# hyeeiin/ECG-Multimodal-Model

Hardware: AMD Instinct MI355X
Metric: samples/sec fwd+bwd, batch-256 multimodal (img+sig+clin), 1->8 MI355X (higher is better)
Workload: dtype bf16; 1 GPU; full multimodal (image 3x224x224 + 5000-pt signal + 16-dim clinical), fwd+bwd+Adam, encoders unfrozen; image_hw=224x224, per_gpu_batch=256, global_batch=256, parallelism=dp1

## Files before the change

### ecg-multimodal-model_amd/csrc/api.hip

```cpp
#include <stdarg.h>

#include "ops.h"

static thread_local char g_err[512] = "";

void ecg_set_error(const char* fmt, ...) {
  va_list ap;
  va_start(ap, fmt);
  vsnprintf(g_err, sizeof(g_err), fmt, ap);
  va_end(ap);
}

static inline ConvGeom geom_of(const ecgmm_conv_desc* c) {
  return make_geom(c->N, c->H, c->W, c->Cin, c->Cout, c->R, c->S, c->stride, c->pad_h, c->pad_w);
}
#define S_(x) ((hipStream_t)(x))

extern "C" {

int ecgmm_version(void) { return ECGMM_VERSION; }
const char* ecgmm_last_error(void) { return g_err; }

const char* ecgmm_switch_name(int i) { return i >= 0 && i < sw::COUNT ? sw::ALL[i]->env : nullptr; }
int ecgmm_switch_get(const char* env_name, int64_t* value) {
  Switch* s = sw::find(env_name);
  if (!s) ECG_FAIL(ECGMM_ERR_SHAPE, "switch_get: unknown switch %s", env_name ? env_name : "(null)");
  if (!value) ECG_FAIL(ECGMM_ERR_SHAPE, "switch_get: null value pointer");
  *value = s->get();
  return 0;
}
int ecgmm_switch_set(const char* env_name, int64_t value) {
  Switch* s = sw::find(env_name);
  if (!s) ECG_FAIL(ECGMM_ERR_SHAPE, "switch_set: unknown switch %s", env_name ? env_name : "(null)");
  if (s == &sw::SIDE_WGRAD)
    ECG_FAIL(ECGMM_ERR_SHAPE, "switch_set: ECGMM_SIDE_WGRAD is each plan's own state after start-up, call ecgmm_side_wgrad()");
  if (!s->runtime) ECG_FAIL(ECGMM_ERR_SHAPE, "switch_set: %s is read once at start-up", s->env);
  s->set((long)value);
  return 0;
}
int ecgmm_conv_halo_enable(int on) { sw::CONV_HALO.set(on); return 0; }
int ecgmm_conv_halo_cus(int cus) { sw::HALO_CUS.set(cus); return 0; }
int ecgmm_conv_halo_w4(int on) { sw::HALO_W4.set(on); return 0; }
int ecgmm_conv_halo_stagger(int on) { sw::HALO_STAGGER.set(on); return 0; }
int ecgmm_conv_halo_stream(int on) { sw::HALO_STREAM.set(on); return 0; }
int ecgmm_conv_halo_pingpong(int on) { sw::HALO_PP.set(on); return 0; }
int ecgmm_conv_wgrad_pingpong(int on) { sw::WGRAD_PP.set(on); return 0; }
int ecgmm_conv_wgrad_ring_enable(int on) { sw::WGRAD_RING.set(on); return 0; }
int ecgmm_bn_fold(int on) { sw::BN_FOLD.set(on); return 0; }
int ecgmm_bn_fold_slice(int on) { sw::BN_FOLD_SLICE.set(on); return 0; }
int ecgmm_bn_dual(int on) { ecg_bn_dual_set(on); return 0; }
int ecgmm_bn_fuse_min_pixels(int64_t m) { sw::BN_FUSE_MIN_M.set((long)m); return 0; }
int ecgmm_stem_recompute(int on) { sw::STEM_RECOMPUTE.set(on); return 0; }
int ecgmm_infer_down_side(int on) { sw::INFER_DOWN_SIDE.set(on); return 0; }

int ecgmm_nchw_to_nhwc(int dtype, const float* src, void* dst, int N, int C, int64_t HW, void* stream) {
  return ecg_nchw_to_nhwc(dtype, src, dst, N, C, (long)HW, S_(stream));
}
int ecgmm_nhwc_to_nchw(int dtype, const void* src, float* dst, int N, int C, int64_t HW, void* stream) {
  return ecg_nhwc_to_nchw(dtype, src, dst, N, C, (long)HW, S_(stream));
}
int ecgmm_cast(int dtype, const float* src, void* dst, int64_t n, void* stream) {
  return ecg_cast(dtype, src, dst, (long)n, S_(stream));
}
int ecgmm_uncast(int dtype, const void* src, float* dst, int64_t n, void* stream) {
  return ecg_uncast(dtype, src, dst, (long)n, S_(stream));
}
int ecgmm_pack_conv_weight(int dtype, const float* w, void* fwd, void* dgrad, int Cout, int Cin, int RS,
                           void* stream) {
  return ecg_pack_weight(dtype, w, fwd, dgrad, Cout, Cin, RS, S_(stream));
}

int ecgmm_conv_stats_rows(int64_t out_pixels) { return ecg_conv_stats_rows((long)out_pixels); }
int ecgmm_conv_fwd(int dtype, const ecgmm_conv_desc* c, const void* x, const void* w_fwd, const float* bias, void* y,
                   float* stats, int act, void* stream) {
  return ecg_conv_igemm(dtype, 0, geom_of(c), x, w_fwd, y, bias, nullptr, stats, act, S_(stream));
}
int ecgmm_conv_bwd_data(int dtype, const ecgmm_conv_desc* c, const void* dy, const void* w_dgrad, const void* addend,
                        void* dx, void* stream) {
  return ecg_conv_igemm(dtype, 1, geom_of(c), dy, w_dgrad, dx, nullptr, addend, nullptr, 0, S_(stream));
}
size_t ecgmm_conv_bwd_weight_workspace(int dtype, const ecgmm_conv_desc* c) {
  return ecg_conv_wgrad_workspace(dtype, geom_of(c));
}
int ecgmm_conv_bwd_weight(int dtype, const ecgmm_conv_desc* c, const void* x, const void* dy, float* dw, int accumulate,
                          void* ws, size_t ws_bytes, void* stream) {
  return ecg_conv_wgrad(dtype, geom_of(c), x, dy, dw, accumulate, ws, ws_bytes, S_(stream));
}

size_t ecgmm_stem_packed_elems(int Cin, int R) { return ecg_stem_packed_elems(Cin, R); }
int ecgmm_stem_stats_rows(int N, int Cin, int H, int W, int R) { return ecg_stem_stats_rows(N, Cin, H, W, R); }
int ecgmm_stem_pack(int dtype, const float* w, void* packed, int Cin, int R, void* stream) {
  return ecg_stem_pack(dtype, w, packed, Cin, R, S_(stream));
}
int ecgmm_stem_fwd(int dtype, const float* x, const void* packed, const float* bias, void* y, float* stats, int N,
                   int Cin, int H, int W, int R, void* stream) {
  return ecg_stem_fwd(dtype, x, packed, bias, y, stats, N, Cin, H, W, R, S_(stream));
}
int ecgmm_stem_wg_stats_rows(int N, int Cin, int H, int W, int R) { return ecg_stem_wg_stats_rows(N, Cin, H, W, R); }
int ecgmm_stem_fwd_wgrows(int dtype, const float* x, const void* packed, const float* bias, void* y, float* stats, int N,
                          int Cin, int H, int W, int R, void* stream) {
  return ecg_stem_fwd_wgrows(dtype, x, packed, bias, y, stats, N, Cin, H, W, R, S_(stream));
}
int ecgmm_stem_stats_only_rows(int N, int Cin, int H, int W, int R) { return ecg_stem_stats_only_rows(N, Cin, H, W, R); }
int ecgmm_stem_stats_only(int dtype, const float* x, const void* packed, const float* bias, float* stats, int N, int Cin,
                          int H, int W, int R, void* stream) {
  return ecg_stem_stats_only(dtype, x, packed, bias, stats, N, Cin, H, W, R, S_(stream));
}
int ecgmm_stem_pool_fwd(const float* x, const void* packed, const float* coef, void* pooled, uint8_t* idx, int N, int Cin,
                        int H, int W, void* stream) {
  return ecg_stem_pool_fwd(x, packed, coef, pooled, idx, N, Cin, H, W, S_(stream));
}
size_t ecgmm_stem_pool_bwd_workspace(int N, int Cin, int H, int W) { return ecg_stem_pool_bwd_workspace(N, Cin, H, W); }
int ecgmm_stem_pool_bwd(const float* x, const void* packed, const float* coef, const float* gamma, const void* dp,
                        const void* pooled, const uint8_t* idx, float* dgamma, float* dbeta, float* dw_oihw, void* ws,
                        size_t ws_bytes, int N, int Cin, int H, int W, void* stream) {
  return ecg_stem_pool_bwd(x, packed, coef, gamma, dp, pooled, idx, dgamma, dbeta, dw_oihw, ws, ws_bytes, N, Cin, H, W,
                           S_(stream));
}
size_t ecgmm_stem_bwd_weight_workspace(int N, int Cin, int H, int W, int R) {
  return ecg_stem_wgrad_workspace(N, Cin, H, W, R);
}
int ecgmm_stem_bwd_weight(int dtype, const float* x, const void* dy, float* dw, int accumulate, void* ws,
                          size_t ws_bytes, int N, int Cin, int H, int W, int R, void* stream) {
  return ecg_stem_wgrad(dtype, x, dy, dw, accumulate, ws, ws_bytes, N, Cin, H, W, R, S_(stream));
}

int ecgmm_stem_bwd_data(int dtype, const void* dy, const float* w_oihw, float* dx, int N, int Cin, int H, int W, int R,
                        void* stream) {
  return ecg_stem_dgrad(dtype, dy, w_oihw, dx, N, Cin, H, W, R, S_(stream));
}

int ecgmm_bn_eval_bwd(int dtype, const void* dout, const void* maskref, const float* gate, const float* addc,
                      int rows_per_sample, const void* y, const float* coef, float* dgamma, float* dbeta, void* dy,
                      void* dz_out, float* dbias, int64_t M, int C, float* scratch, void* stream) {
  return ecg_bn_eval_bwd(dtype, dout, maskref, gate, addc, rows_per_sample, y, coef, dgamma, dbeta, dy, dz_out, dbias,
                         (long)M, C, scratch, S_(stream));
}
int ecgmm_bn_small_eval_bwd(const float* x, const float* dy, const float* gamma, const float* save, float* dx,
                            float* dgamma, float* dbeta, int N, int C, int accumulate, void* stream) {
  return ecg_bn_small_eval_bwd(x, dy, gamma, save, dx, dgamma, dbeta, N, C, accumulate, S_(stream));
}

int ecgmm_col_stats_rows(int dtype, int64_t M, int C) { return ecg_bn_rows(dtype, (long)M, C); }
int ecgmm_col_stats(int dtype, const void* x, int64_t M, int C, float* partial, void* stream) {
  int rows = 0;
  return ecg_col_stats(dtype, x, (long)M, C, partial, &rows, S_(stream));
}
int ecgmm_bn_finalize(const float* partial, int rows, int C, double count, const float* gamma, const float* beta,
                      float* rm, float* rv, int64_t* nbt, float momentum, float eps, float* coef, void* stream) {
  return ecg_bn_finalize(partial, rows, C, count, gamma, beta, rm, rv, (long long*)nbt, momentum, eps, coef,
                         S_(stream));
}
int ecgmm_bn_eval_coef(int C, const float* gamma, const float* beta, const float* rm, const float* rv, float eps,
                       float* coef, void* stream) {
  return ecg_bn_eval_coef(C, gamma, beta, rm, rv, eps, coef, S_(stream));
}
int ecgmm_bn_act(int dtype, const void* y, const float* coef, const void* res, const float* rcoef, const float* gate,
                 int rows_per_sample, int relu, void* out, int64_t M, int C, void* stream) {
  return ecg_bn_act(dtype, y, coef, res, rcoef, gate, rows_per_sample, relu, out, (long)M, C, S_(stream));
}
int ecgmm_bn_act_from_rows(int dtype, const void* y, const float* partial, int rows, double count, const float* gamma,
                           const float* beta, float* running_mean, float* running_var, int64_t* num_batches_tracked,
                           float momentum, float eps, float* coef_out, const void* res, const float* rcoef,
                           const float* gate, int rows_per_sample, int relu, void* out, int64_t M, int C, void* stream) {
  return ecgmm_bn_act_from_rows_bits(dtype, y, partial, rows, count, gamma, beta, running_mean, running_var, num_batches_tracked,
                                     momentum, eps, coef_out, res, rcoef, gate, rows_per_sample, relu, out, nullptr, M, C, stream);
}
int ecgmm_bn_act_from_rows_bits(int dtype, const void* y, const float* partial, int rows, double count, const float* gamma,
                                const float* beta, float* running_mean, float* running_var, int64_t* num_batches_tracked,
                                float momentum, float eps, float* coef_out, const void* res, const float* rcoef,
                                const float* gate, int rows_per_sample, int relu, void* out, uint8_t* relu_bits, int64_t M,
                                int C, void* stream) {
  if (!partial || !coef_out) ECG_FAIL(ECGMM_ERR_SHAPE, "bn_act_from_rows: null partial rows / coef");
  if (!ecg_bn_fold_ok(C, rows)) {
    ECG_TRY(ecg_bn_finalize(partial, rows, C, count, gamma, beta, running_mean, running_var, (long long*)num_batches_tracked,
                            momentum, eps, coef_out, S_(stream)));
    return ecg_bn_act(dtype, y, coef_out, res, rcoef, gate, rows_per_sample, relu, out, (long)M, C, S_(stream), relu_bits);
  }
  EcgBnFold f = {partial, rows, count, gamma, beta, running_mean, running_var, (long long*)num_batches_tracked, momentum, eps};
  return ecg_bn_act_fold(dtype, y, coef_out, f, res, rcoef, gate, rows_per_sample, relu, out, (long)M, C, S_(stream), relu_bits);
}
size_t ecgmm_bn_bwd_scratch(int dtype, int64_t M, int C) { return ecg_bn_bwd_scratch(dtype, (long)M, C); }
int ecgmm_bn_bwd(int dtype, const void* dout, const void* maskref, const float* gate, const float* addc,
                 int rows_per_sample, const void* y, const float* coef, const float* gamma, float* dgamma,
                 float* dbeta, void* dy, void* dz_out, float* dbias, int64_t M, int C, void* scratch, void* stream) {
  return ecg_bn_bwd(dtype, dout, maskref, gate, addc, rows_per_sample, y, coef, gamma, dgamma, dbeta, dy, dz_out, dbias,
                    (long)M, C, (float*)scratch, S_(stream));
}
int ecgmm_bn_bwd_bits(int dtype, const void* dout, const uint8_t* mask_bits, const float* gate, const float* addc,
                      int rows_per_sample, const void* y, const float* coef, const float* gamma, float* dgamma,
                      float* dbeta, void* dy, void* dz_out, float* dbias, int64_t M, int C, void* scratch, void* stream) {
  if (dtype != ECGMM_BF16 || !mask_bits) ECG_FAIL(ECGMM_ERR_SHAPE, "bn_bwd_bits: bf16 with a bit mask only");
  return ecg_bn_bwd(dtype, dout, nullptr, gate, addc, rows_per_sample, y, coef, gamma, dgamma, dbeta, dy, dz_out, dbias,
                    (long)M, C, (float*)scratch, S_(stream), mask_bits);
}
int ecgmm_bn_bwd_dual(int dtype, const void* dout, const void* maskref, const uint8_t* mask_bits, const float* gate,
                      const float* addc, const void* y_a, const float* coef_a, const float* gamma_a, float* dgamma_a,
                      float* dbeta_a, void* dy_a, const void* y_b, const float* coef_b, const float* gamma_b,
                      float* dgamma_b, float* dbeta_b, void* dy_b, void* dz, float* dbias, int64_t M, int C, void* scratch_a,
                      void* scratch_b, void* stream) {
  return ecg_bn_bwd_dual(dtype, dout, maskref, mask_bits, gate, addc, y_a, coef_a, gamma_a, dgamma_a, dbeta_a, dy_a, y_b,
                         coef_b, gamma_b, dgamma_b, dbeta_b, dy_b, dz, dbias, (long)M, C, (float*)scratch_a, (float*)scratch_b,
                         S_(stream));
}

int ecgmm_conv_bwd_data_bnred(int dtype, const ecgmm_conv_desc* c, const void* dy, const void* w_dgrad,
                              const void* addend, void* dx, const void* bn_y, const void* bn_mask, const float* bn_coef,
                              float* rows, int* nrows, void* stream) {
  if (!bn_y || !bn_coef || !rows || !nrows) ECG_FAIL(ECGMM_ERR_SHAPE, "conv_bwd_data_bnred: null BatchNorm operand");
  const ConvGeom g = geom_of(c);
  *nrows = 0;
  if (!ecg_conv_halo_ok(dtype, 1, g))
    return ecg_conv_igemm(dtype, 1, g, dy, w_dgrad, dx, nullptr, addend, nullptr, 0, S_(stream));
  ConvEpi e = {};
  e.wg_rows = 1; e.red_y = bn_y; e.red_mask = bn_mask; e.red_coef = bn_coef; e.red_rows = rows;
  int rc = ecg_conv_igemm(dtype, 1, g, dy, w_dgrad, dx, nullptr, addend, nullptr, 0, S_(stream), &e);
  if (rc == 0 && e.red_done) *nrows = e.red_rows_n;
  return rc;
}
int ecgmm_conv_fwd_wgrows(int dtype, const ecgmm_conv_desc* c, const void* x, const void* w_fwd, const float* bias, void* y,
                          float* stats, int* nrows, int act, void* stream) {
  if (!stats || !nrows) ECG_FAIL(ECGMM_ERR_SHAPE, "conv_fwd_wgrows: null statistics buffer / row count");
// ... 273 lines not shown
```

### ecg-multimodal-model_amd/csrc/conv_wgrad.hip

```cpp
#include "ops.h"

namespace {

struct WgradParams {
  const void* x;
  const void* dy;
  float* slab;
  int N, H, W, Cin, OH, OW, Cout, S, stride, pad_h, pad_w;
  int M;
  int steps_per_split;
  unsigned mul_hw, sh_hw, mul_w, sh_w;
};

__device__ __forceinline__ void wg_dma16(__amdgpu_buffer_rsrc_t rs, unsigned char* lds_wave_base, unsigned voffset) {
#if defined(__HIP_DEVICE_COMPILE__)
  __builtin_amdgcn_raw_ptr_buffer_load_lds(rs, (__attribute__((address_space(3))) void*)lds_wave_base, 16, voffset, 0, 0,
                                           0);
#endif
}

#ifdef ECG_STAMP
__device__ unsigned long long g_wstamp[8];
#define ECG_WSTAMP_AT(t)                                                                 \
  do {                                                                                    \
// ... 490 lines not shown
      s16x4 hi = __builtin_amdgcn_ds_read_tr16_b64_v4i16((__attribute__((address_space(3))) s16x4*)lds_ptr(a0 + 512u));
      uint2 l2 = __builtin_bit_cast(uint2, lo), h2 = __builtin_bit_cast(uint2, hi);
      fa[a] = (u32x4){l2.x, l2.y, h2.x, h2.y};
    }
    int n_ow = st_ow + d_ow;
    const bool cw = n_ow >= p.W;
    n_ow -= cw ? p.W : 0;
    int n_oh = st_oh + d_oh + (cw ? 1 : 0);
    if (n_oh >= p.H) n_oh -= p.H;
    const unsigned n_rot = (rot + 4096u) & (RING_BYTES - 1);
    const TapOk nk = tap_ok(n_oh, n_ow);
    (void)rot;
    auto rd_tap = [&](int t, u32x4& fb) {
#if defined(WG_ABL) && WG_ABL == 2
      fb = (u32x4){al[t], ah[t], 0x3c003c00u, 0x3c003c00u};
      return;
#endif
      s16x4 lo = __builtin_amdgcn_ds_read_tr16_b64_v4i16((__attribute__((address_space(3))) s16x4*)lds_ptr(al[t]));
      s16x4 hi = __builtin_amdgcn_ds_read_tr16_b64_v4i16((__attribute__((address_space(3))) s16x4*)lds_ptr(ah[t]));
      uint2 l2 = __builtin_bit_cast(uint2, lo), h2 = __builtin_bit_cast(uint2, hi);
      fb = (u32x4){l2.x, l2.y, h2.x, h2.y};
    };
    u32x4 fbA, fbB;
    rd_tap(0, fbA);
#pragma unroll
    for (int t = 0; t < NT; ++t) {
      u32x4& cur = (t & 1) ? fbB : fbA;
      u32x4& nxt = (t & 1) ? fbA : fbB;
      if (t + 1 < NT) rd_tap(t + 1, nxt);
#if defined(WG_ABL) && WG_ABL == 1
      asm volatile("" ::"v"(cur), "v"(fa[0]), "v"(fa[1]), "v"(fa[2]), "v"(fa[3]));
#else
#pragma unroll
      for (int a = 0; a < TA; ++a)
        acc[t][a] = __builtin_amdgcn_mfma_f32_16x16x32_bf16(__builtin_bit_cast(bf16x8_t, fa[a]),
                                                            __builtin_bit_cast(bf16x8_t, cur), acc[t][a], 0, 0, 0);
#endif
      if (t >= 1) tap_addr(t - 1, nk, n_rot, al[t - 1], ah[t - 1]);
      if (PP_OK && t == PP_SPLIT - 1 && pp) {
        __builtin_amdgcn_sched_barrier(0);
        __builtin_amdgcn_s_barrier();
        __builtin_amdgcn_sched_barrier(0);
      }
    }
    tap_addr(NT - 1, nk, n_rot, al[NT - 1], ah[NT - 1]);
    st_oh = n_oh;
    st_ow = n_ow;
  };

  const int nsteps = max(s_end - s_begin, 0);
  if (iters > 0) {
    if (nsteps > 0) {
      for (int pc = wv; pc * 8 < 32 + 2 * p.HLa; pc += 4) x_piece(P0 - p.HLa + pc * 8);
      dy_piece(0, s_begin);
      for (int j = 1; j < RING_D && j < nsteps; ++j) dma_step(j, s_begin + j);
    }
    ring_wait_vmcnt<0>();
    __builtin_amdgcn_s_waitcnt(0xC07F);
    __builtin_amdgcn_s_barrier();
    unsigned rot = 0u;
    if (pp && grp == 1) __builtin_amdgcn_s_barrier();
    for (int k = 0; k < iters; ++k) {
      if (GROUPS == 1 || k < nsteps) {
#if !(defined(WG_ABL) && WG_ABL == 3)
        if (k + RING_D < nsteps) dma_step((k + RING_D) % RING_NDY, s_begin + k + RING_D);
#endif
        compute(k % RING_NDY, rot);
        rot = (rot + 4096u) & (RING_BYTES - 1);
        const int younger = (k + RING_D < nsteps ? k + RING_D : nsteps - 1) - (k + 1);
        if (younger >= 2) ring_wait_vmcnt<4>();
        else if (younger == 1) ring_wait_vmcnt<2>();
        else ring_wait_vmcnt<0>();
      } else if (pp) {
        __builtin_amdgcn_s_barrier();
      }
      __builtin_amdgcn_s_waitcnt(0xC07F);
      __builtin_amdgcn_s_barrier();
    }
    if (pp && grp == 0) __builtin_amdgcn_s_barrier();
  }

  if constexpr (GROUPS == 2) {
    float* red = reinterpret_cast<float*>(smem_wg) + (tid & 255);
    if (grp == 1) {
#pragma unroll
      for (int t = 0; t < NT; ++t)
#pragma unroll
        for (int a = 0; a < TA; ++a)
#pragma unroll
          for (int j = 0; j < 4; ++j) red[((t * TA + a) * 4 + j) * 256] = acc[t][a][j];
    }
    __syncthreads();
    if (grp == 1) return;
#pragma unroll
    for (int t = 0; t < NT; ++t)
#pragma unroll
      for (int a = 0; a < TA; ++a)
#pragma unroll
        for (int j = 0; j < 4; ++j) acc[t][a][j] += red[((t * TA + a) * 4 + j) * 256];
  }

  float* base = p.slab + (((size_t)split * NT) * p.Cout + co0 + fq * 4) * p.Cin + ci0 + wave * 16 + fr;
#pragma unroll
  for (int t = 0; t < NT; ++t)
#pragma unroll
    for (int a = 0; a < TA; ++a)
#pragma unroll
      for (int j = 0; j < 4; ++j) base[((size_t)t * p.Cout + a * 16 + j) * p.Cin] = acc[t][a][j];
}

void magic_div(unsigned d, unsigned& m, unsigned& sh) {
  int l = 0;
  while ((1u << l) < d) ++l;
  m = (unsigned)(((1ull << (31 + l)) + d - 1) / d);
  sh = 31 + l;
}

__global__ void wgrad_reduce_kernel(const float* __restrict__ slab, float* __restrict__ grad, int nsplit, int RS,
                                    int Cout, int Cin, int accumulate) {
  __shared__ float sh[4][64];
  size_t per = (size_t)RS * Cout * Cin;
  size_t i = (size_t)blockIdx.x * 64 + (threadIdx.x & 63);
  const int grp = threadIdx.x >> 6;
  float s0 = 0.f, s1 = 0.f;
  if (i < per) {
    int k = grp;
    for (; k + 12 < nsplit; k += 16) {
      const float a0 = slab[(size_t)k * per + i], a1 = slab[(size_t)(k + 4) * per + i];
      const float a2 = slab[(size_t)(k + 8) * per + i], a3 = slab[(size_t)(k + 12) * per + i];
      s0 += a0;
      s1 += a1;
      s0 += a2;
      s1 += a3;
    }
    for (; k + 4 < nsplit; k += 8) {
      s0 += slab[(size_t)k * per + i];
      s1 += slab[(size_t)(k + 4) * per + i];
    }
    if (k < nsplit) s0 += slab[(size_t)k * per + i];
  }
  sh[grp][threadIdx.x & 63] = s0 + s1;
  __syncthreads();
  if (grp == 0 && i < per) {
    float s = (sh[0][threadIdx.x] + sh[1][threadIdx.x]) + (sh[2][threadIdx.x] + sh[3][threadIdx.x]);
    int ci = (int)(i % Cin);
    size_t r = i / Cin;
    int co = (int)(r % Cout);
    int tap = (int)(r / Cout);
    size_t o = ((size_t)co * Cin + ci) * RS + tap;
    grad[o] = accumulate ? grad[o] + s : s;
  }
}

template <typename T, int NT, int GROUPS>
int launch_wgrad_nt(WgradParams& p, dim3 grid, hipStream_t stream) {
  size_t lds = (size_t)GROUPS * 2 * (1 + NT) * 4096;
  if (GROUPS == 2 && lds < (size_t)NT * 16 * 1024) lds = (size_t)NT * 16 * 1024;
  static bool attr_set = false;
  if (!attr_set) {
    (void)hipFuncSetAttribute((const void*)wgrad_kernel<T, NT, GROUPS>, hipFuncAttributeMaxDynamicSharedMemorySize, (int)lds);
    attr_set = true;
  }
  hipLaunchKernelGGL((wgrad_kernel<T, NT, GROUPS>), grid, dim3(256 * GROUPS), lds, stream, p);
  ECG_CHECK_LAUNCH("wgrad_kernel");
  return 0;
}

int wgrad_groups(int dtype, const ConvGeom& g) {
  return dtype == ECGMM_BF16 && g.R * g.S >= 3 && !sw::WGRAD_GROUPS.get() ? 2 : 1;
}

template <typename T>
int launch_wgrad(const ConvGeom& g, WgradParams& p, int nsplit, int groups, hipStream_t stream) {
  const int RS = g.R * g.S;
  dim3 grid(ceil_div(g.Cout, 64) * ceil_div(g.Cin, 64), nsplit);
  if (g.S != 1 && g.S != 3) ECG_FAIL(ECGMM_ERR_SHAPE, "conv wgrad: filter width %d unsupported (1 or 3)", g.S);
  if constexpr (sizeof(T) == 2) {
    if (groups == 2 && RS == 3) return launch_wgrad_nt<T, 3, 2>(p, grid, stream);
    if (groups == 2 && RS == 9) return launch_wgrad_nt<T, 9, 2>(p, grid, stream);
  }
  if (RS == 1) return launch_wgrad_nt<T, 1, 1>(p, grid, stream);
  if (RS == 3) return launch_wgrad_nt<T, 3, 1>(p, grid, stream);
  if (RS == 9) return launch_wgrad_nt<T, 9, 1>(p, grid, stream);
  ECG_FAIL(ECGMM_ERR_SHAPE, "conv wgrad: %dx%d filter unsupported (1, 3 or 9 taps)", g.R, g.S);
}

bool wgrad_ring_ok(int dtype, const ConvGeom& g) {
  const long level = sw::WGRAD_RING.get();
  if (!level || dtype != ECGMM_BF16 || g.stride != 1 || g.S != 3 || g.pad_w != 1) return false;
  if (!((g.R == 3 && g.pad_h == 1) || (g.R == 1 && g.pad_h == 0))) return false;
  if (g.OH != g.H || g.OW != g.W || g.W < 4 || g.Cin % 64 || g.Cout % 64) return false;
  const int HL = g.pad_h * g.W + 1, HLa = (HL + 7) / 8 * 8;
  if (HL + HLa + 32 * RING_D + 32 > RING_ROWS) return false;
  const double M = (double)g.N * g.H * g.W;
  if (!(M * g.Cin * 2.0 < 2.0e9 && M * g.Cout * 2.0 < 2.0e9)) return false;
  if (level == 2) return true;
  return g.R == 3 || g.Cin >= 128;
}

template <int NT, int GROUPS>
int launch_wgrad_ring(const WgradRingParams& p, dim3 grid, hipStream_t stream) {
  int lds = GROUPS * RING_LDS;
  if (GROUPS == 2 && lds < NT * 16 * 1024) lds = NT * 16 * 1024;
  static bool attr_set = false;
  if (!attr_set) {
    (void)hipFuncSetAttribute((const void*)wgrad_ring_kernel<NT, GROUPS>, hipFuncAttributeMaxDynamicSharedMemorySize, lds);
    attr_set = true;
  }
  hipLaunchKernelGGL((wgrad_ring_kernel<NT, GROUPS>), grid, dim3(256 * GROUPS), lds, stream, p);
  ECG_CHECK_LAUNCH("wgrad_ring_kernel");
  return 0;
}

bool g_wgrad_narrow = false;
int g_wgrad_narrow_slots = 256;
int pick_nsplit(const ConvGeom& g, int kp, int groups) {
  long M = (long)g.N * g.OH * g.OW;
  int tiles = ceil_div(g.Cout, 64) * ceil_div(g.Cin, 64);
  int steps = ceil_div(M, kp);
  const int slots_env = (int)sw::WGRAD_WGS.get();
  const int slots = slots_env > 0 ? slots_env : (g_wgrad_narrow ? g_wgrad_narrow_slots : 512);
  int want = ceil_div(slots / groups, tiles);
  int ns = want < 1 ? 1 : want;
  if (ns > steps) ns = steps;
  if (ns > 512) ns = 512;
  return ns < 1 ? 1 : ns;
}

}

void ecg_conv_wgrad_narrow(bool narrow, int slots) { g_wgrad_narrow = narrow; g_wgrad_narrow_slots = slots > 0 ? slots : 256; }

size_t ecg_conv_wgrad_workspace(int dtype, const ConvGeom& g) {
  const bool keep = g_wgrad_narrow;
  g_wgrad_narrow = false;
  struct Restore { bool v; ~Restore() { g_wgrad_narrow = v; } } restore{keep};
  int ns = pick_nsplit(g, dtype == ECGMM_BF16 ? 32 : 16, 1);
  return (size_t)ns * g.R * g.S * g.Cout * g.Cin * sizeof(float);
}

int ecg_conv_wgrad(int dtype, const ConvGeom& g, const void* x, const void* dy, float* grad_oihw, int accumulate,
                   void* workspace, size_t workspace_bytes, hipStream_t stream) {
  const int kp = dtype == ECGMM_BF16 ? 32 : 16;
  const int vec = dtype == ECGMM_BF16 ? 8 : 4;
  if (g.Cin % vec || g.Cout % vec)
    ECG_FAIL(ECGMM_ERR_SHAPE, "conv wgrad: channels (%d,%d) must be multiples of %d", g.Cin, g.Cout, vec);
  long M = (long)g.N * g.OH * g.OW;
  if (M <= 0 || M > 0x7fffffffL) ECG_FAIL(ECGMM_ERR_SHAPE, "conv wgrad: pixel count %ld out of range", M);
  const bool ring = wgrad_ring_ok(dtype, g);
  const int groups = wgrad_groups(dtype, g);
  int ns = pick_nsplit(g, kp, groups);
  size_t need = (size_t)ns * g.R * g.S * g.Cout * g.Cin * sizeof(float);
  if (workspace_bytes < need || !workspace)
    ECG_FAIL(ECGMM_ERR_WORKSPACE, "conv wgrad: workspace %zu < %zu bytes", workspace_bytes, need);
  WgradParams p;
  p.x = x; p.dy = dy; p.slab = (float*)workspace;
  p.N = g.N; p.H = g.H; p.W = g.W; p.Cin = g.Cin; p.OH = g.OH; p.OW = g.OW; p.Cout = g.Cout; p.S = g.S;
  p.stride = g.stride; p.pad_h = g.pad_h; p.pad_w = g.pad_w; p.M = (int)M;
  p.steps_per_split = ceil_div(ceil_div(M, kp), ns);
  magic_div((unsigned)(g.OH * g.OW), p.mul_hw, p.sh_hw);
  magic_div((unsigned)g.OW, p.mul_w, p.sh_w);
  if (dtype != ECGMM_BF16 && dtype != ECGMM_F32) ECG_FAIL(ECGMM_ERR_DTYPE, "conv wgrad: bad dtype %d", dtype);
  ecg_prof_begin(ECG_PROF_WGRAD, 2.0 * (double)M * g.Cout * g.R * g.S * g.Cin,
                 (double)dtype_size(dtype) * ((double)g.N * g.H * g.W * g.Cin + (double)M * g.Cout) +
                     4.0 * g.R * g.S * g.Cin * g.Cout,
                 stream);
  int rc;
  if (ring) {
    WgradRingParams q;
    q.x = x; q.dy = dy; q.slab = (float*)workspace;
    q.H = g.H; q.W = g.W; q.Cin = g.Cin; q.Cout = g.Cout; q.pad_h = g.pad_h; q.M = (int)M;
    q.steps_per_split = p.steps_per_split;
    q.HL = g.pad_h * g.W + 1;
    q.HLa = (q.HL + 7) / 8 * 8;
    q.mul_hw = p.mul_hw; q.sh_hw = p.sh_hw; q.mul_w = p.mul_w; q.sh_w = p.sh_w;
    q.pingpong = (int)sw::WGRAD_PP.get();
    dim3 grid((g.Cout / 64) * (g.Cin / 64), ns);
    if (groups == 2) rc = g.R == 3 ? launch_wgrad_ring<9, 2>(q, grid, stream) : launch_wgrad_ring<3, 2>(q, grid, stream);
    else rc = g.R == 3 ? launch_wgrad_ring<9, 1>(q, grid, stream) : launch_wgrad_ring<3, 1>(q, grid, stream);
  } else {
    rc = dtype == ECGMM_BF16 ? launch_wgrad<bf16_t>(g, p, ns, groups, stream) : launch_wgrad<float>(g, p, ns, 1, stream);
  }
  ecg_prof_end(stream);
  ECG_TRY(rc);
  size_t per = (size_t)g.R * g.S * g.Cout * g.Cin;
  hipLaunchKernelGGL(wgrad_reduce_kernel, dim3(ceil_div(per, 64)), dim3(256), 0, stream, (const float*)workspace,
                     grad_oihw, ns, g.R * g.S, g.Cout, g.Cin, accumulate);
  ECG_CHECK_LAUNCH("wgrad_reduce_kernel");
  return 0;
}
```

### ecg-multimodal-model_amd/csrc/elementwise.hip

```cpp
#include "ops.h"

namespace {

constexpr int EW_THREADS = 256;

__device__ __forceinline__ u32x4 ld16(const void* p) { return *reinterpret_cast<const u32x4*>(p); }
__device__ __forceinline__ u32x4 ld16s(const void* p) {
#ifndef EW_NO_NT
  return __builtin_nontemporal_load(reinterpret_cast<const u32x4*>(p));
#else
  return *reinterpret_cast<const u32x4*>(p);
#endif
}
struct RowDiv { unsigned mul, sh; };
__device__ __forceinline__ long row_div(long r, RowDiv d) { return (long)(((unsigned long long)(unsigned)r * d.mul) >> d.sh); }
static RowDiv make_row_div(int d) {
  unsigned dd = d < 1 ? 1u : (unsigned)d;
  int l = 0;
  while ((1u << l) < dd) ++l;
  RowDiv r;
  r.mul = (unsigned)(((1ull << (31 + l)) + dd - 1) / dd);
  r.sh = 31u + (unsigned)l;
  return r;
}
// ... 1174 lines not shown
    unpack16<T>(qv, v);
#pragma unroll
    for (int j = 0; j < VEC; ++j) {
      f[j] = m[j] > 0.f ? f[j] : 0.f;
      const float yc = v[j] - mu[j];
      ag[j] += f[j] * (v[j] * sc[j] + sf[j]);
      a1[j] += f[j];
      a2[j] += f[j] * yc;
      a3[j] += yc;
    }
    st16(dz + o, pack16<T>(f));
  };
  int r = slice;
  for (; r + 3 * nsl < R; r += 4 * nsl) {
    u32x4 qd[4], qm[4], qv[4];
#pragma unroll
    for (int u = 0; u < 4; ++u) {
      const size_t o = ((size_t)n * R + r + u * nsl) * C + c0;
      qd[u] = ld16(dout + o);
      qm[u] = ld16(maskref + o);
      qv[u] = ld16(y + o);
    }
    __builtin_amdgcn_sched_barrier(0);
#pragma unroll
    for (int u = 0; u < 4; ++u) row(((size_t)n * R + r + u * nsl) * C + c0, qd[u], qm[u], qv[u]);
  }
  for (; r < R; r += nsl) {
    const size_t o = ((size_t)n * R + r) * C + c0;
    const u32x4 qd = ld16(dout + o), qm = ld16(maskref + o), qv = ld16(y + o);
    row(o, qd, qm, qv);
  }
  float* const outs[4] = {dg, a1o, a2o, a3o};
#pragma unroll
  for (int q = 0; q < 4; ++q) {
#pragma unroll
    for (int j = 0; j < VEC; ++j) sh[threadIdx.x][j] = q == 0 ? ag[j] : q == 1 ? a1[j] : q == 2 ? a2[j] : a3[j];
    __syncthreads();
    for (int c = threadIdx.x; c < C; c += EW_THREADS) {
      const int ck = c / VEC, j = c % VEC;
      float s_ = 0.f;
      for (int k = 0; k < nsl; ++k) s_ += sh[k * cpr + ck][j];
      outs[q][(size_t)n * C + c] = s_;
    }
    __syncthreads();
  }
}

constexpr int SE_ROWS = 16;
__global__ __launch_bounds__(256) void se_bn_rows_kernel(const float* __restrict__ a1, const float* __restrict__ a2,
                                                         const float* __restrict__ a3, const float* __restrict__ gate,
                                                         const float* __restrict__ addc, int N, int R, int C,
                                                         float* __restrict__ rows) {
  __shared__ float sh[2][4][64];
  const int c = blockIdx.x * 64 + (threadIdx.x & 63), sl = threadIdx.x >> 6, j = blockIdx.y;
  float s1 = 0.f, s2 = 0.f;
  if (c < C)
    for (int n = j + SE_ROWS * sl; n < N; n += SE_ROWS * 4) {
      const size_t o = (size_t)n * C + c;
      const float g = gate ? gate[o] : 1.f, ad = addc ? addc[o] : 0.f;
      s1 += g * a1[o] + ad * (float)R;
      s2 += g * a2[o] + ad * a3[o];
    }
  sh[0][sl][threadIdx.x & 63] = s1;
  sh[1][sl][threadIdx.x & 63] = s2;
  __syncthreads();
  if (sl == 0 && c < C) {
    float* row = rows + (size_t)j * 2 * C;
    row[c] = (sh[0][0][threadIdx.x] + sh[0][1][threadIdx.x]) + (sh[0][2][threadIdx.x] + sh[0][3][threadIdx.x]);
    row[C + c] = (sh[1][0][threadIdx.x] + sh[1][1][threadIdx.x]) + (sh[1][2][threadIdx.x] + sh[1][3][threadIdx.x]);
  }
}

template <typename T>
__global__ void bcast_rows_kernel(const float* __restrict__ v, T* __restrict__ out, long total, int R, int C,
                                  float scale) {
  for (long i = (long)blockIdx.x * blockDim.x + threadIdx.x; i < total; i += (long)gridDim.x * blockDim.x) {
    int c = (int)(i % C);
    long n = i / ((long)R * C);
    Elem<T>::st(out + i, v[n * C + c] * scale);
  }
}

template <typename T>
__global__ __launch_bounds__(1024) void bcast_rows_vec_kernel(const float* __restrict__ v, T* __restrict__ out, long M,
                                                              RowDiv rdiv, int C, float scale) {
  constexpr int VEC = Elem<T>::VEC;
  const int cpr = C / VEC, rpi = 1024 / cpr;
  const int c0 = (threadIdx.x % cpr) * VEC, r0 = threadIdx.x / cpr;
  for (long r = (long)blockIdx.x * rpi + r0; r < M; r += (long)gridDim.x * rpi) {
    const float* src = v + row_div(r, rdiv) * C + c0;
    float f[VEC];
#pragma unroll
    for (int j = 0; j < VEC; ++j) f[j] = src[j] * scale;
    st16(out + r * C + c0, pack16<T>(f));
  }
}

template <typename T>
__global__ void pack_weight_kernel(const float* __restrict__ w, T* __restrict__ fwd, T* __restrict__ dgr, int Cout,
                                   int Cin, int RS) {
  long total = (long)Cout * Cin * RS;
  for (long i = (long)blockIdx.x * blockDim.x + threadIdx.x; i < total; i += (long)gridDim.x * blockDim.x) {
    int tap = (int)(i % RS);
    long r = i / RS;
    int ci = (int)(r % Cin), co = (int)(r / Cin);
    float v = w[i];
    if (fwd) Elem<T>::st(fwd + ((size_t)co * RS + tap) * Cin + ci, v);
    if (dgr) Elem<T>::st(dgr + ((size_t)ci * RS + tap) * Cout + co, v);
  }
}

struct PackBatch {
  const float* w[ECG_PACK_MAX];
  void* fwd[ECG_PACK_MAX];
  void* dgr[ECG_PACK_MAX];
  int cout[ECG_PACK_MAX], cin[ECG_PACK_MAX], rs[ECG_PACK_MAX];
  int blk0[ECG_PACK_MAX + 1];
  int n;
};
constexpr int PACK_T = 32, PACK_RS_MAX = 9;
template <typename T>
__global__ __launch_bounds__(256) void pack_weight_batch_kernel(PackBatch b) {
  __shared__ float tile[PACK_T][PACK_T * PACK_RS_MAX + 1];
  int t = 0;
  while (t + 1 < b.n && (int)blockIdx.x >= b.blk0[t + 1]) ++t;
  const int Cout = b.cout[t], Cin = b.cin[t], RS = b.rs[t];
  const float* __restrict__ w = b.w[t];
  T* __restrict__ fwd = (T*)b.fwd[t];
  T* __restrict__ dgr = (T*)b.dgr[t];
  const int ci_tiles = (Cin + PACK_T - 1) / PACK_T;
  const int lb = blockIdx.x - b.blk0[t];
  const int co0 = (lb / ci_tiles) * PACK_T, ci0 = (lb % ci_tiles) * PACK_T;
  const int nci = min(PACK_T, Cin - ci0), nco = min(PACK_T, Cout - co0);
  const int run = nci * RS;
  for (int i = threadIdx.x; i < nco * run; i += 256) {
    const int co = i / run, k = i - co * run;
    tile[co][k] = w[((size_t)(co0 + co) * Cin + ci0) * RS + k];
  }
  __syncthreads();
  if (fwd) {
    for (int i = threadIdx.x; i < nco * RS * PACK_T; i += 256) {
      const int ci = i % PACK_T, ct = i / PACK_T, tap = ct % RS, co = ct / RS;
      if (ci < nci) Elem<T>::st(fwd + ((size_t)(co0 + co) * RS + tap) * Cin + ci0 + ci, tile[co][ci * RS + tap]);
    }
  }
  if (dgr) {
    for (int i = threadIdx.x; i < nci * RS * PACK_T; i += 256) {
      const int co = i % PACK_T, ct = i / PACK_T, tap = ct % RS, ci = ct / RS;
      if (co < nco) Elem<T>::st(dgr + ((size_t)(ci0 + ci) * RS + tap) * Cout + co0 + co, tile[co][ci * RS + tap]);
    }
  }
}

template <typename T, bool TO_NHWC>
__global__ __launch_bounds__(256) void nchw_nhwc_kernel(const void* __restrict__ src_, void* __restrict__ dst_, int C,
                                                        long HW) {
  __shared__ float tile[32][33];
  const int n = blockIdx.z;
  const long p0 = (long)blockIdx.x * 32;
  const int c0 = blockIdx.y * 32;
  const int tx = threadIdx.x & 31, ty = threadIdx.x >> 5;
  if (TO_NHWC) {
    const float* src = (const float*)src_ + (size_t)n * C * HW;
    T* dst = (T*)dst_ + (size_t)n * C * HW;
    for (int k = ty; k < 32; k += 8) {
      int c = c0 + k;
      long pp = p0 + tx;
      tile[k][tx] = (c < C && pp < HW) ? src[(size_t)c * HW + pp] : 0.f;
    }
    __syncthreads();
    for (int k = ty; k < 32; k += 8) {
      long pp = p0 + k;
      int c = c0 + tx;
      if (c < C && pp < HW) Elem<T>::st(dst + (size_t)pp * C + c, tile[tx][k]);
    }
  } else {
    const T* src = (const T*)src_ + (size_t)n * C * HW;
    float* dst = (float*)dst_ + (size_t)n * C * HW;
    for (int k = ty; k < 32; k += 8) {
      long pp = p0 + k;
      int c = c0 + tx;
      tile[k][tx] = (c < C && pp < HW) ? Elem<T>::ld(src + (size_t)pp * C + c) : 0.f;
    }
    __syncthreads();
    for (int k = ty; k < 32; k += 8) {
      int c = c0 + k;
      long pp = p0 + tx;
      if (c < C && pp < HW) dst[(size_t)c * HW + pp] = tile[tx][k];
    }
  }
}

template <typename T>
__global__ void cast_kernel(const float* __restrict__ src, T* __restrict__ dst, long n) {
  for (long i = (long)blockIdx.x * blockDim.x + threadIdx.x; i < n; i += (long)gridDim.x * blockDim.x)
    Elem<T>::st(dst + i, src[i]);
}
template <typename T>
__global__ void uncast_kernel(const T* __restrict__ src, float* __restrict__ dst, long n) {
  for (long i = (long)blockIdx.x * blockDim.x + threadIdx.x; i < n; i += (long)gridDim.x * blockDim.x)
    dst[i] = Elem<T>::ld(src + i);
}

inline int ew_grid(long work_items, int per_block) {
  long b = (work_items + per_block - 1) / per_block;
  if (b > 4096) b = 4096;
  if (b < 1) b = 1;
  return (int)b;
}
inline bool chunk_ok(int C, int dtype) {
  int vec = dtype == ECGMM_BF16 ? 8 : 4;
  if (C % vec) return false;
  int cpr = C / vec;
  return cpr <= EW_THREADS && (EW_THREADS % cpr) == 0;
}

}

#define DISPATCH_T(dtype, CALL_BF16, CALL_F32, what)                 \
  if ((dtype) == ECGMM_BF16) { CALL_BF16; }                          \
  else if ((dtype) == ECGMM_F32) { CALL_F32; }                       \
  else ECG_FAIL(ECGMM_ERR_DTYPE, what ": bad dtype %d", (int)(dtype))

int ecg_bn_rows(int dtype, long M, int C) {
  int vec = dtype == ECGMM_BF16 ? 8 : 4;
  if (C < vec) return 1;
  int rpi = EW_THREADS / (C / vec);
  int g = ew_grid(M, rpi * 8);
  return g > 1024 ? 1024 : g;
}

static int fold_rows(const float*& partial, int& rows, int width, hipStream_t stream) {
  if (rows <= 512) return 0;
  float* tail = const_cast<float*>(partial) + (size_t)rows * width;
  int chunk = ceil_div(rows, ECG_TAIL_ROWS);
  int nb = ceil_div(rows, chunk);
  hipLaunchKernelGGL(rows_stage1_kernel, dim3(ceil_div(width, 64), nb), dim3(1024), 0, stream, partial, rows, width,
                     chunk, tail);
  ECG_CHECK_LAUNCH("rows_stage1");
  partial = tail;
  rows = nb;
  return 0;
}

int ecg_bn_finalize(const float* partial, int rows, int C, double count, const float* gamma, const float* beta,
                    float* rm, float* rv, long long* nbt, float momentum, float eps, float* coef,
                    hipStream_t stream) {
  ECG_TRY(fold_rows(partial, rows, 2 * C, stream));
  hipLaunchKernelGGL(bn_finalize_kernel, dim3(ceil_div(C, 64)), dim3(1024), 0, stream, partial, rows, C, count, gamma,
                     beta, rm, rv, nbt, momentum, eps, coef);
  ECG_CHECK_LAUNCH("bn_finalize");
  return 0;
}

int ecg_bn_eval_coef(int C, const float* gamma, const float* beta, const float* rm, const float* rv, float eps,
                     float* coef, hipStream_t stream) {
  hipLaunchKernelGGL(bn_eval_coef_kernel, dim3(ceil_div(C, 256)), dim3(256), 0, stream, C, gamma, beta, rm, rv, eps,
                     coef);
  ECG_CHECK_LAUNCH("bn_eval_coef");
  return 0;
}

int ecg_col_stats(int dtype, const void* x, long M, int C, float* partial, int* rows_out, hipStream_t stream) {
  if (!chunk_ok(C, dtype)) ECG_FAIL(ECGMM_ERR_SHAPE, "col_stats: C=%d unsupported", C);
  int grid = ecg_bn_rows(dtype, M, C);
  *rows_out = grid;
  DISPATCH_T(dtype,
             hipLaunchKernelGGL(col_stats_kernel<bf16_t>, dim3(grid), dim3(EW_THREADS), 0, stream, (const bf16_t*)x, M,
                                C, partial),
             hipLaunchKernelGGL(col_stats_kernel<float>, dim3(grid), dim3(EW_THREADS), 0, stream, (const float*)x, M, C,
                                partial),
             "col_stats");
  ECG_CHECK_LAUNCH("col_stats");
  return 0;
}

bool ecg_bn_fold_ok(int C, int rows) {
  if (!sw::BN_FOLD.get() || rows < 1 || rows > 512 || C > 512) return false;
  return C >= 128 ? C % 128 == 0 : (C >= 16 && 1024 % C == 0);
}

static int bn_fold_slices(int C) {
  return sw::BN_FOLD_SLICE.get() && C >= 256 && C % 128 == 0 ? C / 128 : 1;
}
static dim3 bn_fold_grid(int dtype, long M, int C, int ns, int threads, int trips) {
  const int vec = dtype == ECGMM_BF16 ? 8 : 4;
  int gx = ew_grid(M, (threads / (C / ns / vec)) * trips);
  if (gx > 256 / ns) gx = 256 / ns;
  return dim3(gx, ns);
}

int ecg_bn_act_fold(int dtype, const void* y, float* coef, const EcgBnFold& f, const void* res, const float* rcoef,
                    const float* gate, int rows_per_sample, int relu, void* out, long M, int C, hipStream_t stream,
                    unsigned char* relu_bits) {
  if (!chunk_ok(C, dtype)) ECG_FAIL(ECGMM_ERR_SHAPE, "bn_act: C=%d unsupported", C);
  if (!ecg_bn_fold_ok(C, f.rows)) ECG_FAIL(ECGMM_ERR_SHAPE, "bn_act_fold: C=%d rows=%d not foldable", C, f.rows);
  BnActParams p;
  memset(&p, 0, sizeof(p));
  p.y = y; p.coef = coef; p.res = res; p.rcoef = rcoef; p.gate = gate; p.out = out; p.M = M; p.C = C;
  p.rows_per_sample = rows_per_sample > 0 ? rows_per_sample : 1; p.relu = relu;
  p.rdiv = make_row_div(p.rows_per_sample);
  p.fin.partial = f.partial; p.fin.rows = f.rows; p.fin.count = f.count; p.fin.gamma = f.gamma; p.fin.beta = f.beta;
  p.fin.rm = f.rm; p.fin.rv = f.rv; p.fin.nbt = f.nbt; p.fin.momentum = f.momentum; p.fin.eps = f.eps; p.fin.coef_out = coef;
  p.relu_bits = dtype == ECGMM_BF16 && relu ? relu_bits : nullptr;
  const dim3 grid = bn_fold_grid(dtype, M, C, bn_fold_slices(C), BN_ACT_THREADS, 4);
  DISPATCH_T(dtype, hipLaunchKernelGGL(bn_act_kernel<bf16_t>, grid, dim3(BN_ACT_THREADS), 0, stream, p),
// ... 255 lines not shown

bool ecg_stem_fuse_on() { return sw::STEM_FUSE.get() != 0; }

int ecg_pool_bn_bwd(int dtype, const void* dp, const void* pooled, const unsigned char* idx, const void* y,
                    const float* coef, const float* gamma, float* dgamma, float* dbeta, void* dy, float* dbias, int N,
                    int H, int W, int C, float* scratch, hipStream_t stream) {
  if (!chunk_ok(C, dtype)) ECG_FAIL(ECGMM_ERR_SHAPE, "pool_bn_bwd: C=%d unsupported", C);
  const int OH = (H - 1) / 2 + 1, OW = (W - 1) / 2 + 1;
  const int rows = bn_bwd_rows(dtype, (long)N * H * W, C);
  DISPATCH_T(dtype, (pool_bwd_launch<bf16_t>(dp, pooled, idx, y, coef, gamma, dgamma, dbeta, dy, dbias, N, H, W, C, OH, OW, scratch, rows, stream)),
             (pool_bwd_launch<float>(dp, pooled, idx, y, coef, gamma, dgamma, dbeta, dy, dbias, N, H, W, C, OH, OW, scratch, rows, stream)),
             "pool_bn_bwd");
  ECG_CHECK_LAUNCH("pool_bn_bwd");
  return 0;
}

int ecg_rows_sum(const float* partial, int rows, int C, float* out, int accumulate, hipStream_t stream) {
  hipLaunchKernelGGL(rows_sum_kernel, dim3(ceil_div(C, 64)), dim3(1024), 0, stream, partial, rows, C, out, accumulate);
  ECG_CHECK_LAUNCH("rows_sum");
  return 0;
}

int ecg_bnrelu_maxpool(int dtype, const void* y, const float* coef, void* out, unsigned char* idx, int N, int H, int W,
                       int C, hipStream_t stream) {
  if (!chunk_ok(C, dtype)) ECG_FAIL(ECGMM_ERR_SHAPE, "maxpool: C=%d unsupported", C);
  int OH = (H + 2 - 3) / 2 + 1, OW = (W + 2 - 3) / 2 + 1;
  int vec = dtype == ECGMM_BF16 ? 8 : 4;
  int grid = ew_grid((long)N * OH * ((OW + 1) / 2) * (C / vec), EW_THREADS);
  DISPATCH_T(dtype,
             hipLaunchKernelGGL(bnrelu_maxpool_kernel<bf16_t>, dim3(grid), dim3(EW_THREADS), 0, stream,
                                (const bf16_t*)y, coef, (bf16_t*)out, idx, N, H, W, C, OH, OW),
             hipLaunchKernelGGL(bnrelu_maxpool_kernel<float>, dim3(grid), dim3(EW_THREADS), 0, stream, (const float*)y,
                                coef, (float*)out, idx, N, H, W, C, OH, OW),
             "maxpool");
  ECG_CHECK_LAUNCH("bnrelu_maxpool");
  return 0;
}

int ecg_maxpool_relu_bwd(int dtype, const void* dp, const void* pooled, const unsigned char* idx, void* dz, int N,
                         int H, int W, int C, hipStream_t stream) {
  if (!chunk_ok(C, dtype)) ECG_FAIL(ECGMM_ERR_SHAPE, "maxpool bwd: C=%d unsupported", C);
  int OH = (H + 2 - 3) / 2 + 1, OW = (W + 2 - 3) / 2 + 1;
  int vec = dtype == ECGMM_BF16 ? 8 : 4;
  int grid = ew_grid((long)N * ((H + 1) / 2) * ((W + 1) / 2) * (C / vec), EW_THREADS);
  DISPATCH_T(dtype,
             hipLaunchKernelGGL(maxpool_relu_bwd_kernel<bf16_t>, dim3(grid), dim3(EW_THREADS), 0, stream,
                                (const bf16_t*)dp, (const bf16_t*)pooled, idx, (bf16_t*)dz, N, H, W, C, OH, OW),
             hipLaunchKernelGGL(maxpool_relu_bwd_kernel<float>, dim3(grid), dim3(EW_THREADS), 0, stream,
                                (const float*)dp, (const float*)pooled, idx, (float*)dz, N, H, W, C, OH, OW),
             "maxpool bwd");
  ECG_CHECK_LAUNCH("maxpool_relu_bwd");
  return 0;
}

int ecg_avgpool(int dtype, const void* x, float* out, int N, int R, int C, const float* coef, hipStream_t stream) {
  if (!chunk_ok(C, dtype)) ECG_FAIL(ECGMM_ERR_SHAPE, "avgpool: C=%d unsupported", C);
  DISPATCH_T(dtype,
             hipLaunchKernelGGL((sample_reduce_kernel<bf16_t, false>), dim3(N), dim3(EW_THREADS), 0, stream,
                                (const bf16_t*)x, (const bf16_t*)nullptr, (const bf16_t*)nullptr, coef, out, R, C),
             hipLaunchKernelGGL((sample_reduce_kernel<float, false>), dim3(N), dim3(EW_THREADS), 0, stream,
                                (const float*)x, (const float*)nullptr, (const float*)nullptr, coef, out, R, C),
             "avgpool");
  ECG_CHECK_LAUNCH("avgpool");
  return 0;
}

int ecg_bcast_rows(int dtype, const float* v, void* out, int N, int R, int C, float scale, hipStream_t stream) {
  long total = (long)N * R * C;
  const int vecw = dtype == ECGMM_BF16 ? 8 : 4;
  if (C % vecw == 0 && C / vecw <= 1024 && 1024 % (C / vecw) == 0 && ((uintptr_t)out & 15) == 0) {
    const long M = (long)N * R;
    int g = ew_grid(M, (1024 / (C / vecw)) * 4);
    if (g > 256) g = 256;
    DISPATCH_T(dtype,
               hipLaunchKernelGGL(bcast_rows_vec_kernel<bf16_t>, dim3(g), dim3(1024), 0, stream, v, (bf16_t*)out, M, make_row_div(R), C, scale),
               hipLaunchKernelGGL(bcast_rows_vec_kernel<float>, dim3(g), dim3(1024), 0, stream, v, (float*)out, M, make_row_div(R), C, scale),
               "bcast_rows");
    ECG_CHECK_LAUNCH("bcast_rows_vec");
    return 0;
  }
  int grid = ew_grid(total, 256);
  DISPATCH_T(dtype,
             hipLaunchKernelGGL(bcast_rows_kernel<bf16_t>, dim3(grid), dim3(256), 0, stream, v, (bf16_t*)out, total, R,
                                C, scale),
             hipLaunchKernelGGL(bcast_rows_kernel<float>, dim3(grid), dim3(256), 0, stream, v, (float*)out, total, R, C,
                                scale),
             "bcast_rows");
  ECG_CHECK_LAUNCH("bcast_rows");
  return 0;
}

int ecg_se_gate_grad(int dtype, const void* dout, const void* maskref, const void* y, const float* coef, float* dg,
                     int N, int R, int C, hipStream_t stream) {
  if (!chunk_ok(C, dtype)) ECG_FAIL(ECGMM_ERR_SHAPE, "se_gate_grad: C=%d unsupported", C);
  DISPATCH_T(dtype,
             hipLaunchKernelGGL((sample_reduce_kernel<bf16_t, true>), dim3(N), dim3(EW_THREADS), 0, stream,
                                (const bf16_t*)dout, (const bf16_t*)maskref, (const bf16_t*)y, coef, dg, R, C),
             hipLaunchKernelGGL((sample_reduce_kernel<float, true>), dim3(N), dim3(EW_THREADS), 0, stream,
                                (const float*)dout, (const float*)maskref, (const float*)y, coef, dg, R, C),
             "se_gate_grad");
  ECG_CHECK_LAUNCH("se_gate_grad");
  return 0;
}

int ecg_se_gate_bn(int dtype, const void* dout, const void* maskref, const void* y, const float* coef, void* dz,
                   float* dg, float* a1, float* a2, float* a3, int N, int R, int C, hipStream_t stream) {
  if (!chunk_ok(C, dtype)) ECG_FAIL(ECGMM_ERR_SHAPE, "se_gate_bn: C=%d unsupported", C);
  DISPATCH_T(dtype,
             hipLaunchKernelGGL(se_gate_bn_kernel<bf16_t>, dim3(N), dim3(EW_THREADS), 0, stream, (const bf16_t*)dout,
                                (const bf16_t*)maskref, (const bf16_t*)y, coef, (bf16_t*)dz, dg, a1, a2, a3, R, C),
             hipLaunchKernelGGL(se_gate_bn_kernel<float>, dim3(N), dim3(EW_THREADS), 0, stream, (const float*)dout,
                                (const float*)maskref, (const float*)y, coef, (float*)dz, dg, a1, a2, a3, R, C),
             "se_gate_bn");
  ECG_CHECK_LAUNCH("se_gate_bn");
  return 0;
}
int ecg_se_bn_rows(const float* a1, const float* a2, const float* a3, const float* gate, const float* addc, int N, int R,
                   int C, float* rows, hipStream_t stream) {
  hipLaunchKernelGGL(se_bn_rows_kernel, dim3(ceil_div(C, 64), SE_ROWS), dim3(256), 0, stream, a1, a2, a3, gate, addc, N, R,
                     C, rows);
  ECG_CHECK_LAUNCH("se_bn_rows");
  return 0;
}
int ecg_se_bn_nrows() { return SE_ROWS; }

int ecg_pack_weight(int dtype, const float* w_oihw, void* fwd, void* dgrad, int Cout, int Cin, int RS,
                    hipStream_t stream) {
  long total = (long)Cout * Cin * RS;
  int grid = ew_grid(total, 256);
  DISPATCH_T(dtype,
             hipLaunchKernelGGL(pack_weight_kernel<bf16_t>, dim3(grid), dim3(256), 0, stream, w_oihw, (bf16_t*)fwd,
                                (bf16_t*)dgrad, Cout, Cin, RS),
             hipLaunchKernelGGL(pack_weight_kernel<float>, dim3(grid), dim3(256), 0, stream, w_oihw, (float*)fwd,
                                (float*)dgrad, Cout, Cin, RS),
             "pack_weight");
  ECG_CHECK_LAUNCH("pack_weight");
  return 0;
}

int ecg_pack_weight_batch(int dtype, const EcgPackItem* items, int n, hipStream_t stream) {
  for (int base = 0; base < n; base += ECG_PACK_MAX) {
    PackBatch b;
    memset(&b, 0, sizeof(b));
    b.n = n - base < ECG_PACK_MAX ? n - base : ECG_PACK_MAX;
    int blocks = 0;
    for (int i = 0; i < b.n; ++i) {
      const EcgPackItem& it = items[base + i];
      b.w[i] = it.w; b.fwd[i] = it.fwd; b.dgr[i] = it.dgrad; b.cout[i] = it.Cout; b.cin[i] = it.Cin; b.rs[i] = it.RS;
      b.blk0[i] = blocks;
      if (it.RS > 9) ECG_FAIL(ECGMM_ERR_SHAPE, "pack_weight_batch: %d taps unsupported (<= 9)", it.RS);
      blocks += ceil_div(it.Cout, 32) * ceil_div(it.Cin, 32);
    }
    b.blk0[b.n] = blocks;
    DISPATCH_T(dtype, hipLaunchKernelGGL(pack_weight_batch_kernel<bf16_t>, dim3(blocks), dim3(256), 0, stream, b),
               hipLaunchKernelGGL(pack_weight_batch_kernel<float>, dim3(blocks), dim3(256), 0, stream, b), "pack_weight_batch");
    ECG_CHECK_LAUNCH("pack_weight_batch");
  }
  return 0;
}

int ecg_nchw_to_nhwc(int dtype, const float* src, void* dst, int N, int C, long HW, hipStream_t stream) {
  dim3 grid(ceil_div(HW, 32), ceil_div(C, 32), N);
  DISPATCH_T(dtype,
             hipLaunchKernelGGL((nchw_nhwc_kernel<bf16_t, true>), grid, dim3(256), 0, stream, src, dst, C, HW),
             hipLaunchKernelGGL((nchw_nhwc_kernel<float, true>), grid, dim3(256), 0, stream, src, dst, C, HW),
             "nchw_to_nhwc");
  ECG_CHECK_LAUNCH("nchw_to_nhwc");
  return 0;
}

int ecg_nhwc_to_nchw(int dtype, const void* src, float* dst, int N, int C, long HW, hipStream_t stream) {
  dim3 grid(ceil_div(HW, 32), ceil_div(C, 32), N);
  DISPATCH_T(dtype,
             hipLaunchKernelGGL((nchw_nhwc_kernel<bf16_t, false>), grid, dim3(256), 0, stream, src, dst, C, HW),
             hipLaunchKernelGGL((nchw_nhwc_kernel<float, false>), grid, dim3(256), 0, stream, src, dst, C, HW),
             "nhwc_to_nchw");
  ECG_CHECK_LAUNCH("nhwc_to_nchw");
  return 0;
}

int ecg_cast(int dtype, const float* src, void* dst, long n, hipStream_t stream) {
  int grid = ew_grid(n, 256);
  DISPATCH_T(dtype, hipLaunchKernelGGL(cast_kernel<bf16_t>, dim3(grid), dim3(256), 0, stream, src, (bf16_t*)dst, n),
             hipLaunchKernelGGL(cast_kernel<float>, dim3(grid), dim3(256), 0, stream, src, (float*)dst, n), "cast");
  ECG_CHECK_LAUNCH("cast");
  return 0;
}
int ecg_uncast(int dtype, const void* src, float* dst, long n, hipStream_t stream) {
  int grid = ew_grid(n, 256);
  DISPATCH_T(dtype,
             hipLaunchKernelGGL(uncast_kernel<bf16_t>, dim3(grid), dim3(256), 0, stream, (const bf16_t*)src, dst, n),
             hipLaunchKernelGGL(uncast_kernel<float>, dim3(grid), dim3(256), 0, stream, (const float*)src, dst, n),
             "uncast");
  ECG_CHECK_LAUNCH("uncast");
  return 0;
}
```

### ecg-multimodal-model_amd/csrc/ops.h

```cpp
#pragma once
#include "common.h"
#include "switches.h"

int ecg_iir_lanes(const double* a, int order, int E);

int ecg_conv_stats_rows(long M);
struct ConvEpi {
  const void* red_y;
  const void* red_mask;
  const float* red_coef;
  float* red_rows;
  int wg_rows;
  const void* src2;
  const void* wpk2;
  int src2_done;
  int stats_rows;
  int red_done;
  int red_rows_n;
};
int ecg_conv_igemm(int dtype, int mode, const ConvGeom& g, const void* src, const void* wpk, void* dst,
                   const float* bias, const void* addend, float* stats, int act, hipStream_t stream,
                   ConvEpi* epi = nullptr);
bool ecg_conv_halo_ok(int dtype, int mode, const ConvGeom& g);
int ecg_conv_halo_rows(int mode, const ConvGeom& g);
int ecg_conv_halo(int mode, const ConvGeom& g, const void* src, const void* wpk, void* dst, const float* bias,
                  const void* addend, float* stats, int act, ConvEpi* epi, hipStream_t stream);
size_t ecg_conv_wgrad_workspace(int dtype, const ConvGeom& g);
void ecg_conv_wgrad_narrow(bool narrow, int slots = 256);
int ecg_conv_wgrad(int dtype, const ConvGeom& g, const void* x, const void* dy, float* grad_oihw, int accumulate,
                   void* workspace, size_t workspace_bytes, hipStream_t stream);
size_t ecg_stem_packed_elems(int Cin, int R);
int ecg_stem_stats_rows(int N, int Cin, int H, int W, int R);
int ecg_stem_pack(int dtype, const float* w, void* out, int Cin, int R, hipStream_t stream);
int ecg_stem_fwd(int dtype, const float* x, const void* wpk, const float* bias, void* y, float* stats, int N, int Cin,
                 int H, int W, int R, hipStream_t stream);
size_t ecg_stem_wgrad_workspace(int N, int Cin, int H, int W, int R);
int ecg_stem_wgrad(int dtype, const float* x, const void* dy, float* grad, int accumulate, void* workspace,
                   size_t workspace_bytes, int N, int Cin, int H, int W, int R, hipStream_t stream);
int ecg_stem_stats_only_rows(int N, int Cin, int H, int W, int R);
int ecg_stem_wg_stats_rows(int N, int Cin, int H, int W, int R);
int ecg_stem_fwd_wgrows(int dtype, const float* x, const void* wpk, const float* bias, void* y, float* stats, int N, int Cin,
                        int H, int W, int R, hipStream_t stream);
int ecg_stem_stats_only(int dtype, const float* x, const void* wpk, const float* bias, float* stats, int N, int Cin, int H,
                        int W, int R, hipStream_t stream);
int ecg_stem_wgrad_reduce(const float* slab, float* grad, int rows, int NG, int accumulate, hipStream_t stream);
int ecg_stem_dgrad(int dtype, const void* dy, const float* w, float* dx, int N, int Cin, int H, int W, int R,
                   hipStream_t stream);
bool ecg_stem_fused_ok(int dtype, int Cin, int R);
int ecg_stem_pool_fwd(const float* x, const void* wpk, const float* coef, void* pooled, unsigned char* idx, int N, int Cin,
                      int H, int W, hipStream_t stream);
size_t ecg_stem_pool_bwd_workspace(int N, int Cin, int H, int W);
int ecg_stem_pool_bwd(const float* x, const void* wpk, const float* coef, const float* gamma, const void* dp, const void* pooled,
                      const unsigned char* idx, float* dgamma, float* dbeta, float* dw, void* ws, size_t ws_bytes, int N,
                      int Cin, int H, int W, hipStream_t stream);
int ecg_pool_bn_bwd_reduce(int dtype, const void* dp, const void* pooled, const float* coef, const float* gamma, float* dgamma,
                           float* dbeta, int N, int H, int W, int C, float* scratch, const float** bcoef_out,
                           hipStream_t stream);
int ecg_bn_rows(int dtype, long M, int C);
int ecg_bn_finalize(const float* partial, int rows, int C, double count, const float* gamma, const float* beta,
                    float* rm, float* rv, long long* nbt, float momentum, float eps, float* coef, hipStream_t stream);
int ecg_bn_eval_coef(int C, const float* gamma, const float* beta, const float* rm, const float* rv, float eps,
                     float* coef, hipStream_t stream);
int ecg_col_stats(int dtype, const void* x, long M, int C, float* partial, int* rows_out, hipStream_t stream);
struct EcgBnFold {
  const float* partial; int rows; double count;
  const float* gamma; const float* beta;
  float* rm; float* rv; long long* nbt;
  float momentum, eps;
};
bool ecg_bn_fold_ok(int C, int rows);
int ecg_bn_act_fold(int dtype, const void* y, float* coef, const EcgBnFold& f, const void* res, const float* rcoef,
                    const float* gate, int rows_per_sample, int relu, void* out, long M, int C, hipStream_t stream,
                    unsigned char* relu_bits = nullptr);
int ecg_bn_act(int dtype, const void* y, const float* coef, const void* res, const float* rcoef, const float* gate,
               int rows_per_sample, int relu, void* out, long M, int C, hipStream_t stream, unsigned char* relu_bits = nullptr);
size_t ecg_bn_bwd_scratch(int dtype, long M, int C);
int ecg_bn_bwd(int dtype, const void* dout, const void* maskref, const float* gate, const float* addc,
               int rows_per_sample, const void* y, const float* coef, const float* gamma, float* dgamma, float* dbeta,
               void* dy, void* dz_out, float* dbias, long M, int C, float* scratch, hipStream_t stream,
               const unsigned char* mask_bits = nullptr);
int ecg_bn_bwd_dual(int dtype, const void* dout, const void* maskref, const unsigned char* mask_bits, const float* gate,
                    const float* addc, const void* y_a, const float* coef_a, const float* gamma_a, float* dgamma_a,
                    float* dbeta_a, void* dy_a, const void* y_b, const float* coef_b, const float* gamma_b, float* dgamma_b,
                    float* dbeta_b, void* dy_b, void* dz, float* dbias, long M, int C, float* scratch_a, float* scratch_b,
                    hipStream_t stream);
void ecg_bn_dual_set(int on);
bool ecg_bn_dual_on();
int ecg_bn_bwd_tail(int dtype, const void* dout, const void* maskref, const void* y, const float* coef,
                    const float* gamma, float* dgamma, float* dbeta, void* dy, const float* partial, int rows, long M,
                    int C, float* scratch, hipStream_t stream, const float* gate = nullptr, const float* addc = nullptr,
                    int rows_per_sample = 1, float* dbias = nullptr);
int ecg_bn_eval_bwd(int dtype, const void* dout, const void* maskref, const float* gate, const float* addc,
                    int rows_per_sample, const void* y, const float* coef, float* dgamma, float* dbeta, void* dy,
                    void* dz_out, float* dbias, long M, int C, float* scratch, hipStream_t stream);
int ecg_bn_small_eval_bwd(const float* x, const float* dy, const float* gamma, const float* save, float* dx, float* dgamma,
                          float* dbeta, int N, int C, int accumulate, hipStream_t stream);
int ecg_gradcam(int dtype, const void* act, const float* dpooled, float* small, float* out, int N, int Hs, int Ws, int C,
                int H, int W, hipStream_t stream);
size_t ecg_crnn_gradcam_workspace(int B, int Tp, int Fp, int C);
int ecg_crnn_gradcam(const float* seq, const float* dseq, const int* steps, const int* frames, void* ws, size_t ws_bytes,
                     float* cam, int B, int Tp, int C, int Fp, int F, int T, hipStream_t stream);
int ecg_se_gate_bn(int dtype, const void* dout, const void* maskref, const void* y, const float* coef, void* dz,
                   float* dg, float* a1, float* a2, float* a3, int N, int R, int C, hipStream_t stream);
int ecg_se_bn_nrows();
int ecg_se_bn_rows(const float* a1, const float* a2, const float* a3, const float* gate, const float* addc, int N, int R,
                   int C, float* rows, hipStream_t stream);
int ecg_rows_sum(const float* partial, int rows, int C, float* out, int accumulate, hipStream_t stream);
int ecg_bnrelu_maxpool(int dtype, const void* y, const float* coef, void* out, unsigned char* idx, int N, int H, int W,
                       int C, hipStream_t stream);
int ecg_maxpool_relu_bwd(int dtype, const void* dp, const void* pooled, const unsigned char* idx, void* dz, int N,
                         int H, int W, int C, hipStream_t stream);
int ecg_pool_bn_bwd(int dtype, const void* dp, const void* pooled, const unsigned char* idx, const void* y,
                    const float* coef, const float* gamma, float* dgamma, float* dbeta, void* dy, float* dbias, int N,
                    int H, int W, int C, float* scratch, hipStream_t stream);
bool ecg_stem_fuse_on();
int ecg_avgpool(int dtype, const void* x, float* out, int N, int R, int C, const float* coef, hipStream_t stream);
int ecg_bcast_rows(int dtype, const float* v, void* out, int N, int R, int C, float scale, hipStream_t stream);
int ecg_se_gate_grad(int dtype, const void* dout, const void* maskref, const void* y, const float* coef, float* dg,
                     int N, int R, int C, hipStream_t stream);
constexpr int ECG_PACK_MAX = 24;
struct EcgPackItem {
  const float* w;
  void* fwd;
  void* dgrad;
  int Cout, Cin, RS;
};
int ecg_pack_weight_batch(int dtype, const EcgPackItem* items, int n, hipStream_t stream);
constexpr int ECG_FOLD_MAX = 32;
enum { ECG_FOLD_CONV = 0,
       ECG_FOLD_STEM = 1,
       ECG_FOLD_COPY = 2,
       ECG_FOLD_OIHW = 3 };
struct EcgFoldItem {
  int kind;
  const float* w;
  const float* conv_bias;
  const float *gamma, *beta, *rm, *rv;
  void* wout;
  float* bout;
  float* scale_out;
  int Cout, Cin, RS;
};
int ecg_fold_batch(int dtype, const EcgFoldItem* items, int n, float eps, hipStream_t stream);
int ecg_relu_maxpool(int dtype, const void* y, void* out, int N, int H, int W, int C, hipStream_t stream);
int ecg_gate_res_relu(int dtype, const void* y, const float* gate, const void* res, void* out, long M, int C,
                      int rows_per_sample, hipStream_t stream);
int ecg_resnet1d_side_enable(int on);
int ecg_pack_weight(int dtype, const float* w_oihw, void* fwd, void* dgrad, int Cout, int Cin, int RS,
                    hipStream_t stream);
int ecg_nchw_to_nhwc(int dtype, const float* src, void* dst, int N, int C, long HW, hipStream_t stream);
int ecg_nhwc_to_nchw(int dtype, const void* src, float* dst, int N, int C, long HW, hipStream_t stream);
int ecg_cast(int dtype, const float* src, void* dst, long n, hipStream_t stream);
int ecg_uncast(int dtype, const void* src, float* dst, long n, hipStream_t stream);
int ecg_linear_fwd_valu(const float* x, const float* w, const float* bias, float* y, int B, int In, int Out, int act,
                        hipStream_t s);
int ecg_linear_dgrad_valu(const float* dy, const float* w, float* dx, int B, int In, int Out, int accumulate,
                          hipStream_t s);
int ecg_linear_wgrad_valu(const float* dy, const float* x, float* dw, float* db, int B, int In, int Out,
                          int accumulate, hipStream_t s);
int ecg_act_bwd(const float* dy, const float* y, float* dz, long n, int act, hipStream_t s);
int ecg_axpby(float a, const float* x, float b, float* y, long n, hipStream_t s);
int ecg_layernorm_fwd(const float* const* seg, const int* dims, int nseg, const float* fusion_w, const float* gamma,
                      const float* beta, float* out, float* stat, float* soft_w, int B, float eps, hipStream_t s);
size_t ecg_layernorm_bwd_scratch(int B, int D);
int ecg_layernorm_bwd(const float* const* seg, const int* dims, int nseg, const float* fusion_w, const float* gamma,
                      const float* stat, const float* dout, float* const* dseg, int dseg_accumulate, float* dgamma,
                      float* dbeta, float* dfusion_w, int B, float* scratch, hipStream_t s);
bool ecg_head_fused_ok(const int* dim, int B, int hidden, int num_classes);
int ecg_head_partial_floats(const int* dim, int num_classes);
int ecg_head_bwd_blocks(int B);
int ecg_head_rows_fwd(const float* const* raw, const float* const* ln_g, const float* const* ln_b,
                      const float* const* cls_w, const float* const* cls_b, const float* aw, const float* fg,
                      const float* fb, float* const* feat, float* const* stat, float* const* logits, float* rowvar,
                      float* fused, float* statf, float* soft_w, const int* dim, int B, int NC, float eps,
                      hipStream_t s);
int ecg_head_rows_bwd(const float* const* raw, const float* const* ln_g, const float* const* cls_w, const float* aw,
                      const float* fg, const float* const* feat, const float* const* stat, const float* statf,
                      const float* dfused, const float* const* dlog, const float* dvar, const float* gs,
                      float* const* draw, const int* have, float* partial, const int* dim, int B, int NC,
                      hipStream_t s);
int ecg_head_finalize(const float* partial, int rows, const int* dim, int NC, float* const* g_ln, float* const* g_cls,
                      float* g_aw, float* g_fg, float* g_fb, const float* aw, const int* have, const int* have_cls,
                      int have_fusion, const float* dz, int B, int H, float* fc0_db, hipStream_t s);
// ... 106 lines not shown
```

### ecg-multimodal-model_amd/csrc/plan_common.h

```cpp
#pragma once
#include "net_desc.h"

inline const float* P(const void* const* params, int i) { return (const float*)params[i]; }
inline float* G(void* const* grads, int i) { return grads ? (float*)grads[i] : nullptr; }

#define ECG_NEED(ptr, have, need, what)                                                                       \
  do {                                                                                                        \
    if (!(ptr) || (have) < (need)) ECG_FAIL(ECGMM_ERR_WORKSPACE, "%s %zu < %zu", what, (size_t)(have), (size_t)(need)); \
  } while (0)

inline int bn_coef(const BnCfg& c, const float* stats, int rows, int C, long count, const void* const* params, int p_bn,
                   void* const* buffers, int b_bn, float* coef, hipStream_t s) {
  if (c.training)
    return ecg_bn_finalize(stats, rows, C, (double)count, P(params, p_bn), P(params, p_bn + 1), (float*)buffers[b_bn],
                           (float*)buffers[b_bn + 1], (long long*)buffers[b_bn + 2], c.momentum, c.eps, coef, s);
  return ecg_bn_eval_coef(C, P(params, p_bn), P(params, p_bn + 1), (const float*)buffers[b_bn],
                          (const float*)buffers[b_bn + 1], c.eps, coef, s);
}

inline int bn_bwd_mode(const BnCfg& c, const void* dout, const void* maskref, const float* gate, const float* addc, int rps,
                       const void* y, const float* coef, const float* gamma, float* dgamma, float* dbeta, void* dy,
                       void* dz_out, float* dbias, long M, int C, float* scratch, hipStream_t s,
                       const unsigned char* mask_bits = nullptr) {
  if (c.training)
    return ecg_bn_bwd(c.dtype, dout, maskref, gate, addc, rps, y, coef, gamma, dgamma, dbeta, dy, dz_out, dbias, M, C,
                      scratch, s, mask_bits);
  return ecg_bn_eval_bwd(c.dtype, dout, maskref, gate, addc, rps, y, coef, dgamma, dbeta, dy, dz_out, dbias, M, C, scratch,
                         s);
}

inline int stem_forward(int dt, const float* x, const void* wpk, const float* bias, void* y, float* stats, int N, int Cin,
                        int H, int W, int R, hipStream_t s) {
  if (dt == ECGMM_BF16) return ecg_stem_fwd_wgrows(dt, x, wpk, bias, y, stats, N, Cin, H, W, R, s);
  return ecg_stem_fwd(dt, x, wpk, bias, y, stats, N, Cin, H, W, R, s);
}
inline int stem_forward_rows(int dt, int N, int Cin, int H, int W, int R) {
  return dt == ECGMM_BF16 ? ecg_stem_wg_stats_rows(N, Cin, H, W, R) : ecg_stem_stats_rows(N, Cin, H, W, R);
}

inline int se_mlp_forward(const float* m, const float* w1, const float* b1, const float* w2, const float* b2, float* h,
                          float* g, int N, int C, int CR, hipStream_t s) {
  if (ecg_se_mlp_fused_ok(C, CR)) return ecg_se_mlp_fwd(m, w1, b1, w2, b2, h, g, N, C, CR, s);
  ECG_TRY(ecg_linear_fwd(m, w1, b1, h, N, C, CR, ECGMM_ACT_RELU, nullptr, s));
  return ecg_linear_fwd(h, w2, b2, g, N, CR, C, ECGMM_ACT_SIGMOID, nullptr, s);
}

struct BlockWs {
  void *w1f, *w1d, *w2f, *w2d, *wdf, *wdd;
  void *y1, *a1, *y2, *yd, *out;
  unsigned char* bits;
  float *coef1, *coef2, *coefd, *m, *h, *g;
};
inline void layout_block(Arena& a, BlockWs& b, int N, size_t pix, int cin, int cout, int taps, bool down, size_t es,
                         bool want_bits, int cr) {
  const size_t osz = (size_t)N * pix * cout, w1 = (size_t)cout * cin * taps * es, w2 = (size_t)cout * cout * taps * es;
  b = BlockWs{};
  b.w1f = a.take_bytes(w1, "w1f");
  b.w1d = a.take_bytes(w1, "w1d");
  b.w2f = a.take_bytes(w2, "w2f");
  b.w2d = a.take_bytes(w2, "w2d");
  b.y1 = a.take_bytes(osz * es, "y1");
  b.a1 = a.take_bytes(osz * es, "a1");
  b.y2 = a.take_bytes(osz * es, "y2");
  b.out = a.take_bytes(osz * es, "out");
  if (want_bits) b.bits = a.take<unsigned char>(osz / 8, "bits");
  b.coef1 = a.take<float>(4 * cout, "coef1");
  b.coef2 = a.take<float>(4 * cout, "coef2");
  if (cr) {
    b.m = a.take<float>((size_t)N * cout, "m");
    b.h = a.take<float>((size_t)N * cr, "h");
    b.g = a.take<float>((size_t)N * cout, "g");
  }
  if (down) {
    b.wdf = a.take_bytes((size_t)cout * cin * es, "wdf");
    b.wdd = a.take_bytes((size_t)cout * cin * es, "wdd");
    b.yd = a.take_bytes(osz * es, "yd");
    b.coefd = a.take<float>(4 * cout, "coefd");
  }
}

inline int ws_view_find(const char* who, const WsTable& t, const char* name, int index, size_t ws_bytes, size_t* offset,
                        size_t* bytes) {
  if (t.overflow) ECG_FAIL(ECGMM_ERR_SHAPE, "%s: more named tensors than the view table holds", who);
  for (int i = 0; i < t.n; ++i) {
    const WsTable::Entry& e = t.e[i];
    if (e.index != index || strcmp(e.name, name) != 0) continue;
    if (e.off + e.bytes > ws_bytes) ECG_FAIL(ECGMM_ERR_WORKSPACE, "%s: '%s' ends past the workspace", who, name);
    *offset = e.off;
    *bytes = e.bytes;
    return 0;
  }
  ECG_FAIL(ECGMM_ERR_SHAPE, "%s: no tensor '%s' (index %d) for this descriptor", who, name, index);
}
```

### ecg-multimodal-model_amd/csrc/plan_resnet18.hip

```cpp
#include "plan_common.h"
#include "side_stream.h"

namespace {
bool stem_recompute(int dtype) {
  return sw::STEM_RECOMPUTE.get() && ecg_stem_fused_ok(dtype, 3, 7);
}
bool relu_bits_on() { return sw::RELU_BITS.get() != 0; }

int build(const ecgmm_resnet18_desc* d, Net18& r) {
  ECG_TRY(net18_static(d, r, "resnet18"));
  return net18_shape(r, "resnet18");
}

struct FwdWs {
  void* wstem;
  void* y0; float* coef0; void* p0; unsigned char* idx0;
  BlockWs b[8];
  float* pooled;
  float* stats;
  float* stats_d;
  size_t bytes;
};

void layout_fwd(const Net18& r, void* base, FwdWs& w, WsTable* views = nullptr) {
// ... 159 lines not shown
  Net18 r;
  if (build(d, r)) return 0;
  BwdWs w;
  layout_bwd(r, nullptr, w);
  return w.bytes;
}

extern "C" int ecgmm_resnet18_ws_view(const ecgmm_resnet18_desc* d, int backward, const char* name, int index,
                                      size_t* offset, size_t* bytes) {
  Net18 r;
  ECG_TRY(build(d, r));
  if (!name || !offset || !bytes) ECG_FAIL(ECGMM_ERR_SHAPE, "resnet18 ws_view: null argument");
  WsTable t;
  FwdWs w;
  BwdWs q;
  if (backward) layout_bwd(r, nullptr, q, &t);
  else layout_fwd(r, nullptr, w, &t);
  return ws_view_find(backward ? "resnet18 ws_view (backward)" : "resnet18 ws_view (forward)", t, name, index,
                      backward ? q.bytes : w.bytes, offset, bytes);
}

extern "C" int ecgmm_resnet18_forward(const ecgmm_resnet18_desc* d, const float* image, const void* const* params,
                                      void* const* buffers, float* feat_out, void* ws, size_t ws_bytes,
                                      void* stream_) {
  hipStream_t s = (hipStream_t)stream_;
  Net18 r;
  ECG_TRY(build(d, r));
  FwdWs w;
  layout_fwd(r, ws, w);
  ECG_NEED(ws, ws_bytes, w.bytes, "resnet18 fwd: workspace");
  const int dt = r.d.dtype, N = r.d.N;
  const int stats_rows = r.d.training ? 1 : 0;
  ECG_TRY(side_init());
  const bool side_fwd = g_side.enabled && sw::DOWN_SIDE.get();

  ecg_tl_mark(100, s);
  {
    EcgPackItem items[ECG_PACK_MAX];
    int n = 0;
    for (int i = 0; i < 8; ++i) {
      const Blk18& k = r.blk[i];
      BlockWs& b = w.b[i];
      items[n++] = {P(params, k.p_conv1), b.w1f, b.w1d, k.cout, k.cin, 9};
      items[n++] = {P(params, k.p_conv2), b.w2f, b.w2d, k.cout, k.cout, 9};
      if (k.down) items[n++] = {P(params, k.p_dconv), b.wdf, b.wdd, k.cout, k.cin, 1};
    }
    ECG_TRY(ecg_pack_weight_batch(dt, items, n, s));
  }
  ECG_TRY(ecg_stem_pack(dt, P(params, 0), w.wstem, 3, 7, s));
  if (stem_recompute(dt)) {
    if (stats_rows) ECG_TRY(ecg_stem_stats_only(dt, image, w.wstem, nullptr, w.stats, N, 3, r.d.H, r.d.W, 7, s));
    ECG_TRY(bn_coef(r.bn, w.stats, ecg_stem_stats_only_rows(N, 3, r.d.H, r.d.W, 7), 64, (long)N * r.H1 * r.W1, params, 1,
                    buffers, 0, w.coef0, s));
    ECG_TRY(ecg_stem_pool_fwd(image, w.wstem, w.coef0, w.p0, w.idx0, N, 3, r.d.H, r.d.W, s));
  } else {
    ECG_TRY(stem_forward(dt, image, w.wstem, nullptr, w.y0, stats_rows ? w.stats : nullptr, N, 3, r.d.H, r.d.W, 7, s));
    ECG_TRY(bn_coef(r.bn, w.stats, stem_forward_rows(dt, N, 3, r.d.H, r.d.W, 7), 64, (long)N * r.H1 * r.W1, params, 1,
                    buffers, 0, w.coef0, s));
    ECG_TRY(ecg_bnrelu_maxpool(dt, w.y0, w.coef0, w.p0, w.idx0, N, r.H1, r.W1, 64, s));
  }

  ecg_tl_mark(101, s);
  const void* cur = w.p0;
  for (int i = 0; i < 8; ++i) {
    const Blk18& k = r.blk[i];
    BlockWs& b = w.b[i];
    const long M = (long)N * k.hout * k.wout;
    const int rows = ecg_conv_stats_rows(M);
    ConvGeom g1 = k.conv1_geom(N);
    ConvGeom g2 = k.conv2_geom(N);
    ConvEpi e1 = {}, e2 = {};
    e1.wg_rows = e2.wg_rows = 1;
    hipEvent_t down_done = nullptr;
    const bool down_side = k.down && side_fwd;
    if (down_side) {
      ConvGeom gd = k.down_geom(N);
      side_fork(s);
      ECG_TRY(ecg_conv_igemm(dt, 0, gd, cur, b.wdf, b.yd, nullptr, nullptr, stats_rows ? w.stats_d : nullptr, 0, g_side.s));
      ECG_TRY(bn_coef(r.bn, w.stats_d, rows, k.cout, M, params, k.p_dbn, buffers, k.b_dbn, b.coefd, g_side.s));
      down_done = side_mark();
    }
    ECG_TRY(ecg_conv_igemm(dt, 0, g1, cur, b.w1f, b.y1, nullptr, nullptr, stats_rows ? w.stats : nullptr, 0, s, &e1));
    ECG_TRY(bn_then_act(r, w.stats, e1.stats_rows, k.cout, M, params, k.p_bn1, buffers, k.b_bn1, b.coef1, b.y1, nullptr,
                        nullptr, b.a1, s));
    ECG_TRY(ecg_conv_igemm(dt, 0, g2, b.a1, b.w2f, b.y2, nullptr, nullptr, stats_rows ? w.stats : nullptr, 0, s, &e2));
    if (k.down) {
      if (down_side) {
        main_wait(s, down_done);
      } else {
        ConvGeom gd = k.down_geom(N);
        ECG_TRY(ecg_conv_igemm(dt, 0, gd, cur, b.wdf, b.yd, nullptr, nullptr, stats_rows ? w.stats_d : nullptr, 0, s));
        ECG_TRY(bn_coef(r.bn, w.stats_d, rows, k.cout, M, params, k.p_dbn, buffers, k.b_dbn, b.coefd, s));
      }
      ECG_TRY(bn_then_act(r, w.stats, e2.stats_rows, k.cout, M, params, k.p_bn2, buffers, k.b_bn2, b.coef2, b.y2, b.yd,
                          b.coefd, b.out, s, r.d.training && relu_bits_on() ? b.bits : nullptr));
    } else {
      ECG_TRY(bn_then_act(r, w.stats, e2.stats_rows, k.cout, M, params, k.p_bn2, buffers, k.b_bn2, b.coef2, b.y2, cur,
                          nullptr, b.out, s, r.d.training && relu_bits_on() ? b.bits : nullptr));
    }
    cur = b.out;
    ecg_tl_mark(102 + i, s);
  }
  const Blk18& last = r.blk[7];
  ECG_TRY(ecg_avgpool(dt, cur, w.pooled, N, last.hout * last.wout, 512, nullptr, s));
  ECG_TRY(ecg_linear_fwd(w.pooled, P(params, r.p_fc), P(params, r.p_fc + 1), feat_out, N, 512, r.d.out_dim, 0, nullptr,
                         s));
  ecg_tl_mark(110, s);
  return 0;
}

static int r18_backward(const ecgmm_resnet18_desc* d, const float* image, const float* dfeat, const void* const* params,
                        void* const* grads, void* ws_fwd, void* ws_bwd, size_t ws_bwd_bytes, int stage_begin, int stage_end,
                        float* dimage, hipStream_t s) {
  Net18 r;
  ECG_TRY(build(d, r));
  const bool train = r.d.training != 0;
  if (stem_recompute(r.d.dtype) && (dimage || !train))
    ECG_FAIL(ECGMM_ERR_SHAPE, "resnet18 bwd: %s needs the stored stem conv output; switch ecgmm_stem_recompute(0) "
             "(ECGMM_STEM_RECOMPUTE) off", dimage ? "the input gradient" : "an eval-mode backward");
  FwdWs w;
  layout_fwd(r, ws_fwd, w);
  BwdWs q;
  layout_bwd(r, ws_bwd, q);
  ECG_NEED(ws_fwd && ws_bwd, ws_bwd_bytes, q.bytes, "resnet18 bwd: workspace");
  const int dt = r.d.dtype, N = r.d.N;
  ECG_TRY(side_init());
  const bool side = g_side.enabled;
  ecg_conv_wgrad_narrow(side, N >= 192 ? 192 : 256);
  struct NarrowOff { ~NarrowOff() { ecg_conv_wgrad_narrow(false); } } narrow_off;
  hipStream_t ws = side ? g_side.s : s;

  if (stage_begin == 0) ecg_tl_mark(200, s);
  for (int st = stage_begin; st < stage_end; ++st) {
    if (st > 0) ecg_tl_mark(200 + st, s);
    if (st == 0) {
      g_side.doneA = g_side.doneB = g_side.doneC = nullptr;
      for (int a = 0; a < 3; ++a) g_side.done2[a][0] = g_side.done2[a][1] = nullptr;
      const Blk18& last = r.blk[7];
      ECG_TRY(fc_bwd(r, w, q, dfeat, params, grads, s));
      const int R = last.hout * last.wout;
      ECG_TRY(ecg_bcast_rows(dt, q.dpooled, q.X[0], N, R, 512, 1.f / (float)R, s));
    } else if (st <= 8) {
      const int i = 8 - st;
      const Blk18& k = r.blk[i];
      BlockWs& b = w.b[i];
      const void* in = i == 0 ? w.p0 : w.b[i - 1].out;
      const void* dcur = q.X[(st - 1) & 1];
      void* din = q.X[st & 1];
      const long M = (long)N * k.hout * k.wout;
      ConvGeom g1 = k.conv1_geom(N);
      ConvGeom g2 = k.conv2_geom(N);
      const int pp = st & 1;
      void *dyb = q.dy[pp], *dy1b = q.dy1[pp], *dydb = q.dyd[pp];
      bool fused2 = false;
      int fused2_rows = 0;
      const bool fuse_here = train && sw::BN_FUSE.get() && M >= sw::BN_FUSE_MIN_M.get();
      if (fuse_here && i + 1 < 8 && !r.blk[i + 1].down) {
        const Blk18& kn = r.blk[i + 1];
        const ConvGeom gn = kn.conv1_geom(N);
        fused2 = ecg_conv_halo_ok(dt, 1, gn);
        fused2_rows = fused2 ? ecg_conv_halo_rows(1, gn) : 0;
      }
      main_wait(s, g_side.done2[0][pp]);
      const void* dzp = q.dz;
      const bool dual = k.down && train && !fused2 && ecg_bn_dual_on() &&
                        ecg_bn_bwd_scratch(dt, M, k.cout) <= RED_ROWS_FLOATS * sizeof(float);
      if (dual) {
        main_wait(s, g_side.done2[2][pp]);
        ECG_TRY(ecg_bn_bwd_dual(dt, dcur, b.out, relu_bits_on() ? b.bits : nullptr, nullptr, nullptr, b.y2, b.coef2,
                                P(params, k.p_bn2), G(grads, k.p_bn2), G(grads, k.p_bn2 + 1), dyb, b.yd, b.coefd,
                                P(params, k.p_dbn), G(grads, k.p_dbn), G(grads, k.p_dbn + 1), dydb, q.dz, nullptr, M, k.cout,
                                q.bn_scratch, q.red2, s));
      } else if (fused2) {
        dzp = dcur;
        ECG_TRY(ecg_bn_bwd_tail(dt, dcur, nullptr, b.y2, b.coef2, P(params, k.p_bn2), G(grads, k.p_bn2),
                                G(grads, k.p_bn2 + 1), dyb, q.red2, fused2_rows, M, k.cout, q.bn_scratch, s));
      } else {
        ECG_TRY(bn_bwd_mode(r.bn, dcur, b.out, nullptr, nullptr, 1, b.y2, b.coef2, P(params, k.p_bn2), G(grads, k.p_bn2),
                            G(grads, k.p_bn2 + 1), dyb, q.dz, nullptr, M, k.cout, q.bn_scratch, s,
                            train && relu_bits_on() ? b.bits : nullptr));
      }
      if (G(grads, k.p_conv2)) {
        if (side) side_fork(s);
        ECG_TRY(ecg_conv_wgrad(dt, g2, b.a1, dyb, G(grads, k.p_conv2), 0, q.wg_ws, q.wg_bytes, ws));
        if (side) g_side.done2[0][pp] = side_mark();
      }
      ConvEpi ea = {};
      if (fuse_here) { ea.wg_rows = 1; ea.red_y = b.y1; ea.red_mask = b.y1; ea.red_coef = b.coef1; ea.red_rows = q.red1; }
      ECG_TRY(ecg_conv_igemm(dt, 1, g2, dyb, b.w2d, q.da, nullptr, nullptr, nullptr, 0, s, &ea));
      main_wait(s, g_side.done2[1][pp]);
      if (ea.red_done) {
        ECG_TRY(ecg_bn_bwd_tail(dt, q.da, b.y1, b.y1, b.coef1, P(params, k.p_bn1), G(grads, k.p_bn1),
                                G(grads, k.p_bn1 + 1), dy1b, q.red1, ea.red_rows_n, M, k.cout, q.bn_scratch, s));
      } else {
        ECG_TRY(bn_bwd_mode(r.bn, q.da, b.y1, nullptr, nullptr, 1, b.y1, b.coef1, P(params, k.p_bn1), G(grads, k.p_bn1),
                            G(grads, k.p_bn1 + 1), dy1b, nullptr, nullptr, M, k.cout, q.bn_scratch, s));
      }
      if (G(grads, k.p_conv1)) {
        if (side) side_fork(s);
        ECG_TRY(ecg_conv_wgrad(dt, g1, in, dy1b, G(grads, k.p_conv1), 0, q.wg_ws, q.wg_bytes, ws));
        if (side) g_side.done2[1][pp] = side_mark();
      }
      if (k.down) {
        ConvGeom gd = k.down_geom(N);
        if (!dual) {
          main_wait(s, g_side.done2[2][pp]);
          ECG_TRY(bn_bwd_mode(r.bn, dzp, nullptr, nullptr, nullptr, 1, b.yd, b.coefd, P(params, k.p_dbn), G(grads, k.p_dbn),
                              G(grads, k.p_dbn + 1), dydb, nullptr, nullptr, M, k.cout, q.bn_scratch, s));
        }
        if (G(grads, k.p_dconv)) {
          if (side) side_fork(s);
          ECG_TRY(ecg_conv_wgrad(dt, gd, in, dydb, G(grads, k.p_dconv), 0, q.wg_ws, q.wg_bytes, ws));
          if (side) g_side.done2[2][pp] = side_mark();
        }
        ConvEpi ed = {};
        ed.src2 = dydb; ed.wpk2 = b.wdd;
        if (!sw::DOWN_FOLD.get()) ed.src2 = nullptr;
        if (ed.src2) {
          ECG_TRY(ecg_conv_igemm(dt, 1, g1, dy1b, b.w1d, din, nullptr, nullptr, nullptr, 0, s, &ed));
        }
        if (!ed.src2_done) {
          ECG_TRY(ecg_conv_igemm(dt, 1, gd, dydb, b.wdd, q.dtmp, nullptr, nullptr, nullptr, 0, s));
          ECG_TRY(ecg_conv_igemm(dt, 1, g1, dy1b, b.w1d, din, nullptr, q.dtmp, nullptr, 0, s));
        }
      } else {
        ConvEpi eb = {};
        if (fuse_here && i > 0 && ecg_conv_halo_ok(dt, 1, g1)) {
          const BlockWs& pb = w.b[i - 1];
          eb.wg_rows = 1; eb.red_y = pb.y2; eb.red_mask = pb.out; eb.red_coef = pb.coef2; eb.red_rows = q.red2;
        }
        ECG_TRY(ecg_conv_igemm(dt, 1, g1, dy1b, b.w1d, din, nullptr, dzp, nullptr, 0, s, &eb));
      }
    } else if (st == 9) {
      const void* dp0 = q.X[8 & 1];
      if (stem_recompute(dt)) {
        ECG_TRY(ecg_stem_pool_bwd(image, w.wstem, w.coef0, P(params, 1), dp0, w.p0, w.idx0, G(grads, 1), G(grads, 2),
                                  G(grads, 0), q.stem_ws, q.stem_bytes, N, 3, r.d.H, r.d.W, s));
        continue;
      }
      if (train && ecg_stem_fuse_on()) {
        ECG_TRY(ecg_pool_bn_bwd(dt, dp0, w.p0, w.idx0, w.y0, w.coef0, P(params, 1), G(grads, 1), G(grads, 2), q.big1,
                                nullptr, N, r.H1, r.W1, 64, q.bn_scratch, s));
      } else {
        ECG_TRY(ecg_maxpool_relu_bwd(dt, dp0, w.p0, w.idx0, q.big0, N, r.H1, r.W1, 64, s));
        ECG_TRY(bn_bwd_mode(r.bn, q.big0, nullptr, nullptr, nullptr, 1, w.y0, w.coef0, P(params, 1), G(grads, 1), G(grads, 2),
                            q.big1, nullptr, nullptr, (long)N * r.H1 * r.W1, 64, q.bn_scratch, s));
      }
      if (G(grads, 0)) {
        ECG_TRY(ecg_stem_wgrad(dt, image, q.big1, G(grads, 0), 0, q.stem_ws, q.stem_bytes, N, 3, r.d.H, r.d.W, 7, s));
      }
      if (dimage) ECG_TRY(ecg_stem_dgrad(dt, q.big1, P(params, 0), dimage, N, 3, r.d.H, r.d.W, 7, s));
    } else {
      ECG_FAIL(ECGMM_ERR_SHAPE, "resnet18 bwd: stage %d out of range", st);
    }
  }
  if (stage_end == 10) ecg_tl_mark(210, s);
  if (side && !g_side.defer_join) {
    hipEvent_t e = side_next_ev();
    (void)hipEventRecord(e, g_side.s);
    (void)hipStreamWaitEvent(s, e, 0);
  }
  if (stage_end == 10) ecg_tl_mark(211, s);
  return 0;
}

extern "C" int ecgmm_resnet18_backward(const ecgmm_resnet18_desc* d, const float* image, const float* dfeat,
                                       const void* const* params, void* const* grads, void* ws_fwd, void* ws_bwd,
                                       size_t ws_bwd_bytes, int stage_begin, int stage_end, void* stream_) {
  return r18_backward(d, image, dfeat, params, grads, ws_fwd, ws_bwd, ws_bwd_bytes, stage_begin, stage_end, nullptr,
                      (hipStream_t)stream_);
}

extern "C" int ecgmm_resnet18_backward_dx(const ecgmm_resnet18_desc* d, const float* image, const float* dfeat,
                                          const void* const* params, void* const* grads, void* ws_fwd, void* ws_bwd,
                                          size_t ws_bwd_bytes, int stage_begin, int stage_end, float* dimage,
                                          void* stream_) {
  return r18_backward(d, image, dfeat, params, grads, ws_fwd, ws_bwd, ws_bwd_bytes, stage_begin, stage_end, dimage,
                      (hipStream_t)stream_);
}

extern "C" int ecgmm_resnet18_gradcam(const ecgmm_resnet18_desc* d, const float* dfeat, const void* const* params,
                                      void* ws_fwd, void* ws_bwd, size_t ws_bwd_bytes, float* cam, void* stream_) {
  hipStream_t s = (hipStream_t)stream_;
  Net18 r;
  ECG_TRY(build(d, r));
  FwdWs w;
  layout_fwd(r, ws_fwd, w);
  BwdWs q;
  layout_bwd(r, ws_bwd, q);
  ECG_NEED(ws_fwd && ws_bwd, ws_bwd_bytes, q.bytes, "resnet18 gradcam: workspace");
  if (!dfeat || !cam) ECG_FAIL(ECGMM_ERR_SHAPE, "resnet18 gradcam: null operand");
  ECG_TRY(fc_bwd(r, w, q, dfeat, params, nullptr, s));
  const Blk18& last = r.blk[7];
  return ecg_gradcam(r.d.dtype, w.b[7].out, q.dpooled, (float*)q.X[0], cam, r.d.N, last.hout, last.wout, 512, r.d.H, r.d.W,
                     s);
}
```

### ecg-multimodal-model_amd/csrc/plan_resnet1d.hip

```cpp
#include "plan_common.h"
#include "side_stream.h"

namespace {

int build(const ecgmm_resnet1d_desc* d, Net1D& r) {
  ECG_TRY(net1d_static(d, r, "resnet1d"));
  return net1d_shape(r, "resnet1d");
}

struct Fwd1 {
  void* wstem; void* y0; float* coef0; void* p0; unsigned char* idx0;
  BlockWs b[3];
  float *pooled, *h1, *hd;
  unsigned char* dmask;
  float* stats;
  size_t bytes;
};

void layout_fwd(const Net1D& r, void* base, Fwd1& w, WsTable* views = nullptr) {
  Arena a(base, views);
  const size_t es = dtype_size(r.d.dtype);
  const int N = r.d.N;
  w.wstem = a.take_bytes(ecg_stem_packed_elems(r.d.cin, 1) * es, "wstem");
  w.y0 = a.take_bytes((size_t)N * r.L1 * 64 * es, "y0");
// ... 98 lines not shown
  return ecg_linear_bwd(q.dh1, w.pooled, P(params, pc + T1_CLS_W1), q.dpooled, G(grads, pc + T1_CLS_W1),
                        G(grads, pc + T1_CLS_B1), N, 256, 64, q.lin_ws, q.lin_bytes, s);
}

}

static SideStream g_side1;
int ecg_resnet1d_side_enable(int on) {
  ECG_TRY(g_side1.init());
  g_side1.enabled = on != 0;
  return 0;
}
static bool g_side1_alone = true;
extern "C" int ecgmm_resnet1d_side_wgrad(int on) {
  g_side1_alone = on != 0;
  return 0;
}

extern "C" size_t ecgmm_resnet1d_fwd_workspace(const ecgmm_resnet1d_desc* d) {
  Net1D r;
  if (build(d, r)) return 0;
  Fwd1 w;
  layout_fwd(r, nullptr, w);
  return w.bytes;
}
extern "C" size_t ecgmm_resnet1d_bwd_workspace(const ecgmm_resnet1d_desc* d) {
  Net1D r;
  if (build(d, r)) return 0;
  Bwd1 w;
  layout_bwd(r, nullptr, w);
  return w.bytes;
}

extern "C" int ecgmm_resnet1d_ws_view(const ecgmm_resnet1d_desc* d, int backward, const char* name, int index,
                                      size_t* offset, size_t* bytes) {
  Net1D r;
  ECG_TRY(build(d, r));
  if (!name || !offset || !bytes) ECG_FAIL(ECGMM_ERR_SHAPE, "resnet1d ws_view: null argument");
  WsTable t;
  Fwd1 w;
  Bwd1 q;
  if (backward) layout_bwd(r, nullptr, q, &t);
  else layout_fwd(r, nullptr, w, &t);
  return ws_view_find(backward ? "resnet1d ws_view (backward)" : "resnet1d ws_view (forward)", t, name, index,
                      backward ? q.bytes : w.bytes, offset, bytes);
}

extern "C" int ecgmm_resnet1d_forward(const ecgmm_resnet1d_desc* d, const float* signal, const void* const* params,
                                      void* const* buffers, float* feat_out, void* ws, size_t ws_bytes,
                                      void* stream_) {
  hipStream_t s = (hipStream_t)stream_;
  Net1D r;
  ECG_TRY(build(d, r));
  Fwd1 w;
  layout_fwd(r, ws, w);
  ECG_NEED(ws, ws_bytes, w.bytes, "resnet1d fwd: workspace");
  const int dt = r.d.dtype, N = r.d.N, cin = r.d.cin;
  float* st = r.d.training ? w.stats : nullptr;

  {
    EcgPackItem items[ECG_PACK_MAX];
    int n = 0;
    for (int i = 0; i < 3; ++i) {
      const Blk1& k = r.blk[i];
      BlockWs& b = w.b[i];
      items[n++] = {P(params, k.p0 + T1_CONV1_W), b.w1f, b.w1d, k.cout, k.cin, 3};
      items[n++] = {P(params, k.p0 + T1_CONV2_W), b.w2f, b.w2d, k.cout, k.cout, 3};
      if (k.down) items[n++] = {P(params, k.p0 + T1_DOWN_W), b.wdf, b.wdd, k.cout, k.cin, 1};
    }
    ECG_TRY(ecg_pack_weight_batch(dt, items, n, s));
  }
  ECG_TRY(ecg_stem_pack(dt, P(params, 0), w.wstem, cin, 1, s));
  ECG_TRY(stem_forward(dt, signal, w.wstem, P(params, 1), w.y0, st, N, cin, 1, r.d.L, 1, s));
  ECG_TRY(bn_coef(r.bn, w.stats, stem_forward_rows(dt, N, cin, 1, r.d.L, 1), 64, (long)N * r.L1, params, 2, buffers, 0,
                  w.coef0, s));
  ECG_TRY(ecg_bnrelu_maxpool(dt, w.y0, w.coef0, w.p0, w.idx0, N, 1, r.L1, 64, s));

  const void* cur = w.p0;
  for (int i = 0; i < 3; ++i) {
    const Blk1& k = r.blk[i];
    BlockWs& b = w.b[i];
    const int p = k.p0, bb = k.b0;
    const long M = (long)N * k.lout;
    const int rows = ecg_conv_stats_rows(M);
    ConvGeom g1 = k.conv1_geom(N);
    ConvGeom g2 = k.conv2_geom(N);
    ECG_TRY(ecg_conv_igemm(dt, 0, g1, cur, b.w1f, b.y1, P(params, p + T1_CONV1_B), nullptr, st, 0, s));
    ECG_TRY(bn_coef(r.bn, w.stats, rows, k.cout, M, params, p + T1_BN1, buffers, bb + T1B_BN1, b.coef1, s));
    ECG_TRY(ecg_bn_act(dt, b.y1, b.coef1, nullptr, nullptr, nullptr, 1, 1, b.a1, M, k.cout, s));
    ECG_TRY(ecg_conv_igemm(dt, 0, g2, b.a1, b.w2f, b.y2, P(params, p + T1_CONV2_B), nullptr, st, 0, s));
    ECG_TRY(bn_coef(r.bn, w.stats, rows, k.cout, M, params, p + T1_BN2, buffers, bb + T1B_BN2, b.coef2, s));
    ECG_TRY(ecg_avgpool(dt, b.y2, b.m, N, k.lout, k.cout, b.coef2, s));
    ECG_TRY(se_mlp_forward(b.m, P(params, p + T1_SE_W1), P(params, p + T1_SE_B1), P(params, p + T1_SE_W2),
                           P(params, p + T1_SE_B2), b.h, b.g, N, k.cout, k.cr, s));
    if (k.down) {
      ConvGeom gd = k.down_geom(N);
      ECG_TRY(ecg_conv_igemm(dt, 0, gd, cur, b.wdf, b.yd, P(params, p + T1_DOWN_B), nullptr, st, 0, s));
      ECG_TRY(bn_coef(r.bn, w.stats, rows, k.cout, M, params, p + T1_DBN, buffers, bb + T1B_DBN, b.coefd, s));
      ECG_TRY(ecg_bn_act(dt, b.y2, b.coef2, b.yd, b.coefd, b.g, k.lout, 1, b.out, M, k.cout, s));
    } else {
      ECG_TRY(ecg_bn_act(dt, b.y2, b.coef2, cur, nullptr, b.g, k.lout, 1, b.out, M, k.cout, s));
    }
    cur = b.out;
  }
  const int pc = r.p_cls;
  ECG_TRY(ecg_avgpool(dt, cur, w.pooled, N, r.blk[2].lout, 256, nullptr, s));
  ECG_TRY(ecg_linear_fwd(w.pooled, P(params, pc + T1_CLS_W1), P(params, pc + T1_CLS_B1), w.h1, N, 256, 64, ECGMM_ACT_RELU,
                         nullptr, s));
  const float* hin = w.h1;
  if (r.d.training && r.d.dropout_p > 0.f) {
    ECG_TRY(ecg_dropout_fwd(w.h1, w.hd, w.dmask, (long)N * 64, r.d.dropout_p, r.d.seed, r.d.offset, s));
    hin = w.hd;
  }
  ECG_TRY(ecg_linear_fwd(hin, P(params, pc + T1_CLS_W2), P(params, pc + T1_CLS_B2), feat_out, N, 64, r.d.num_classes, 0,
                         nullptr, s));
  return 0;
}

static int r1d_backward(const ecgmm_resnet1d_desc* d, const float* signal, const float* dfeat, const void* const* params,
                        void* const* grads, void* ws_fwd, void* ws_bwd, size_t ws_bwd_bytes, int stage_begin, int stage_end,
                        float* dsignal, hipStream_t s) {
  Net1D r;
  ECG_TRY(build(d, r));
  const bool train = r.d.training != 0;
  Fwd1 w;
  layout_fwd(r, ws_fwd, w);
  Bwd1 q;
  layout_bwd(r, ws_bwd, q);
  ECG_NEED(ws_fwd && ws_bwd, ws_bwd_bytes, q.bytes, "resnet1d bwd: workspace");
  const int dt = r.d.dtype, N = r.d.N, cin = r.d.cin;
  ECG_TRY(g_side1.init());
  const bool side = g_side1.enabled && g_side1_alone;
  ecg_conv_wgrad_narrow(side);
  struct NarrowOff { ~NarrowOff() { ecg_conv_wgrad_narrow(false); } } narrow_off;
  hipStream_t wst = side ? g_side1.s : s;

  for (int st = stage_begin; st < stage_end; ++st) {
    if (st == 0) {
      g_side1.doneA = g_side1.doneB = g_side1.doneC = nullptr;
      ECG_TRY(classifier_bwd(r, w, q, dfeat, params, grads, s));
      const int R = r.blk[2].lout;
      ECG_TRY(ecg_bcast_rows(dt, q.dpooled, q.X[0], N, R, 256, 1.f / (float)R, s));
    } else if (st <= 3) {
      const int i = 3 - st;
      const Blk1& k = r.blk[i];
      BlockWs& b = w.b[i];
      const int p = k.p0;
      const void* in = i == 0 ? w.p0 : w.b[i - 1].out;
      const void* dcur = q.X[(st - 1) & 1];
      void* din = q.X[st & 1];
      const long M = (long)N * k.lout;
      ConvGeom g1 = k.conv1_geom(N);
      ConvGeom g2 = k.conv2_geom(N);
      const bool se_merge = sw::SE_MERGE.get() && train;
      if (se_merge) {
        ECG_TRY(ecg_se_gate_bn(dt, dcur, b.out, b.y2, b.coef2, q.dz, q.dg, q.sa1, q.sa2, q.sa3, N, k.lout, k.cout, s));
      } else {
        ECG_TRY(ecg_se_gate_grad(dt, dcur, b.out, b.y2, b.coef2, q.dg, N, k.lout, k.cout, s));
      }
      if (ecg_se_mlp_fused_ok(k.cout, k.cr)) {
        ECG_TRY(ecg_se_mlp_bwd(q.dg, b.g, b.h, b.m, P(params, p + T1_SE_W1), P(params, p + T1_SE_W2), q.ds, q.dh, q.dm,
                               G(grads, p + T1_SE_W1), G(grads, p + T1_SE_B1), G(grads, p + T1_SE_W2), G(grads, p + T1_SE_B2),
                               N, k.cout, k.cr, 1.f / (float)k.lout, s));
      } else {
        ECG_TRY(ecg_act_bwd(q.dg, b.g, q.ds, (long)N * k.cout, ECGMM_ACT_SIGMOID, s));
        ECG_TRY(ecg_linear_bwd(q.ds, b.h, P(params, p + T1_SE_W2), q.dh, G(grads, p + T1_SE_W2), G(grads, p + T1_SE_B2), N,
                               k.cr, k.cout, q.lin_ws, q.lin_bytes, s));
        ECG_TRY(ecg_act_bwd(q.dh, b.h, q.dh, (long)N * k.cr, ECGMM_ACT_RELU, s));
        ECG_TRY(ecg_linear_bwd(q.dh, b.m, P(params, p + T1_SE_W1), q.dm, G(grads, p + T1_SE_W1), G(grads, p + T1_SE_B1), N,
                               k.cout, k.cr, q.lin_ws, q.lin_bytes, s));
        ECG_TRY(ecg_axpby(1.f / (float)k.lout, q.dm, 0.f, q.dm, (long)N * k.cout, s));
      }
      main_wait(s, g_side1.doneA);
      if (se_merge) {
        ECG_TRY(ecg_se_bn_rows(q.sa1, q.sa2, q.sa3, b.g, q.dm, N, k.lout, k.cout, q.se_rows, s));
        ECG_TRY(ecg_bn_bwd_tail(dt, q.dz, nullptr, b.y2, b.coef2, P(params, p + T1_BN2), G(grads, p + T1_BN2),
                                G(grads, p + T1_BN2 + 1), q.dy, q.se_rows, ecg_se_bn_nrows(), M, k.cout, q.bn_scratch, s, b.g,
                                q.dm, k.lout, G(grads, p + T1_CONV2_B)));
      } else {
        ECG_TRY(bn_bwd_mode(r.bn, dcur, b.out, b.g, q.dm, k.lout, b.y2, b.coef2, P(params, p + T1_BN2), G(grads, p + T1_BN2),
                            G(grads, p + T1_BN2 + 1), q.dy, q.dz, G(grads, p + T1_CONV2_B), M, k.cout, q.bn_scratch, s));
      }
      if (G(grads, p + T1_CONV2_W)) {
        if (side) g_side1.fork(s);
        ECG_TRY(ecg_conv_wgrad(dt, g2, b.a1, q.dy, G(grads, p + T1_CONV2_W), 0, q.wg_ws, q.wg_bytes, wst));
        if (side) g_side1.doneA = g_side1.mark();
      }
      ECG_TRY(ecg_conv_igemm(dt, 1, g2, q.dy, b.w2d, q.da, nullptr, nullptr, nullptr, 0, s));
      main_wait(s, g_side1.doneB);
      ECG_TRY(bn_bwd_mode(r.bn, q.da, b.y1 , nullptr, nullptr, 1, b.y1, b.coef1,
                          P(params, p + T1_BN1), G(grads, p + T1_BN1), G(grads, p + T1_BN1 + 1), q.dy1, nullptr,
                          G(grads, p + T1_CONV1_B), M, k.cout, q.bn_scratch, s));
      if (G(grads, p + T1_CONV1_W)) {
        if (side) g_side1.fork(s);
        ECG_TRY(ecg_conv_wgrad(dt, g1, in, q.dy1, G(grads, p + T1_CONV1_W), 0, q.wg_ws, q.wg_bytes, wst));
        if (side) g_side1.doneB = g_side1.mark();
      }
      if (k.down) {
        ConvGeom gd = k.down_geom(N);
        main_wait(s, g_side1.doneC);
        ECG_TRY(bn_bwd_mode(r.bn, q.dz, nullptr, nullptr, nullptr, 1, b.yd, b.coefd, P(params, p + T1_DBN),
                            G(grads, p + T1_DBN), G(grads, p + T1_DBN + 1), q.dyd, nullptr, G(grads, p + T1_DOWN_B), M, k.cout,
                            q.bn_scratch, s));
        if (G(grads, p + T1_DOWN_W)) {
          if (side) g_side1.fork(s);
          ECG_TRY(ecg_conv_wgrad(dt, gd, in, q.dyd, G(grads, p + T1_DOWN_W), 0, q.wg_ws, q.wg_bytes, wst));
          if (side) g_side1.doneC = g_side1.mark();
        }
        ConvEpi ed = {};
        if (sw::DOWN_FOLD.get()) { ed.src2 = q.dyd; ed.wpk2 = b.wdd; }
        if (ed.src2) ECG_TRY(ecg_conv_igemm(dt, 1, g1, q.dy1, b.w1d, din, nullptr, nullptr, nullptr, 0, s, &ed));
        if (!ed.src2_done) {
          ECG_TRY(ecg_conv_igemm(dt, 1, gd, q.dyd, b.wdd, q.dtmp, nullptr, nullptr, nullptr, 0, s));
          ECG_TRY(ecg_conv_igemm(dt, 1, g1, q.dy1, b.w1d, din, nullptr, q.dtmp, nullptr, 0, s));
        }
      } else {
        ECG_TRY(ecg_conv_igemm(dt, 1, g1, q.dy1, b.w1d, din, nullptr, q.dz, nullptr, 0, s));
      }
    } else if (st == 4) {
      const void* dp0 = q.X[3 & 1];
      if (train && ecg_stem_fuse_on()) {
        ECG_TRY(ecg_pool_bn_bwd(dt, dp0, w.p0, w.idx0, w.y0, w.coef0, P(params, 2), G(grads, 2), G(grads, 3), q.big1,
                                G(grads, 1), N, 1, r.L1, 64, q.bn_scratch, s));
      } else {
        ECG_TRY(ecg_maxpool_relu_bwd(dt, dp0, w.p0, w.idx0, q.big0, N, 1, r.L1, 64, s));
        ECG_TRY(bn_bwd_mode(r.bn, q.big0, nullptr, nullptr, nullptr, 1, w.y0, w.coef0, P(params, 2), G(grads, 2), G(grads, 3),
                            q.big1, nullptr, G(grads, 1), (long)N * r.L1, 64, q.bn_scratch, s));
      }
      if (G(grads, 0))
        ECG_TRY(ecg_stem_wgrad(dt, signal, q.big1, G(grads, 0), 0, q.stem_ws, q.stem_bytes, N, cin, 1, r.d.L, 1, s));
      if (dsignal) ECG_TRY(ecg_stem_dgrad(dt, q.big1, P(params, 0), dsignal, N, cin, 1, r.d.L, 1, s));
    } else {
      ECG_FAIL(ECGMM_ERR_SHAPE, "resnet1d bwd: stage %d out of range", st);
    }
  }
  if (side) ECG_TRY(g_side1.wait_on(s));
  return 0;
}

extern "C" int ecgmm_resnet1d_backward(const ecgmm_resnet1d_desc* d, const float* signal, const float* dfeat,
                                       const void* const* params, void* const* grads, void* ws_fwd, void* ws_bwd,
                                       size_t ws_bwd_bytes, int stage_begin, int stage_end, void* stream_) {
  return r1d_backward(d, signal, dfeat, params, grads, ws_fwd, ws_bwd, ws_bwd_bytes, stage_begin, stage_end, nullptr,
                      (hipStream_t)stream_);
}

extern "C" int ecgmm_resnet1d_backward_dx(const ecgmm_resnet1d_desc* d, const float* signal, const float* dfeat,
                                          const void* const* params, void* const* grads, void* ws_fwd, void* ws_bwd,
                                          size_t ws_bwd_bytes, int stage_begin, int stage_end, float* dsignal,
                                          void* stream_) {
  return r1d_backward(d, signal, dfeat, params, grads, ws_fwd, ws_bwd, ws_bwd_bytes, stage_begin, stage_end, dsignal,
                      (hipStream_t)stream_);
}

extern "C" int ecgmm_resnet1d_gradcam(const ecgmm_resnet1d_desc* d, const float* dfeat, const void* const* params,
                                      void* ws_fwd, void* ws_bwd, size_t ws_bwd_bytes, float* cam, void* stream_) {
  hipStream_t s = (hipStream_t)stream_;
  Net1D r;
  ECG_TRY(build(d, r));
  Fwd1 w;
  layout_fwd(r, ws_fwd, w);
  Bwd1 q;
  layout_bwd(r, ws_bwd, q);
  ECG_NEED(ws_fwd && ws_bwd, ws_bwd_bytes, q.bytes, "resnet1d gradcam: workspace");
  if (!dfeat || !cam) ECG_FAIL(ECGMM_ERR_SHAPE, "resnet1d gradcam: null operand");
  ECG_TRY(classifier_bwd(r, w, q, dfeat, params, nullptr, s));
  return ecg_gradcam(r.d.dtype, w.b[2].out, q.dpooled, (float*)q.X[0], cam, r.d.N, 1, r.blk[2].lout, 256, 1, r.d.L, s);
}
```

### ecg-multimodal-model_amd/csrc/switches.h

```cpp
#pragma once
#include <limits.h>

#include "common.h"

struct Switch {
  enum Kind {
    ON,
    OFF,
    LEVEL,
    INT
  };
  const char* env;
  Kind kind;
  long def;
  long hi, neg;
  bool runtime;
  const char* doc;
  long v = LONG_MIN;

  long clamp(long x) const {
    if (kind == LEVEL) return x < 0 ? 0 : x > hi ? hi : x;
    if (kind == INT) return x < 0 ? neg : x;
    return x != 0;
  }
  long from_env() const {
    if (kind == ON) return env_on(env);
    if (kind == OFF) return env_off(env);
    if (kind == LEVEL) return env_level(env, (int)hi, (int)def);
    return clamp(env_int(env, def));
  }
  long get() {
    if (v == LONG_MIN) v = from_env();
    return v;
  }
  void set(long x) { v = clamp(x); }
};

namespace sw {
constexpr long NEVER = 1L << 40;
inline Switch CONV_HALO      {"ECGMM_CONV_HALO",       Switch::LEVEL, 1,     2, 0,     true,  "halo-resident conv kernel: 0 = never, 1 = where it is faster, 2 = wherever applicable"};
inline Switch HALO_CUS       {"ECGMM_HALO_CUS",        Switch::INT,   0,     0, 0,     true,  "cap on the CUs (persistent workgroups) of a halo-kernel launch; 0 or negative = all"};
inline Switch HALO_W4        {"ECGMM_HALO_W4",         Switch::OFF,   0,     0, 0,     true,  "64 -> 64 channel 3x3 tiles on 4-wave workgroups, two per CU"};
inline Switch HALO_STAGGER   {"ECGMM_HALO_STAGGER",    Switch::ON,    1,     0, 0,     true,  "waves 4-7 run a step's first MFMA block behind its barrier (0: lock step); bit-identical"};
inline Switch HALO_STREAM    {"ECGMM_HALO_STREAM",     Switch::ON,    1,     0, 0,     true,  "stream form of the 64 -> 64 channel 3x3 tiles (0: one tile at a time); bit-identical"};
inline Switch HALO_PP        {"ECGMM_HALO_PP",         Switch::ON,    1,     0, 0,     true,  "ping-pong K loop on the 128-channel 3x3 tiles (0: lock step); bit-identical"};
inline Switch HALO_NCS1      {"ECGMM_HALO_NCS1",       Switch::ON,    1,     0, 0,     false, "64-channel 3x3 layers prefetch the next tile's halo during the K loop"};
inline Switch WGRAD_RING     {"ECGMM_WGRAD_RING",      Switch::LEVEL, 1,     2, 0,     true,  "ring weight-gradient kernel: 0 = never, 1 = where it is faster, 2 = wherever applicable"};
inline Switch WGRAD_PP       {"ECGMM_WGRAD_PP",        Switch::OFF,   0,     0, 0,     true,  "ping-pong between the two wave groups of the ring weight gradient; bit-identical"};
inline Switch WGRAD_GROUPS   {"ECGMM_WGRAD_GROUPS",    Switch::OFF,   0,     0, 0,     false, "1 = 256-thread weight-gradient workgroups instead of two 4-wave groups sharing a slab tile"};
inline Switch WGRAD_WGS      {"ECGMM_WGRAD_WGS",       Switch::INT,   0,     0, 0,     false, "four-wave slots of a weight-gradient launch; 0 or negative = 512 alone, the plan's choice on the side stream"};
inline Switch BN_FOLD        {"ECGMM_BN_FOLD",         Switch::ON,    1,     0, 0,     true,  "BatchNorm finalize folded into its consumer pass (0: separate launches)"};
inline Switch BN_FOLD_SLICE  {"ECGMM_BN_FOLD_SLICE",   Switch::ON,    1,     0, 0,     true,  "folded passes at C >= 256 as (pixel chunk, 128-channel slice) workgroups; bit-identical"};
inline Switch BN_FUSE        {"ECGMM_BN_FUSE",         Switch::ON,    1,     0, 0,     false, "0 = BatchNorm-backward reductions always as their own pass, whatever the threshold"};
inline Switch BN_FUSE_MIN_M  {"ECGMM_BN_FUSE_MIN_M",   Switch::INT,   NEVER, 0, NEVER, true,  "pixel count from which a BatchNorm-backward reduction is fused into the producing dgrad; negative = never"};
inline Switch RELU_BITS      {"ECGMM_RELU_BITS",       Switch::ON,    1,     0, 0,     false, "bn2's backward reads the ReLU mask as bits the forward wrote (forward and backward must agree)"};
inline Switch STEM_FUSE      {"ECGMM_STEM_FUSE",       Switch::ON,    1,     0, 0,     false, "stem backward as one pool + BatchNorm pass (0: max-pool backward + full BatchNorm backward)"};
inline Switch STEM_RECOMPUTE {"ECGMM_STEM_RECOMPUTE",  Switch::OFF,   0,     0, 0,     true,  "image stem by recompute, without its full-resolution conv output (changes the workspace layouts)"};
inline Switch DOWN_FOLD      {"ECGMM_DOWN_FOLD",       Switch::ON,    1,     0, 0,     false, "downsample branch's input gradient folded into the stride-2 dgrad (0: own launch + addend)"};
inline Switch DOWN_SIDE      {"ECGMM_DOWN_SIDE",       Switch::ON,    1,     0, 0,     false, "downsample branch of the training forward on the side stream (0: the caller's stream)"};
inline Switch SIDE_WGRAD     {"ECGMM_SIDE_WGRAD",      Switch::ON,    1,     0, 0,     false, "initial state of each plan's weight-gradient side stream; per plan at run time: ecgmm_side_wgrad()"};
inline Switch INFER_DOWN_SIDE{"ECGMM_INFER_DOWN_SIDE", Switch::OFF,   0,     0, 0,     true,  "downsample convolution of the inference plans on a side stream beside conv1"};
inline Switch SE_MERGE       {"ECGMM_SE_MERGE",        Switch::ON,    1,     0, 0,     false, "ResNet1D_SE backward: SE-gate gradient and bn2's reduction in one pass (0: two passes)"};
inline Switch SE_MLP_FUSED   {"ECGMM_SE_MLP_FUSED",    Switch::ON,    1,     0, 0,     false, "the SE MLP as fused kernels (0: per-op launches)"};
inline Switch HEAD_FUSED     {"ECGMM_HEAD_FUSED",      Switch::ON,    1,     0, 0,     false, "fusion head on the row kernels of head_fused.hip (0: ~45 per-op launches)"};
inline Switch DENSE16        {"ECGMM_DENSE16",         Switch::ON,    1,     0, 0,     false, "batch-sized Linear layers on dense16_kernel (0: the implicit-GEMM route)"};

inline Switch* const ALL[] = {
    &CONV_HALO,  &HALO_CUS,      &HALO_W4,       &HALO_STAGGER, &HALO_STREAM,   &HALO_PP,   &HALO_NCS1,  &WGRAD_RING,      &WGRAD_PP,
    &WGRAD_GROUPS, &WGRAD_WGS,   &BN_FOLD,       &BN_FOLD_SLICE, &BN_FUSE,      &BN_FUSE_MIN_M, &RELU_BITS, &STEM_FUSE,    &STEM_RECOMPUTE,
    &DOWN_FOLD,  &DOWN_SIDE,     &SIDE_WGRAD,    &INFER_DOWN_SIDE, &SE_MERGE,   &SE_MLP_FUSED, &HEAD_FUSED, &DENSE16};
constexpr int COUNT = (int)(sizeof(ALL) / sizeof(ALL[0]));

inline Switch* find(const char* env) {
  for (Switch* s : ALL)
    if (env && strcmp(s->env, env) == 0) return s;
  return nullptr;
}
}
```

### ecg-multimodal-model_amd/hip/lib.py

```python
import ctypes as C
import os

F32, BF16 = 0, 1
ACT_NONE, ACT_RELU, ACT_SIGMOID = 0, 1, 2
RESNET18_NPARAMS, RESNET18_NBUFFERS = 62, 60
RESNET1D_NPARAMS, RESNET1D_NBUFFERS = 52, 27

_PKG_DIR = os.path.dirname(os.path.dirname(os.path.abspath(__file__)))
LIB_PATH = os.environ.get("ECGMM_LIB") or os.path.join(_PKG_DIR, "libecgmm_hip.so")

vp, i32, i64, u64, f32, f64, sz = C.c_void_p, C.c_int, C.c_int64, C.c_uint64, C.c_float, C.c_double, C.c_size_t


class ConvDesc(C.Structure):
    _fields_ = [(n, i32) for n in ("N", "H", "W", "Cin", "Cout", "R", "S", "stride", "pad_h", "pad_w")]


class ResNet18Desc(C.Structure):
    _fields_ = [("N", i32), ("H", i32), ("W", i32), ("out_dim", i32), ("dtype", i32), ("training", i32),
                ("bn_momentum", f32), ("bn_eps", f32)]


class ResNet1DDesc(C.Structure):
    _fields_ = [("N", i32), ("cin", i32), ("L", i32), ("num_classes", i32), ("dtype", i32), ("training", i32),
                ("bn_momentum", f32), ("bn_eps", f32), ("dropout_p", f32), ("seed", u64), ("offset", u64)]


class HeadDesc(C.Structure):
    _fields_ = [("B", i32), ("dim", i32 * 3), ("hidden", i32), ("num_classes", i32), ("training", i32),
                ("ln_eps", f32), ("dropout_p", f32), ("seed", u64), ("offset", u64)]


class LSTMDesc(C.Structure):
    _fields_ = [(n, i32) for n in ("B", "T", "In", "H", "layers", "bidirectional", "batch_first", "save_for_backward")]


class MHADesc(C.Structure):
    _fields_ = [(n, i32) for n in ("S", "N", "heads", "head_dim", "batch_first")] + [("p_drop", f32)]


class CRNNFrontDesc(C.Structure):
    _fields_ = [("B", i32), ("F", i32), ("T", i32), ("dtype", i32), ("training", i32), ("bn_momentum", f32), ("bn_eps", f32)]


class TransformerInferDesc(C.Structure):
    _fields_ = [(n, i32) for n in ("B", "L", "input_dim", "E", "heads", "ff", "layers", "classes", "batch_first")] + [("eps", f32)]


class TabNetInferDesc(C.Structure):
    _fields_ = [(n, i32) for n in ("input_dim", "n_d", "n_a", "n_steps", "n_shared", "n_independent", "out_dim")] + \
               [("gamma", f32), ("epsilon", f32), ("bn_eps", f32)]


P = C.POINTER
SIGNATURES = {
    "ecgmm_version": (i32, []),
    "ecgmm_last_error": (C.c_char_p, []),
    "ecgmm_switch_name": (C.c_char_p, [i32]),
    "ecgmm_switch_get": (i32, [C.c_char_p, P(i64)]),
    "ecgmm_switch_set": (i32, [C.c_char_p, i64]),
    "ecgmm_resnet18_fwd_workspace": (sz, [P(ResNet18Desc)]),
    "ecgmm_resnet18_bwd_workspace": (sz, [P(ResNet18Desc)]),
    "ecgmm_resnet18_forward": (i32, [P(ResNet18Desc), vp, P(vp), P(vp), vp, vp, sz, vp]),
    "ecgmm_resnet18_backward": (i32, [P(ResNet18Desc), vp, vp, P(vp), P(vp), vp, vp, sz, i32, i32, vp]),
    "ecgmm_resnet18_backward_dx": (i32, [P(ResNet18Desc), vp, vp, P(vp), P(vp), vp, vp, sz, i32, i32, vp, vp]),
    "ecgmm_resnet18_gradcam": (i32, [P(ResNet18Desc), vp, P(vp), vp, vp, sz, vp, vp]),
    "ecgmm_resnet18_ws_view": (i32, [P(ResNet18Desc), i32, C.c_char_p, i32, P(sz), P(sz)]),
    "ecgmm_head_fwd_workspace": (sz, [P(HeadDesc)]),
    "ecgmm_head_bwd_workspace": (sz, [P(HeadDesc)]),
    "ecgmm_head_forward": (i32, [P(HeadDesc), P(vp), P(vp), P(vp), vp, vp, vp, sz, vp]),
    "ecgmm_head_backward": (i32, [P(HeadDesc), P(vp), P(vp), P(vp), P(vp), vp, P(vp), vp, vp, sz, vp]),
    "ecgmm_conv_halo_enable": (i32, [i32]),
    "ecgmm_conv_halo_cus": (i32, [i32]),
    "ecgmm_conv_halo_w4": (i32, [i32]),
    "ecgmm_conv_halo_stagger": (i32, [i32]),
    "ecgmm_conv_halo_stream": (i32, [i32]),
    "ecgmm_conv_halo_pingpong": (i32, [i32]),
    "ecgmm_conv_wgrad_pingpong": (i32, [i32]),
    "ecgmm_conv_wgrad_ring_enable": (i32, [i32]),
    "ecgmm_side_wgrad": (i32, [i32]),
    "ecgmm_side_defer_join": (i32, [i32]),
    "ecgmm_resnet1d_side_wgrad": (i32, [i32]),
    "ecgmm_side_wait": (i32, [vp]),
    "ecgmm_side_stream": (vp, []),
    "ecgmm_side_fork": (i32, [vp]),
    "ecgmm_resnet1d_fwd_workspace": (sz, [P(ResNet1DDesc)]),
    "ecgmm_resnet1d_bwd_workspace": (sz, [P(ResNet1DDesc)]),
    "ecgmm_resnet1d_forward": (i32, [P(ResNet1DDesc), vp, P(vp), P(vp), vp, vp, sz, vp]),
    "ecgmm_resnet1d_backward": (i32, [P(ResNet1DDesc), vp, vp, P(vp), P(vp), vp, vp, sz, i32, i32, vp]),
    "ecgmm_resnet1d_backward_dx": (i32, [P(ResNet1DDesc), vp, vp, P(vp), P(vp), vp, vp, sz, i32, i32, vp, vp]),
    "ecgmm_resnet1d_gradcam": (i32, [P(ResNet1DDesc), vp, P(vp), vp, vp, sz, vp, vp]),
    "ecgmm_resnet1d_ws_view": (i32, [P(ResNet1DDesc), i32, C.c_char_p, i32, P(sz), P(sz)]),
    "ecgmm_nchw_to_nhwc": (i32, [i32, vp, vp, i32, i32, i64, vp]),
    "ecgmm_nhwc_to_nchw": (i32, [i32, vp, vp, i32, i32, i64, vp]),
    "ecgmm_cast": (i32, [i32, vp, vp, i64, vp]),
    "ecgmm_uncast": (i32, [i32, vp, vp, i64, vp]),
    "ecgmm_pack_conv_weight": (i32, [i32, vp, vp, vp, i32, i32, i32, vp]),
    "ecgmm_conv_stats_rows": (i32, [i64]),
    "ecgmm_conv_fwd": (i32, [i32, P(ConvDesc), vp, vp, vp, vp, vp, i32, vp]),
    "ecgmm_conv_fwd_wgrows": (i32, [i32, P(ConvDesc), vp, vp, vp, vp, vp, vp, i32, vp]),
    "ecgmm_conv_bwd_data": (i32, [i32, P(ConvDesc), vp, vp, vp, vp, vp]),
    "ecgmm_conv_bwd_weight_workspace": (sz, [i32, P(ConvDesc)]),
    "ecgmm_conv_bwd_weight": (i32, [i32, P(ConvDesc), vp, vp, vp, i32, vp, sz, vp]),
    "ecgmm_stem_packed_elems": (sz, [i32, i32]),
    "ecgmm_stem_stats_rows": (i32, [i32, i32, i32, i32, i32]),
    "ecgmm_stem_pack": (i32, [i32, vp, vp, i32, i32, vp]),
    "ecgmm_stem_fwd": (i32, [i32, vp, vp, vp, vp, vp, i32, i32, i32, i32, i32, vp]),
    "ecgmm_stem_wg_stats_rows": (i32, [i32, i32, i32, i32, i32]),
    "ecgmm_stem_fwd_wgrows": (i32, [i32, vp, vp, vp, vp, vp, i32, i32, i32, i32, i32, vp]),
    "ecgmm_stem_stats_only_rows": (i32, [i32, i32, i32, i32, i32]),
    "ecgmm_stem_stats_only": (i32, [i32, vp, vp, vp, vp, i32, i32, i32, i32, i32, vp]),
    "ecgmm_stem_pool_fwd": (i32, [vp, vp, vp, vp, vp, i32, i32, i32, i32, vp]),
    "ecgmm_stem_pool_bwd_workspace": (sz, [i32, i32, i32, i32]),
    "ecgmm_stem_pool_bwd": (i32, [vp, vp, vp, vp, vp, vp, vp, vp, vp, vp, vp, sz, i32, i32, i32, i32, vp]),
    "ecgmm_stem_bwd_weight_workspace": (sz, [i32, i32, i32, i32, i32]),
    "ecgmm_stem_bwd_weight": (i32, [i32, vp, vp, vp, i32, vp, sz, i32, i32, i32, i32, i32, vp]),
    "ecgmm_stem_bwd_data": (i32, [i32, vp, vp, vp, i32, i32, i32, i32, i32, vp]),
    "ecgmm_col_stats_rows": (i32, [i32, i64, i32]),
    "ecgmm_col_stats": (i32, [i32, vp, i64, i32, vp, vp]),
    "ecgmm_bn_finalize": (i32, [vp, i32, i32, f64, vp, vp, vp, vp, vp, f32, f32, vp, vp]),
    "ecgmm_bn_eval_coef": (i32, [i32, vp, vp, vp, vp, f32, vp, vp]),
    "ecgmm_bn_act": (i32, [i32, vp, vp, vp, vp, vp, i32, i32, vp, i64, i32, vp]),
    "ecgmm_bn_act_from_rows": (i32, [i32, vp, vp, i32, f64, vp, vp, vp, vp, vp, f32, f32, vp, vp, vp, vp, i32, i32, vp, i64, i32, vp]),
    "ecgmm_bn_bwd_scratch": (sz, [i32, i64, i32]),
    "ecgmm_bn_bwd": (i32, [i32, vp, vp, vp, vp, i32, vp, vp, vp, vp, vp, vp, vp, vp, i64, i32, vp, vp]),
    "ecgmm_bn_eval_bwd": (i32, [i32, vp, vp, vp, vp, i32, vp, vp, vp, vp, vp, vp, vp, i64, i32, vp, vp]),
    "ecgmm_conv_bwd_data_with_downsample": (i32, [i32, P(ConvDesc), vp, vp, vp, vp, vp, vp, vp]),
    "ecgmm_conv_bwd_data_bnred": (i32, [i32, P(ConvDesc), vp, vp, vp, vp, vp, vp, vp, vp, P(i32), vp]),
    "ecgmm_conv_bwd_data_bnred_rows": (i32, [i32, P(ConvDesc)]),
    "ecgmm_bn_bwd_from_rows": (i32, [i32, vp, vp, vp, vp, vp, vp, vp, vp, vp, i32, i64, i32, vp, vp]),
    "ecgmm_bnrelu_maxpool": (i32, [i32, vp, vp, vp, vp, i32, i32, i32, i32, vp]),
    "ecgmm_maxpool_relu_bwd": (i32, [i32, vp, vp, vp, vp, i32, i32, i32, i32, vp]),
    "ecgmm_bn_fuse_min_pixels": (i32, [i64]),
    "ecgmm_bn_fold": (i32, [i32]),
    "ecgmm_bn_fold_slice": (i32, [i32]),
    "ecgmm_bn_act_from_rows_bits": (i32, [i32, vp, vp, i32, f64, vp, vp, vp, vp, vp, f32, f32, vp, vp, vp, vp, i32, i32, vp, vp, i64, i32, vp]),
    "ecgmm_bn_bwd_bits": (i32, [i32, vp, vp, vp, vp, i32, vp, vp, vp, vp, vp, vp, vp, vp, i64, i32, vp, vp]),
    "ecgmm_bn_bwd_dual": (i32, [i32] + [vp] * 19 + [i64, i32, vp, vp, vp]),
    "ecgmm_bn_dual": (i32, [i32]),
    "ecgmm_tl_enable": (i32, [i32]),
    "ecgmm_tl_mark": (i32, [i32, vp]),
    "ecgmm_tl_collect": (i32, [i32, vp, vp]),
    "ecgmm_stem_recompute": (i32, [i32]),
    "ecgmm_pool_bn_bwd": (i32, [i32, vp, vp, vp, vp, vp, vp, vp, vp, vp, vp, i32, i32, i32, i32, vp, vp]),
    "ecgmm_avgpool": (i32, [i32, vp, vp, i32, i32, i32, vp, vp]),
    "ecgmm_bcast_rows": (i32, [i32, vp, vp, i32, i32, i32, f32, vp]),
    "ecgmm_se_gate_grad": (i32, [i32, vp, vp, vp, vp, vp, i32, i32, i32, vp]),
    "ecgmm_se_gate_bn": (i32, [i32, vp, vp, vp, vp, vp, vp, vp, vp, vp, i32, i32, i32, vp]),
    "ecgmm_se_mlp_fwd": (i32, [vp, vp, vp, vp, vp, vp, vp, i32, i32, i32, vp]),
    "ecgmm_se_mlp_bwd": (i32, [vp, vp, vp, vp, vp, vp, vp, vp, vp, vp, vp, vp, vp, i32, i32, i32, f32, vp]),
    "ecgmm_linear_fwd": (i32, [vp, vp, vp, vp, i32, i32, i32, i32, vp]),
    "ecgmm_linear_bwd_scratch": (sz, [i32, i32, i32]),
    "ecgmm_linear_bwd": (i32, [vp, vp, vp, vp, vp, vp, i32, i32, i32, vp, sz, vp]),
    "ecgmm_act_bwd": (i32, [vp, vp, vp, i64, i32, vp]),
    "ecgmm_layernorm_fwd": (i32, [P(vp), P(i32), i32, vp, vp, vp, vp, vp, vp, i32, f32, vp]),
    "ecgmm_layernorm_bwd_scratch": (sz, [i32, i32]),
    "ecgmm_layernorm_bwd": (i32, [P(vp), P(i32), i32, vp, vp, vp, vp, P(vp), i32, vp, vp, vp, i32, vp, vp]),
    "ecgmm_varloss_fwd": (i32, [vp, vp, vp, i32, i32, i32, i32, vp, vp, vp]),
    "ecgmm_varloss_bwd": (i32, [vp, i32, i32, vp, vp, i32, vp, i32, vp]),
    "ecgmm_ce_fwd": (i32, [vp, vp, i32, i32, i32, f32, f32, vp, vp, vp]),
    "ecgmm_ce_bwd": (i32, [vp, vp, i32, i32, vp, vp, vp, vp]),
    "ecgmm_ce_plus_fwd": (i32, [vp, vp, i32, i32, vp, f32, vp, vp, vp]),
    "ecgmm_ce_plus_bwd": (i32, [vp, vp, i32, i32, vp, vp, vp, vp, f32, vp]),
    "ecgmm_dropout_fwd": (i32, [vp, vp, vp, i64, f32, u64, u64, vp]),
    "ecgmm_dropout_bwd": (i32, [vp, vp, vp, i64, f32, vp]),
    "ecgmm_adam": (i32, [vp, vp, vp, vp, i64, f32, f32, f32, f32, f32, i64, f32, vp]),
    "ecgmm_axpby": (i32, [f32, vp, f32, vp, i64, vp]),
    "ecgmm_signal_preprocess_workspace": (sz, [i32, i32, i32]),
    "ecgmm_signal_preprocess": (i32, [vp, vp, i32, i32, vp, vp, i32, P(f64), P(f64), P(f64), i32, vp, sz, vp]),
    "ecgmm_signal_preprocess_i16": (i32, [vp, i32, i32, i32, P(i32), i32, vp, vp, i32, vp, i32, i32, P(f64), P(f64), P(f64),
                                          i32, vp]),
    "ecgmm_weighted_sample": (i32, [vp, i64, i64, vp, vp, i64, u64, u64, vp]),
    "ecgmm_signal_filter_zscore": (i32, [vp, vp, i32, i32, P(f64), P(f64), P(f64), i32, i32, f64, vp]),
    "ecgmm_signal_filter_lanes": (i32, [P(f64), i32, i32]),
    "ecgmm_signal_resample_len": (i32, [i32, f64]),
    "ecgmm_signal_resample_workspace": (sz, [i32, i32, i32]),
    "ecgmm_signal_resample": (i32, [vp, i32, i32, vp, i32, f64, vp, i32, vp, vp, sz, vp]),
    "ecgmm_signal_gather_augment": (i32, [vp, i64, i32, vp, i32, vp, vp, i32, f32, f32, f32, f32, i32, i32, u64, u64, vp]),
    "ecgmm_glu_fwd": (i32, [vp, vp, i64, i32, vp]),
    "ecgmm_glu_bwd": (i32, [vp, vp, vp, i64, i32, vp]),
    "ecgmm_sparsemax_fwd": (i32, [vp, vp, i64, i32, vp]),
    "ecgmm_sparsemax_bwd": (i32, [vp, vp, vp, i64, i32, vp]),
    "ecgmm_ew": (i32, [i32, vp, vp, vp, i64, f32, vp]),
    "ecgmm_split_cols": (i32, [vp, vp, vp, i64, i32, i32, i32, vp]),
    "ecgmm_split_cols_bwd": (i32, [vp, vp, vp, vp, i64, i32, i32, i32, vp]),
    "ecgmm_bn_small_fwd": (i32, [vp, vp, vp, vp, vp, vp, vp, vp, i32, i32, i32, f32, f32, vp]),
    "ecgmm_bn_small_bwd": (i32, [vp, vp, vp, vp, vp, vp, vp, i32, i32, i32, vp]),
    "ecgmm_bn_small_eval_bwd": (i32, [vp, vp, vp, vp, vp, vp, vp, i32, i32, i32, vp]),
    "ecgmm_entropy_fwd": (i32, [vp, vp, i64, i32, f32, vp]),
    "ecgmm_entropy_bwd": (i32, [vp, vp, vp, i64, i32, f32, vp]),
    "ecgmm_image_resize_tables_bytes": (sz, [i32, i32, i32, i32]),
    "ecgmm_image_resize_tables": (i32, [i32, i32, i32, i32, vp, sz]),
    "ecgmm_image_transform": (i32, [vp, vp, i32, i32, i32, i32, i32, vp, sz, P(f32), P(f32), vp]),
    "ecgmm_resnet18_infer_prepared_bytes": (sz, [P(ResNet18Desc)]),
    "ecgmm_resnet18_infer_prepare": (i32, [P(ResNet18Desc), P(vp), P(vp), vp, sz, vp]),
    "ecgmm_resnet18_infer_workspace": (sz, [P(ResNet18Desc)]),
    "ecgmm_resnet18_infer": (i32, [P(ResNet18Desc), vp, vp, sz, vp, vp, sz, vp]),
    "ecgmm_resnet1d_infer_prepared_bytes": (sz, [P(ResNet1DDesc)]),
    "ecgmm_resnet1d_infer_prepare": (i32, [P(ResNet1DDesc), P(vp), P(vp), vp, sz, vp]),
    "ecgmm_resnet1d_infer_workspace": (sz, [P(ResNet1DDesc)]),
    "ecgmm_resnet1d_infer": (i32, [P(ResNet1DDesc), vp, vp, sz, vp, vp, sz, vp]),
    "ecgmm_infer_down_side": (i32, [i32]),
    "ecgmm_conv_fwd_fused": (i32, [i32, P(ConvDesc), vp, vp, vp, vp, vp, i32, vp]),
    "ecgmm_fold_conv_bn": (i32, [i32, i32, vp, vp, vp, vp, vp, vp, f32, vp, vp, vp, i32, i32, i32, vp]),
    "ecgmm_relu_maxpool": (i32, [i32, vp, vp, i32, i32, i32, i32, vp]),
    "ecgmm_gate_res_relu": (i32, [i32, vp, vp, vp, vp, i64, i32, i32, vp]),
    "ecgmm_prof_enable": (i32, [i32]),
    "ecgmm_prof_pause": (i32, [i32]),
    "ecgmm_prof_collect": (i32, [i32, P(f64), P(f64), P(f64), P(i64)]),
    "ecgmm_lstm_fwd_workspace": (sz, [P(LSTMDesc)]),
    "ecgmm_lstm_bwd_workspace": (sz, [P(LSTMDesc)]),
    "ecgmm_lstm_forward": (i32, [P(LSTMDesc), vp, P(vp), vp, vp, vp, vp, vp, vp, sz, vp]),
    "ecgmm_lstm_backward": (i32, [P(LSTMDesc), vp, P(vp), vp, vp, vp, vp, vp, vp, vp, P(vp), vp, vp, vp, sz, vp]),
    "ecgmm_lstm_forward_varlen": (i32, [P(LSTMDesc), vp, vp, P(vp), vp, vp, vp, vp, vp, vp, sz, vp]),
    "ecgmm_lstm_backward_varlen": (i32, [P(LSTMDesc), vp, vp, P(vp), vp, vp, vp, vp, vp, vp, vp, P(vp), vp, vp, vp, sz,
                                         vp]),
    "ecgmm_seq_mean_varlen_fwd": (i32, [vp, vp, vp, i32, i32, i32, vp]),
    "ecgmm_seq_mean_varlen_bwd": (i32, [vp, vp, vp, i32, i32, i32, vp]),
    "ecgmm_conv5_in1_stats_rows": (i32, [i32, i32, i32]),
    "ecgmm_conv5_in1_fwd": (i32, [i32, vp, vp, vp, vp, vp, i32, i32, i32, vp]),
    "ecgmm_conv5_in1_bwd_weight_workspace": (sz, [i32, i32, i32]),
    "ecgmm_conv5_in1_bwd_weight": (i32, [i32, vp, vp, vp, vp, i32, vp, sz, i32, i32, i32, vp]),
    "ecgmm_conv5_bwd_weight_workspace": (sz, [i32, P(ConvDesc)]),
    "ecgmm_conv5_bwd_weight": (i32, [i32, P(ConvDesc), vp, vp, vp, i32, vp, sz, vp]),
    "ecgmm_bnrelu_maxpool2": (i32, [i32, vp, vp, vp, vp, i32, i32, i32, i32, i32, vp]),
    "ecgmm_pool2_bn_bwd_workspace": (sz, [i32, i32, i32, i32]),
    "ecgmm_pool2_bn_bwd": (i32, [i32, vp, vp, vp, vp, i32, vp, vp, vp, vp, i32, i32, i32, i32, i32, vp, sz, vp]),
    "ecgmm_crnn_front_fwd_workspace": (sz, [P(CRNNFrontDesc)]),
    "ecgmm_crnn_front_bwd_workspace": (sz, [P(CRNNFrontDesc)]),
    "ecgmm_crnn_front_forward": (i32, [P(CRNNFrontDesc), vp, P(vp), P(vp), vp, vp, sz, vp]),
    "ecgmm_crnn_front_backward": (i32, [P(CRNNFrontDesc), vp, vp, P(vp), P(vp), vp, vp, sz, vp]),
    "ecgmm_crnn_front_backward_dx": (i32, [P(CRNNFrontDesc), vp, vp, P(vp), P(vp), vp, vp, sz, vp, vp]),
    "ecgmm_conv5_in1_bwd_data": (i32, [i32, vp, vp, vp, i32, i32, i32, vp]),
    "ecgmm_conv5_in1_bwd_data_tile": (None, [i32, P(i32), P(i32), P(i32)]),
    "ecgmm_crnn_gradcam_workspace": (sz, [i32, i32, i32, i32]),
    "ecgmm_crnn_gradcam": (i32, [vp, vp, vp, vp, vp, sz, vp, i32, i32, i32, i32, i32, i32, vp]),
    "ecgmm_relu_maxpool2": (i32, [i32, vp, vp, i32, i32, i32, i32, i32, vp]),
    "ecgmm_conv5_in1_relu_pool2": (i32, [i32, vp, vp, vp, vp, i32, i32, i32, vp]),
    "ecgmm_fold_conv5_bn": (i32, [i32, i32, vp, vp, vp, vp, vp, vp, f32, vp, vp, vp, i32, i32, vp]),
    "ecgmm_crnn_front_infer_prepared_bytes": (sz, [P(CRNNFrontDesc)]),
    "ecgmm_crnn_front_infer_prepare": (i32, [P(CRNNFrontDesc), P(vp), P(vp), vp, sz, vp]),
    "ecgmm_crnn_front_infer_workspace": (sz, [P(CRNNFrontDesc)]),
    "ecgmm_crnn_front_infer": (i32, [P(CRNNFrontDesc), vp, vp, sz, vp, vp, sz, vp]),
    "ecgmm_log_spectrogram_frames": (i32, [i32, i32, i32]),
    "ecgmm_log_spectrogram": (i32, [vp, i32, i32, vp, i32, i32, vp, i32, vp]),
    "ecgmm_lime_perturb": (i32, [vp, vp, vp, vp, vp, vp, i32, i32, i32, i32, i32, u64, u64, vp, vp, vp, vp, vp]),
    "ecgmm_lime_ridge_workspace": (sz, [i32, i32, i32]),
    "ecgmm_lime_ridge": (i32, [vp, vp, vp, vp, i32, i32, i32, i32, i32, f64, f64, vp, vp, vp, vp, vp, vp, sz, vp]),
    "ecgmm_lime_prob": (i32, [vp, i64, i32, i32, vp, i64, vp]),
    "ecgmm_shap_mlp_workspace": (sz, [i32, i32, i32, i32, i32]),
    "ecgmm_shap_gradient": (i32, [vp, vp, vp, vp, vp, vp, vp, i32, i32, i32, i32, i32, i32, vp, vp, vp, vp, sz, vp]),
    "ecgmm_shap_deep": (i32, [vp, vp, vp, vp, vp, i32, i32, i32, i32, i32, vp, vp, vp, vp, sz, vp]),
    "ecgmm_mha_bwd_workspace": (sz, [P(MHADesc)]),
    "ecgmm_mha_forward": (i32, [P(MHADesc), vp, vp, vp, u64, u64, vp]),
    "ecgmm_mha_backward": (i32, [P(MHADesc), vp, vp, vp, vp, vp, vp, sz, u64, u64, vp]),
    "ecgmm_mha_keep_mask": (i32, [P(MHADesc), vp, u64, u64, vp]),
    "ecgmm_mha_forward_varlen": (i32, [P(MHADesc), vp, vp, vp, vp, u64, u64, vp]),
    "ecgmm_mha_backward_varlen": (i32, [P(MHADesc), vp, vp, vp, vp, vp, vp, vp, sz, u64, u64, vp]),
    "ecgmm_mha_weights": (i32, [P(MHADesc), vp, vp, vp, vp, i32, vp]),
    "ecgmm_mha_rollout_step": (i32, [P(MHADesc), vp, vp, vp, vp, vp, f32, vp]),
    "ecgmm_embed1d_fwd": (i32, [vp, vp, vp, vp, vp, i32, i32, i32, i32, vp]),
    "ecgmm_embed1d_bwd_workspace": (sz, [i32, i32, i32, i32]),
    "ecgmm_embed1d_bwd": (i32, [vp, vp, vp, vp, vp, vp, vp, i32, i32, i32, i32, i32, vp, sz, vp]),
    "ecgmm_linear_res_ln": (i32, [vp, vp, vp, vp, vp, vp, vp, i64, i32, i32, f32, vp]),
    "ecgmm_ffn_res_ln": (i32, [vp, vp, vp, vp, vp, vp, vp, vp, i64, i32, i32, f32, vp]),
    "ecgmm_transformer_infer_prepared_bytes": (sz, [P(TransformerInferDesc)]),
    "ecgmm_transformer_infer_prepare": (i32, [P(TransformerInferDesc), P(vp), vp, sz, vp]),
    "ecgmm_transformer_infer_workspace": (sz, [P(TransformerInferDesc)]),
    "ecgmm_transformer_infer": (i32, [P(TransformerInferDesc), vp, vp, vp, sz, vp, vp, sz, vp]),
    "ecgmm_tabnet_infer_prepared_bytes": (sz, [P(TabNetInferDesc)]),
    "ecgmm_tabnet_infer_prepare": (i32, [P(TabNetInferDesc), P(vp), vp, sz, vp]),
    "ecgmm_tabnet_infer": (i32, [P(TabNetInferDesc), vp, i64, vp, sz, vp, vp, vp, vp, vp]),
}

LATER_SYMBOLS = ("ecgmm_resnet18_backward_dx", "ecgmm_resnet18_gradcam", "ecgmm_resnet1d_backward_dx",
                 "ecgmm_resnet1d_gradcam", "ecgmm_stem_bwd_data", "ecgmm_bn_eval_bwd", "ecgmm_bn_small_eval_bwd",
                 "ecgmm_resnet18_infer_prepared_bytes", "ecgmm_resnet18_infer_prepare", "ecgmm_resnet18_infer_workspace",
                 "ecgmm_resnet18_infer", "ecgmm_resnet1d_infer_prepared_bytes", "ecgmm_resnet1d_infer_prepare",
                 "ecgmm_resnet1d_infer_workspace", "ecgmm_resnet1d_infer", "ecgmm_infer_down_side", "ecgmm_conv_fwd_fused",
                 "ecgmm_fold_conv_bn", "ecgmm_relu_maxpool", "ecgmm_gate_res_relu",
                 "ecgmm_signal_filter_zscore", "ecgmm_signal_gather_augment",
                 "ecgmm_lstm_fwd_workspace", "ecgmm_lstm_bwd_workspace", "ecgmm_lstm_forward", "ecgmm_lstm_backward",
                 "ecgmm_conv5_in1_stats_rows", "ecgmm_conv5_in1_fwd", "ecgmm_conv5_in1_bwd_weight_workspace",
                 "ecgmm_conv5_in1_bwd_weight", "ecgmm_conv5_bwd_weight_workspace", "ecgmm_conv5_bwd_weight",
                 "ecgmm_bnrelu_maxpool2", "ecgmm_pool2_bn_bwd_workspace", "ecgmm_pool2_bn_bwd",
                 "ecgmm_crnn_front_fwd_workspace", "ecgmm_crnn_front_bwd_workspace", "ecgmm_crnn_front_forward",
                 "ecgmm_crnn_front_backward",
                 "ecgmm_switch_name", "ecgmm_switch_get", "ecgmm_switch_set",
                 "ecgmm_log_spectrogram_frames", "ecgmm_log_spectrogram",
                 "ecgmm_se_mlp_fwd", "ecgmm_se_mlp_bwd",
                 "ecgmm_signal_preprocess_i16", "ecgmm_weighted_sample",
                 "ecgmm_resnet18_ws_view", "ecgmm_resnet1d_ws_view",
                 "ecgmm_lime_perturb", "ecgmm_lime_ridge_workspace", "ecgmm_lime_ridge", "ecgmm_lime_prob",
                 "ecgmm_shap_mlp_workspace", "ecgmm_shap_gradient", "ecgmm_shap_deep",
                 "ecgmm_bn_bwd_dual", "ecgmm_bn_dual",
                 "ecgmm_mha_bwd_workspace", "ecgmm_mha_forward", "ecgmm_mha_backward", "ecgmm_mha_keep_mask",
                 "ecgmm_embed1d_fwd", "ecgmm_embed1d_bwd_workspace", "ecgmm_embed1d_bwd",
                 "ecgmm_se_gate_bn",
                 "ecgmm_lstm_forward_varlen", "ecgmm_lstm_backward_varlen", "ecgmm_seq_mean_varlen_fwd",
                 "ecgmm_seq_mean_varlen_bwd",
                 "ecgmm_signal_filter_lanes",
                 "ecgmm_mha_forward_varlen", "ecgmm_mha_backward_varlen",
                 "ecgmm_mha_weights", "ecgmm_mha_rollout_step",
                 "ecgmm_crnn_front_backward_dx", "ecgmm_conv5_in1_bwd_data", "ecgmm_conv5_in1_bwd_data_tile",
                 "ecgmm_crnn_gradcam_workspace", "ecgmm_crnn_gradcam",
                 "ecgmm_signal_resample_len", "ecgmm_signal_resample_workspace", "ecgmm_signal_resample",
                 "ecgmm_relu_maxpool2", "ecgmm_conv5_in1_relu_pool2", "ecgmm_fold_conv5_bn",
                 "ecgmm_crnn_front_infer_prepared_bytes", "ecgmm_crnn_front_infer_prepare",
                 "ecgmm_crnn_front_infer_workspace", "ecgmm_crnn_front_infer",
                 "ecgmm_linear_res_ln", "ecgmm_ffn_res_ln", "ecgmm_transformer_infer_prepared_bytes",
                 "ecgmm_transformer_infer_prepare", "ecgmm_transformer_infer_workspace", "ecgmm_transformer_infer",
                 "ecgmm_tabnet_infer_prepared_bytes", "ecgmm_tabnet_infer_prepare", "ecgmm_tabnet_infer")

_lib = None


def _missing(name):
    def fail(*_a):
        raise RuntimeError(f"{LIB_PATH} does not export {name}: rebuild the HIP library (there is no fallback)")
    return fail


def lib():
    global _lib
    if _lib is None:
        if not os.path.exists(LIB_PATH):
            raise RuntimeError(
                f"libecgmm_hip.so not found at {LIB_PATH}: the HIP extension is the only compute path "
                "(no CPU fallback). Build it with `python __graft_entry__.py` or "
                "`make -C ecg-multimodal-model_amd/csrc`.")
        import torch
        h = C.CDLL(LIB_PATH)
        for name, (res, args) in SIGNATURES.items():
            if name in LATER_SYMBOLS and os.environ.get("ECGMM_LIB") and not hasattr(h, name):
                setattr(h, name, _missing(name))
                continue
            fn = getattr(h, name)
            fn.restype, fn.argtypes = res, args
        if h.ecgmm_version() != 100:
            raise RuntimeError(f"libecgmm_hip.so version {h.ecgmm_version()} != 100 (stale build?)")
        _lib = h
    return _lib


def check(rc, what=""):
    if rc != 0:
        msg = lib().ecgmm_last_error().decode(errors="replace")
        raise RuntimeError(f"ecgmm {what} failed (code {rc}): {msg}")
```

### include/ecgmm.h

```cpp
#ifndef ECGMM_H
#define ECGMM_H
#include <stddef.h>
#include <stdint.h>

#ifdef __cplusplus
extern "C" {
#endif

#define ECGMM_VERSION 100

enum { ECGMM_F32 = 0, ECGMM_BF16 = 1 };
enum { ECGMM_ACT_NONE = 0, ECGMM_ACT_RELU = 1, ECGMM_ACT_SIGMOID = 2 };
enum {
  ECGMM_OK = 0,
  ECGMM_ERR_SHAPE = 1,
  ECGMM_ERR_DTYPE = 2,
  ECGMM_ERR_WORKSPACE = 3,
  ECGMM_ERR_LAUNCH = 4
};

int ecgmm_version(void);
const char* ecgmm_last_error(void);

const char* ecgmm_switch_name(int i);
int ecgmm_switch_get(const char* env_name, int64_t* value);
int ecgmm_switch_set(const char* env_name, int64_t value);

#define ECGMM_RESNET18_NPARAMS 62
#define ECGMM_RESNET18_NBUFFERS 60
typedef struct {
  int N, H, W;
  int out_dim;
  int dtype;
  int training;
  float bn_momentum, bn_eps;
} ecgmm_resnet18_desc;

size_t ecgmm_resnet18_fwd_workspace(const ecgmm_resnet18_desc* d);
size_t ecgmm_resnet18_bwd_workspace(const ecgmm_resnet18_desc* d);
int ecgmm_resnet18_forward(const ecgmm_resnet18_desc* d, const float* image, const void* const* params,
                           void* const* buffers, float* feat_out, void* ws, size_t ws_bytes, void* stream);
int ecgmm_resnet18_backward(const ecgmm_resnet18_desc* d, const float* image, const float* dfeat,
                            const void* const* params, void* const* grads, void* ws_fwd, void* ws_bwd,
                            size_t ws_bwd_bytes, int stage_begin, int stage_end, void* stream);
int ecgmm_resnet18_backward_dx(const ecgmm_resnet18_desc* d, const float* image, const float* dfeat,
                               const void* const* params, void* const* grads, void* ws_fwd, void* ws_bwd,
                               size_t ws_bwd_bytes, int stage_begin, int stage_end, float* dimage, void* stream);
int ecgmm_resnet18_gradcam(const ecgmm_resnet18_desc* d, const float* dfeat, const void* const* params, void* ws_fwd,
                           void* ws_bwd, size_t ws_bwd_bytes, float* cam, void* stream);
int ecgmm_resnet18_ws_view(const ecgmm_resnet18_desc* d, int backward, const char* name, int index, size_t* offset,
                           size_t* bytes);

int ecgmm_side_wgrad(int on);
int ecgmm_side_defer_join(int defer);
int ecgmm_resnet1d_side_wgrad(int on);
int ecgmm_side_wait(void* stream);
void* ecgmm_side_stream(void);
int ecgmm_side_fork(void* stream);

#define ECGMM_RESNET1D_NPARAMS 52
#define ECGMM_RESNET1D_NBUFFERS 27
typedef struct {
  int N, cin, L;
  int num_classes;
  int dtype;
  int training;
  float bn_momentum, bn_eps;
  float dropout_p;
  uint64_t seed, offset;
} ecgmm_resnet1d_desc;

size_t ecgmm_resnet1d_fwd_workspace(const ecgmm_resnet1d_desc* d);
size_t ecgmm_resnet1d_bwd_workspace(const ecgmm_resnet1d_desc* d);
int ecgmm_resnet1d_forward(const ecgmm_resnet1d_desc* d, const float* signal, const void* const* params,
                           void* const* buffers, float* feat_out, void* ws, size_t ws_bytes, void* stream);
int ecgmm_resnet1d_backward(const ecgmm_resnet1d_desc* d, const float* signal, const float* dfeat,
                            const void* const* params, void* const* grads, void* ws_fwd, void* ws_bwd,
                            size_t ws_bwd_bytes, int stage_begin, int stage_end, void* stream);
int ecgmm_resnet1d_backward_dx(const ecgmm_resnet1d_desc* d, const float* signal, const float* dfeat,
                               const void* const* params, void* const* grads, void* ws_fwd, void* ws_bwd,
                               size_t ws_bwd_bytes, int stage_begin, int stage_end, float* dsignal, void* stream);
int ecgmm_resnet1d_gradcam(const ecgmm_resnet1d_desc* d, const float* dfeat, const void* const* params, void* ws_fwd,
                           void* ws_bwd, size_t ws_bwd_bytes, float* cam, void* stream);
int ecgmm_resnet1d_ws_view(const ecgmm_resnet1d_desc* d, int backward, const char* name, int index, size_t* offset,
                           size_t* bytes);

size_t ecgmm_resnet18_infer_prepared_bytes(const ecgmm_resnet18_desc* d);
int ecgmm_resnet18_infer_prepare(const ecgmm_resnet18_desc* d, const void* const* params, const void* const* buffers,
                                 void* blob, size_t blob_bytes, void* stream);
size_t ecgmm_resnet18_infer_workspace(const ecgmm_resnet18_desc* d);
int ecgmm_resnet18_infer(const ecgmm_resnet18_desc* d, const float* image, const void* blob, size_t blob_bytes,
                         float* feat_out, void* ws, size_t ws_bytes, void* stream);
size_t ecgmm_resnet1d_infer_prepared_bytes(const ecgmm_resnet1d_desc* d);
int ecgmm_resnet1d_infer_prepare(const ecgmm_resnet1d_desc* d, const void* const* params, const void* const* buffers,
                                 void* blob, size_t blob_bytes, void* stream);
size_t ecgmm_resnet1d_infer_workspace(const ecgmm_resnet1d_desc* d);
int ecgmm_resnet1d_infer(const ecgmm_resnet1d_desc* d, const float* signal, const void* blob, size_t blob_bytes,
                         float* feat_out, void* ws, size_t ws_bytes, void* stream);
int ecgmm_infer_down_side(int on);

#define ECGMM_HEAD_NPARAMS 19
typedef struct {
  int B;
  int dim[3];
  int hidden;
  int num_classes;
  int training;
  float ln_eps;
  float dropout_p;
  uint64_t seed, offset;
} ecgmm_head_desc;
size_t ecgmm_head_fwd_workspace(const ecgmm_head_desc* d);
size_t ecgmm_head_bwd_workspace(const ecgmm_head_desc* d);
int ecgmm_head_forward(const ecgmm_head_desc* d, const float* const* raw, const void* const* params,
                       float* const* logits, float* var_loss, float* soft_w, void* ws, size_t ws_bytes, void* stream);
int ecgmm_head_backward(const ecgmm_head_desc* d, const float* const* raw, const void* const* params,
                        void* const* grads, const float* const* dlogits, const float* dvar, float* const* draw,
                        void* ws_fwd, void* ws_bwd, size_t ws_bwd_bytes, void* stream);

typedef struct {
  int N, H, W, Cin, Cout, R, S, stride, pad_h, pad_w;
} ecgmm_conv_desc;

int ecgmm_nchw_to_nhwc(int dtype, const float* src, void* dst, int N, int C, int64_t HW, void* stream);
int ecgmm_nhwc_to_nchw(int dtype, const void* src, float* dst, int N, int C, int64_t HW, void* stream);
int ecgmm_cast(int dtype, const float* src, void* dst, int64_t n, void* stream);
int ecgmm_uncast(int dtype, const void* src, float* dst, int64_t n, void* stream);
int ecgmm_pack_conv_weight(int dtype, const float* w_oihw, void* fwd, void* dgrad, int Cout, int Cin, int RS,
                           void* stream);

int ecgmm_conv_stats_rows(int64_t out_pixels);
int ecgmm_conv_halo_enable(int on);
int ecgmm_conv_halo_cus(int cus);
int ecgmm_conv_halo_w4(int on);
int ecgmm_conv_halo_stagger(int on);
int ecgmm_conv_halo_stream(int on);
int ecgmm_conv_halo_pingpong(int on);
int ecgmm_conv_wgrad_pingpong(int on);
int ecgmm_conv_wgrad_ring_enable(int on);
int ecgmm_conv_fwd(int dtype, const ecgmm_conv_desc* c, const void* x, const void* w_fwd, const float* bias, void* y,
                   float* stats, int act, void* stream);
int ecgmm_conv_fwd_wgrows(int dtype, const ecgmm_conv_desc* c, const void* x, const void* w_fwd, const float* bias, void* y,
                          float* stats, int* nrows, int act, void* stream);
int ecgmm_conv_bwd_data(int dtype, const ecgmm_conv_desc* c, const void* dy, const void* w_dgrad, const void* addend,
                        void* dx, void* stream);
size_t ecgmm_conv_bwd_weight_workspace(int dtype, const ecgmm_conv_desc* c);
int ecgmm_conv_bwd_weight(int dtype, const ecgmm_conv_desc* c, const void* x, const void* dy, float* dw_oihw,
                          int accumulate, void* ws, size_t ws_bytes, void* stream);

size_t ecgmm_stem_packed_elems(int Cin, int R);
int ecgmm_stem_stats_rows(int N, int Cin, int H, int W, int R);
int ecgmm_stem_pack(int dtype, const float* w_oihw, void* packed, int Cin, int R, void* stream);
int ecgmm_stem_fwd(int dtype, const float* x, const void* packed, const float* bias, void* y, float* stats, int N,
                   int Cin, int H, int W, int R, void* stream);
int ecgmm_stem_wg_stats_rows(int N, int Cin, int H, int W, int R);
int ecgmm_stem_fwd_wgrows(int dtype, const float* x, const void* packed, const float* bias, void* y, float* stats, int N,
                          int Cin, int H, int W, int R, void* stream);
size_t ecgmm_stem_bwd_weight_workspace(int N, int Cin, int H, int W, int R);
int ecgmm_stem_bwd_weight(int dtype, const float* x, const void* dy, float* dw_oihw, int accumulate, void* ws,
                          size_t ws_bytes, int N, int Cin, int H, int W, int R, void* stream);
int ecgmm_stem_bwd_data(int dtype, const void* dy, const float* w_oihw, float* dx, int N, int Cin, int H, int W, int R,
                        void* stream);

int ecgmm_stem_stats_only_rows(int N, int Cin, int H, int W, int R);
int ecgmm_stem_stats_only(int dtype, const float* x, const void* packed, const float* bias, float* stats, int N, int Cin,
                          int H, int W, int R, void* stream);
int ecgmm_stem_pool_fwd(const float* x, const void* packed, const float* coef, void* pooled, uint8_t* idx, int N, int Cin,
                        int H, int W, void* stream);
size_t ecgmm_stem_pool_bwd_workspace(int N, int Cin, int H, int W);
int ecgmm_stem_pool_bwd(const float* x, const void* packed, const float* coef, const float* gamma, const void* dp,
                        const void* pooled, const uint8_t* idx, float* dgamma, float* dbeta, float* dw_oihw, void* ws,
                        size_t ws_bytes, int N, int Cin, int H, int W, void* stream);

#define ECGMM_BN_TAIL_ROWS 64
int ecgmm_col_stats_rows(int dtype, int64_t M, int C);
int ecgmm_col_stats(int dtype, const void* x, int64_t M, int C, float* partial, void* stream);
int ecgmm_bn_finalize(const float* partial, int rows, int C, double count, const float* gamma, const float* beta,
                      float* running_mean, float* running_var, int64_t* num_batches_tracked, float momentum, float eps,
                      float* coef, void* stream);
int ecgmm_bn_eval_coef(int C, const float* gamma, const float* beta, const float* running_mean,
                       const float* running_var, float eps, float* coef, void* stream);
int ecgmm_bn_act(int dtype, const void* y, const float* coef, const void* res, const float* rcoef, const float* gate,
                 int rows_per_sample, int relu, void* out, int64_t M, int C, void* stream);
int ecgmm_bn_act_from_rows(int dtype, const void* y, const float* partial, int rows, double count, const float* gamma,
                           const float* beta, float* running_mean, float* running_var, int64_t* num_batches_tracked,
                           float momentum, float eps, float* coef_out, const void* res, const float* rcoef,
                           const float* gate, int rows_per_sample, int relu, void* out, int64_t M, int C, void* stream);
size_t ecgmm_bn_bwd_scratch(int dtype, int64_t M, int C);
int ecgmm_bn_bwd(int dtype, const void* dout, const void* maskref, const float* gate, const float* addc,
                 int rows_per_sample, const void* y, const float* coef, const float* gamma, float* dgamma,
                 float* dbeta, void* dy, void* dz_out, float* dbias, int64_t M, int C, void* scratch, void* stream);
int ecgmm_bn_eval_bwd(int dtype, const void* dout, const void* maskref, const float* gate, const float* addc,
                      int rows_per_sample, const void* y, const float* coef, float* dgamma, float* dbeta, void* dy,
                      void* dz_out, float* dbias, int64_t M, int C, float* scratch, void* stream);

int ecgmm_conv_bwd_data_bnred(int dtype, const ecgmm_conv_desc* c, const void* dy, const void* w_dgrad,
                              const void* addend, void* dx, const void* bn_y, const void* bn_mask, const float* bn_coef,
                              float* rows, int* nrows, void* stream);
int ecgmm_conv_bwd_data_bnred_rows(int dtype, const ecgmm_conv_desc* c);
int ecgmm_conv_bwd_data_with_downsample(int dtype, const ecgmm_conv_desc* c, const void* dy, const void* w_dgrad,
                                        const void* dy_down, const void* w_down_dgrad, void* dx, void* tmp,
                                        void* stream);
int ecgmm_bn_bwd_from_rows(int dtype, const void* dout, const void* maskref, const void* y, const float* coef,
                           const float* gamma, float* dgamma, float* dbeta, void* dy, const float* rows, int nrows,
                           int64_t M, int C, void* scratch, void* stream);

int ecgmm_bn_fuse_min_pixels(int64_t m);
int ecgmm_bn_fold(int on);
int ecgmm_bn_fold_slice(int on);
int ecgmm_bn_act_from_rows_bits(int dtype, const void* y, const float* partial, int rows, double count, const float* gamma,
                                const float* beta, float* running_mean, float* running_var, int64_t* num_batches_tracked,
                                float momentum, float eps, float* coef_out, const void* res, const float* rcoef,
                                const float* gate, int rows_per_sample, int relu, void* out, uint8_t* relu_bits, int64_t M,
                                int C, void* stream);
int ecgmm_bn_bwd_bits(int dtype, const void* dout, const uint8_t* mask_bits, const float* gate, const float* addc,
                      int rows_per_sample, const void* y, const float* coef, const float* gamma, float* dgamma,
                      float* dbeta, void* dy, void* dz_out, float* dbias, int64_t M, int C, void* scratch, void* stream);
int ecgmm_bn_bwd_dual(int dtype, const void* dout, const void* maskref, const uint8_t* mask_bits, const float* gate,
                      const float* addc, const void* y_a, const float* coef_a, const float* gamma_a, float* dgamma_a,
                      float* dbeta_a, void* dy_a, const void* y_b, const float* coef_b, const float* gamma_b,
                      float* dgamma_b, float* dbeta_b, void* dy_b, void* dz, float* dbias, int64_t M, int C, void* scratch_a,
                      void* scratch_b, void* stream);
int ecgmm_bn_dual(int on);
int ecgmm_stem_recompute(int on);

int ecgmm_bnrelu_maxpool(int dtype, const void* y, const float* coef, void* out, uint8_t* idx, int N, int H, int W,
                         int C, void* stream);
int ecgmm_maxpool_relu_bwd(int dtype, const void* dp, const void* pooled, const uint8_t* idx, void* dz, int N, int H,
                           int W, int C, void* stream);
int ecgmm_pool_bn_bwd(int dtype, const void* dp, const void* pooled, const uint8_t* idx, const void* y, const float* coef,
                      const float* gamma, float* dgamma, float* dbeta, void* dy, float* dbias, int N, int H, int W, int C,
                      void* scratch, void* stream);
int ecgmm_avgpool(int dtype, const void* x, float* out, int N, int R, int C, const float* coef, void* stream);
int ecgmm_bcast_rows(int dtype, const float* v, void* out, int N, int R, int C, float scale, void* stream);
int ecgmm_se_gate_grad(int dtype, const void* dout, const void* maskref, const void* y, const float* coef, float* dg,
                       int N, int R, int C, void* stream);
int ecgmm_se_gate_bn(int dtype, const void* dout, const void* maskref, const void* y, const float* coef, void* dz, float* dg,
                     float* a1, float* a2, float* a3, int N, int R, int C, void* stream);
int ecgmm_se_mlp_fwd(const float* m, const float* w1, const float* b1, const float* w2, const float* b2, float* h, float* g,
                     int N, int C, int CR, void* stream);
int ecgmm_se_mlp_bwd(const float* dg, const float* g, const float* h, const float* m, const float* w1, const float* w2,
                     float* ds, float* dh, float* dm, float* dw1, float* db1, float* dw2, float* db2, int N, int C, int CR,
                     float scale, void* stream);

int ecgmm_linear_fwd(const float* x, const float* w, const float* bias, float* y, int B, int In, int Out, int act,
                     void* stream);
size_t ecgmm_linear_bwd_scratch(int B, int In, int Out);
int ecgmm_linear_bwd(const float* dz, const float* x, const float* w, float* dx, float* dw, float* db, int B, int In,
                     int Out, void* scratch, size_t scratch_bytes, void* stream);
int ecgmm_act_bwd(const float* dy, const float* y, float* dz, int64_t n, int act, void* stream);

int ecgmm_layernorm_fwd(const float* const* seg, const int* dims, int nseg, const float* fusion_w, const float* gamma,
                        const float* beta, float* out, float* stat, float* soft_w, int B, float eps, void* stream);
size_t ecgmm_layernorm_bwd_scratch(int B, int D);
int ecgmm_layernorm_bwd(const float* const* seg, const int* dims, int nseg, const float* fusion_w, const float* gamma,
                        const float* stat, const float* dout, float* const* dseg, int dseg_accumulate, float* dgamma,
                        float* dbeta, float* dfusion_w, int B, void* scratch, void* stream);

int ecgmm_varloss_fwd(const float* f0, const float* f1, const float* f2, int B, int D0, int D1, int D2, float* loss,
                      float* scratch, void* stream);
int ecgmm_varloss_bwd(const float* f, int B, int D, const float* gout, const float* scratch, int which, float* df,
                      int accumulate, void* stream);

int ecgmm_ce_fwd(const float* logits, const int64_t* labels, int B, int C, int focal, float alpha, float gamma,
                 float* loss, float* dcoef, void* stream);
int ecgmm_ce_bwd(const float* logits, const int64_t* labels, int B, int C, const float* dcoef, const float* gout,
                 float* dlogits, void* stream);
int ecgmm_ce_plus_fwd(const float* logits, const int64_t* labels, int B, int C, const float* extra, float extra_w,
                      float* loss, float* dcoef, void* stream);
int ecgmm_ce_plus_bwd(const float* logits, const int64_t* labels, int B, int C, const float* dcoef, const float* gout,
                      float* dlogits, float* dextra, float extra_w, void* stream);

int ecgmm_dropout_fwd(const float* x, float* y, uint8_t* mask, int64_t n, float p, uint64_t seed, uint64_t offset,
                      void* stream);
int ecgmm_dropout_bwd(const float* dy, const uint8_t* mask, float* dx, int64_t n, float p, void* stream);

int ecgmm_adam(float* p, const float* g, float* m, float* v, int64_t n, float lr, float beta1, float beta2, float eps,
               float weight_decay, int64_t step, float gscale, void* stream);
int ecgmm_axpby(float a, const float* x, float b, float* y, int64_t n, void* stream);

size_t ecgmm_signal_preprocess_workspace(int S, int L, int order);
int ecgmm_signal_preprocess(const float* x, float* out, int S, int L, const float* sc_mean, const float* sc_scale,
                            int window, const double* b, const double* a, const double* zi, int order, void* ws,
                            size_t ws_bytes, void* stream);
int ecgmm_signal_preprocess_i16(const int16_t* raw, int R, int T, int nsig, const int* chan, int nc, const double* gain,
                                const int* baseline, int step, float* out, int out_len, int window, const double* b,
                                const double* a, const double* zi, int order, void* stream);

int ecgmm_signal_filter_zscore(const float* x, float* out, int S, int L, const double* b, const double* a,
                               const double* zi, int order, int zscore, double eps, void* stream);
int ecgmm_signal_filter_lanes(const double* a, int order, int L);
int ecgmm_signal_resample_len(int n, double ratio);
size_t ecgmm_signal_resample_workspace(int S, int L, int T_out);
int ecgmm_signal_resample(const float* x, int S, int L, const int32_t* lengths, int num, double ratio, float* out, int T_out,
                          int32_t* out_lengths, void* ws, size_t ws_bytes, void* stream);
int ecgmm_signal_gather_augment(const float* src, int64_t n, int L, const int64_t* index, int B, float* out,
                                float* decisions, int augment, float p, float sigma, float scale_lo, float scale_hi,
                                int shift_lo, int shift_hi, uint64_t seed, uint64_t offset, void* stream);
int ecgmm_weighted_sample(const double* cdf, int64_t n, int64_t last_positive, int64_t* out, double* u_out, int64_t count,
                          uint64_t seed, uint64_t offset, void* stream);

// ... 186 lines not shown
```

Baseline: 39870 samples/s.

## Batch wgrad slab reductions per residual block and vectorize weight packing

Splits the conv weight-gradient path into a slab-producing launch and a deferred reduction. A per-block WgradBlock allocates successive workspace regions so up to four wgrad slabs stay live and get reduced by one batched kernel with coalesced per-output-row stores. The batched weight pack kernel gains a 16-byte load/store variant. Both are on by default behind runtime switches. This trades fewer launches and better memory access for more workspace pressure, and it changes when the side-stream marks correspond to finished gradients.

```diff
diff --git a/ecg-multimodal-model_amd/csrc/api.hip b/ecg-multimodal-model_amd/csrc/api.hip
--- a/ecg-multimodal-model_amd/csrc/api.hip
+++ b/ecg-multimodal-model_amd/csrc/api.hip
@@ -49,6 +49,8 @@
 int ecgmm_bn_fold(int on) { sw::BN_FOLD.set(on); return 0; }
 int ecgmm_bn_fold_slice(int on) { sw::BN_FOLD_SLICE.set(on); return 0; }
 int ecgmm_bn_dual(int on) { ecg_bn_dual_set(on); return 0; }
+int ecgmm_conv_wgrad_reduce_batched(int on) { sw::WGRAD_REDUCE_BATCH.set(on); return 0; }
+int ecgmm_pack_conv_weight_16b(int on) { sw::PACK_16B.set(on); return 0; }
 int ecgmm_bn_fuse_min_pixels(int64_t m) { sw::BN_FUSE_MIN_M.set((long)m); return 0; }
 int ecgmm_stem_recompute(int on) { sw::STEM_RECOMPUTE.set(on); return 0; }
 int ecgmm_infer_down_side(int on) { sw::INFER_DOWN_SIDE.set(on); return 0; }
@@ -68,6 +70,28 @@
 int ecgmm_pack_conv_weight(int dtype, const float* w, void* fwd, void* dgrad, int Cout, int Cin, int RS,
                            void* stream) {
   return ecg_pack_weight(dtype, w, fwd, dgrad, Cout, Cin, RS, S_(stream));
+}
+
+int ecgmm_pack_conv_weight_batch(int dtype, int n, const float* const* w, void* const* fwd, void* const* dgrad,
+                                 const int* Cout, const int* Cin, const int* RS, void* stream) {
+  if (n < 0 || n > ECG_PACK_MAX || !w || !fwd || !dgrad || !Cout || !Cin || !RS)
+    ECG_FAIL(ECGMM_ERR_SHAPE, "pack_conv_weight_batch: %d tensors (0..%d) or a null table", n, ECG_PACK_MAX);
+  EcgPackItem items[ECG_PACK_MAX];
+  for (int i = 0; i < n; ++i) {
+    if (!w[i] || Cout[i] < 1 || Cin[i] < 1 || RS[i] < 1)
+      ECG_FAIL(ECGMM_ERR_SHAPE, "pack_conv_weight_batch: tensor %d: null weight or empty shape", i);
+    items[i] = {w[i], fwd[i], dgrad[i], Cout[i], Cin[i], RS[i]};
+  }
+  return ecg_pack_weight_batch(dtype, items, n, S_(stream));
+}
+
+int ecgmm_conv_bwd_weight_reduce_batch(int n, const float* const* slabs, float* const* grads, const int* nsplit, const int* RS,
+                                       const int* Cout, const int* Cin, const int* accumulate, void* stream) {
+  if (n < 0 || n > ECG_WGRAD_BATCH_MAX || !slabs || !grads || !nsplit || !RS || !Cout || !Cin || !accumulate)
+    ECG_FAIL(ECGMM_ERR_SHAPE, "conv_bwd_weight_reduce_batch: %d tensors (0..%d) or a null table", n, ECG_WGRAD_BATCH_MAX);
+  EcgWgradPending p[ECG_WGRAD_BATCH_MAX];
+  for (int i = 0; i < n; ++i) p[i] = {slabs[i], grads[i], nsplit[i], RS[i], Cout[i], Cin[i], accumulate[i]};
+  return ecg_conv_wgrad_reduce_batch(p, n, S_(stream));
 }
 
 int ecgmm_conv_stats_rows(int64_t out_pixels) { return ecg_conv_stats_rows((long)out_pixels); }
diff --git a/ecg-multimodal-model_amd/csrc/conv_wgrad.hip b/ecg-multimodal-model_amd/csrc/conv_wgrad.hip
--- a/ecg-multimodal-model_amd/csrc/conv_wgrad.hip
+++ b/ecg-multimodal-model_amd/csrc/conv_wgrad.hip
@@ -666,6 +666,78 @@
   }
 }
 
+struct ReduceBatch {
+  const float* slab[ECG_WGRAD_BATCH_MAX];
+  float* grad[ECG_WGRAD_BATCH_MAX];
+  int ns[ECG_WGRAD_BATCH_MAX], rs[ECG_WGRAD_BATCH_MAX], cout[ECG_WGRAD_BATCH_MAX], cin[ECG_WGRAD_BATCH_MAX];
+  int acc[ECG_WGRAD_BATCH_MAX];
+  int blk0[ECG_WGRAD_BATCH_MAX + 1];
+  int n;
+};
+constexpr int RED_CI = 64, RED_RS_MAX = 9;
+
+template <int RS, int U>
+__device__ __forceinline__ void reduce_step(const float* __restrict__ p, size_t kstride, size_t tstride, float (&s0)[RS],
+                                            float (&s1)[RS]) {
+  float a[U][RS];
+#pragma unroll
+  for (int u = 0; u < U; ++u)
+#pragma unroll
+    for (int t = 0; t < RS; ++t) a[u][t] = p[(size_t)u * 4 * kstride + (size_t)t * tstride];
+#pragma unroll
+  for (int u = 0; u < U; ++u)
+#pragma unroll
+    for (int t = 0; t < RS; ++t) {
+      if (u & 1) s1[t] += a[u][t];
+      else s0[t] += a[u][t];
+    }
+}
+
+template <int RS>
+__device__ __forceinline__ void reduce_tile(const float* __restrict__ slab, float* __restrict__ grad, int ns, int Cout, int Cin,
+                                            int accumulate, int co, int ci0, float (*sh)[RED_CI * RED_RS_MAX]) {
+  const int lane = threadIdx.x & 63, grp = threadIdx.x >> 6;
+  const int ci = ci0 + lane;
+  const size_t tstride = (size_t)Cout * Cin, kstride = (size_t)RS * tstride;
+  float s0[RS], s1[RS];
+#pragma unroll
+  for (int t = 0; t < RS; ++t) s0[t] = s1[t] = 0.f;
+  if (ci < Cin) {
+    const float* __restrict__ p = slab + (size_t)co * Cin + ci;
+    int k = grp;
+    for (; k + 28 < ns; k += 32) reduce_step<RS, 8>(p + (size_t)k * kstride, kstride, tstride, s0, s1);
+    for (; k + 12 < ns; k += 16) reduce_step<RS, 4>(p + (size_t)k * kstride, kstride, tstride, s0, s1);
+    for (; k + 4 < ns; k += 8) reduce_step<RS, 2>(p + (size_t)k * kstride, kstride, tstride, s0, s1);
+    if (k < ns) reduce_step<RS, 1>(p + (size_t)k * kstride, kstride, tstride, s0, s1);
+  }
+#pragma unroll
+  for (int t = 0; t < RS; ++t) sh[grp][lane * RS + t] = s0[t] + s1[t];
+  __syncthreads();
+  const int nci = min(RED_CI, Cin - ci0);
+  float* __restrict__ out = grad + ((size_t)co * Cin + ci0) * RS;
+  for (int j = threadIdx.x; j < nci * RS; j += 256) {
+    const float s = (sh[0][j] + sh[1][j]) + (sh[2][j] + sh[3][j]);
+    out[j] = accumulate ? out[j] + s : s;
+  }
+}
+
+__global__ __launch_bounds__(256) void wgrad_reduce_batch_kernel(ReduceBatch b) {
+  __shared__ float sh[4][RED_CI * RED_RS_MAX];
+  int t = 0;
+  while (t + 1 < b.n && (int)blockIdx.x >= b.blk0[t + 1]) ++t;
+  const int Cout = b.cout[t], Cin = b.cin[t];
+  const int ci_tiles = (Cin + RED_CI - 1) / RED_CI;
+  const int lb = blockIdx.x - b.blk0[t];
+  const int co = lb / ci_tiles, ci0 = (lb % ci_tiles) * RED_CI;
+  if (co >= Cout) return;
+  switch (b.rs[t]) {
+    case 1: reduce_tile<1>(b.slab[t], b.grad[t], b.ns[t], Cout, Cin, b.acc[t], co, ci0, sh); break;
+    case 3: reduce_tile<3>(b.slab[t], b.grad[t], b.ns[t], Cout, Cin, b.acc[t], co, ci0, sh); break;
+    case 9: reduce_tile<9>(b.slab[t], b.grad[t], b.ns[t], Cout, Cin, b.acc[t], co, ci0, sh); break;
+    default: break;
+  }
+}
+
 template <typename T, int NT, int GROUPS>
 int launch_wgrad_nt(WgradParams& p, dim3 grid, hipStream_t stream) {
   size_t lds = (size_t)GROUPS * 2 * (1 + NT) * 4096;
@@ -753,8 +825,13 @@
   return (size_t)ns * g.R * g.S * g.Cout * g.Cin * sizeof(float);
 }
 
-int ecg_conv_wgrad(int dtype, const ConvGeom& g, const void* x, const void* dy, float* grad_oihw, int accumulate,
-                   void* workspace, size_t workspace_bytes, hipStream_t stream) {
+size_t ecg_conv_wgrad_slab_bytes(int dtype, const ConvGeom& g) {
+  const int ns = pick_nsplit(g, dtype == ECGMM_BF16 ? 32 : 16, wgrad_groups(dtype, g));
+  return (size_t)ns * g.R * g.S * g.Cout * g.Cin * sizeof(float);
+}
+
+int ecg_conv_wgrad_launch(int dtype, const ConvGeom& g, const void* x, const void* dy, float* grad_oihw, int accumulate,
+                          void* workspace, size_t workspace_bytes, hipStream_t stream, EcgWgradPending* pending) {
   const int kp = dtype == ECGMM_BF16 ? 32 : 16;
   const int vec = dtype == ECGMM_BF16 ? 8 : 4;
   if (g.Cin % vec || g.Cout % vec)
@@ -797,9 +874,52 @@
   }
   ecg_prof_end(stream);
   ECG_TRY(rc);
-  size_t per = (size_t)g.R * g.S * g.Cout * g.Cin;
-  hipLaunchKernelGGL(wgrad_reduce_kernel, dim3(ceil_div(per, 64)), dim3(256), 0, stream, (const float*)workspace,
-                     grad_oihw, ns, g.R * g.S, g.Cout, g.Cin, accumulate);
-  ECG_CHECK_LAUNCH("wgrad_reduce_kernel");
+  *pending = {(const float*)workspace, grad_oihw, ns, g.R * g.S, g.Cout, g.Cin, accumulate};
   return 0;
 }
+
+int ecg_conv_wgrad_reduce_batch(const EcgWgradPending* pending, int n, hipStream_t stream) {
+  for (int i = 0; i < n; ++i) {
+    const EcgWgradPending& q = pending[i];
+    if (!q.slab || !q.grad || q.ns < 1 || q.Cout < 1 || q.Cin < 1 || (q.RS != 1 && q.RS != 3 && q.RS != 9))
+      ECG_FAIL(ECGMM_ERR_SHAPE, "conv wgrad reduce: tensor %d: ns %d, %d taps, %d x %d channels unsupported", i, q.ns, q.RS,
+               q.Cout, q.Cin);
+    if ((size_t)q.ns * q.RS * q.Cout * q.Cin > 0x7fffffffffULL || (long)q.Cout * ceil_div(q.Cin, RED_CI) > 0x3fffffffL)
+      ECG_FAIL(ECGMM_ERR_SHAPE, "conv wgrad reduce: tensor %d out of range", i);
+  }
+  if (!sw::WGRAD_REDUCE_BATCH.get()) {
+    for (int i = 0; i < n; ++i) {
+      const EcgWgradPending& q = pending[i];
+      size_t per = (size_t)q.RS * q.Cout * q.Cin;
+      hipLaunchKernelGGL(wgrad_reduce_kernel, dim3(ceil_div(per, 64)), dim3(256), 0, stream, q.slab, q.grad, q.ns, q.RS,
+                         q.Cout, q.Cin, q.accumulate);
+      ECG_CHECK_LAUNCH("wgrad_reduce_kernel");
+    }
+    return 0;
+  }
+  for (int base = 0; base < n; base += ECG_WGRAD_BATCH_MAX) {
+    ReduceBatch b;
+    memset(&b, 0, sizeof(b));
+    b.n = n - base < ECG_WGRAD_BATCH_MAX ? n - base : ECG_WGRAD_BATCH_MAX;
+    long blocks = 0;
+    for (int i = 0; i < b.n; ++i) {
+      const EcgWgradPending& q = pending[base + i];
+      b.slab[i] = q.slab; b.grad[i] = q.grad; b.ns[i] = q.ns; b.rs[i] = q.RS; b.cout[i] = q.Cout; b.cin[i] = q.Cin;
+      b.acc[i] = q.accumulate;
+      b.blk0[i] = (int)blocks;
+      blocks += (long)q.Cout * ceil_div(q.Cin, RED_CI);
+    }
+    if (blocks > 0x7fffffffL) ECG_FAIL(ECGMM_ERR_SHAPE, "conv wgrad reduce: %ld workgroups out of range", blocks);
+    b.blk0[b.n] = (int)blocks;
+    hipLaunchKernelGGL(wgrad_reduce_batch_kernel, dim3((unsigned)blocks), dim3(256), 0, stream, b);
+    ECG_CHECK_LAUNCH("wgrad_reduce_batch_kernel");
+  }
+  return 0;
+}
+
+int ecg_conv_wgrad(int dtype, const ConvGeom& g, const void* x, const void* dy, float* grad_oihw, int accumulate,
+                   void* workspace, size_t workspace_bytes, hipStream_t stream) {
+  EcgWgradPending pending;
+  ECG_TRY(ecg_conv_wgrad_launch(dtype, g, x, dy, grad_oihw, accumulate, workspace, workspace_bytes, stream, &pending));
+  return ecg_conv_wgrad_reduce_batch(&pending, 1, stream);
+}
diff --git a/ecg-multimodal-model_amd/csrc/elementwise.hip b/ecg-multimodal-model_amd/csrc/elementwise.hip
--- a/ecg-multimodal-model_amd/csrc/elementwise.hip
+++ b/ecg-multimodal-model_amd/csrc/elementwise.hip
@@ -1350,6 +1350,89 @@
   }
 }
 
+constexpr int PACK_CP = PACK_T + 1, PACK_TP = PACK_T * PACK_CP + 4;
+template <typename T, int RS_>
+__device__ __forceinline__ void pack_tile_16b(const PackBatch& b, int t, float* tile) {
+  constexpr int VEC = Elem<T>::VEC, NV = PACK_T / VEC;
+  const int Cout = b.cout[t], Cin = b.cin[t], RS = RS_ ? RS_ : b.rs[t];
+  const float* __restrict__ w = b.w[t];
+  T* __restrict__ fwd = (T*)b.fwd[t];
+  T* __restrict__ dgr = (T*)b.dgr[t];
+  const int ci_tiles = (Cin + PACK_T - 1) / PACK_T;
+  const int lb = blockIdx.x - b.blk0[t];
+  const int co0 = (lb / ci_tiles) * PACK_T, ci0 = (lb % ci_tiles) * PACK_T;
+  const int nci = min(PACK_T, Cin - ci0), nco = min(PACK_T, Cout - co0);
+  const int run = nci * RS;
+  if (((Cin * RS) & 3) == 0 && (run & 3) == 0 && ((size_t)w & 15) == 0) {
+    const int run4 = run >> 2;
+    for (int i = threadIdx.x; i < nco * run4; i += 256) {
+      const int co = i / run4, k0 = (i - co * run4) * 4;
+      const u32x4 v = ld16(w + ((size_t)(co0 + co) * Cin + ci0) * RS + k0);
+#pragma unroll
+      for (int e = 0; e < 4; ++e) {
+        const int k = k0 + e, ci = k / RS, tap = k - ci * RS;
+        tile[tap * PACK_TP + co * PACK_CP + ci] = __uint_as_float(v[e]);
+      }
+    }
+  } else {
+    for (int i = threadIdx.x; i < nco * run; i += 256) {
+      const int co = i / run, k = i - co * run, ci = k / RS, tap = k - ci * RS;
+      tile[tap * PACK_TP + co * PACK_CP + ci] = w[((size_t)(co0 + co) * Cin + ci0) * RS + k];
+    }
+  }
+  __syncthreads();
+  if (fwd) {
+    const bool vec = Cin % VEC == 0 && ((size_t)fwd & 15) == 0;
+    for (int i = threadIdx.x; i < RS * PACK_T * NV; i += 256) {
+      const int c = (i % NV) * VEC, ct = i / NV, co = ct % PACK_T, tap = ct / PACK_T;
+      if (co >= nco || c >= nci) continue;
+      const float* src = tile + tap * PACK_TP + co * PACK_CP + c;
+      T* dst = fwd + ((size_t)(co0 + co) * RS + tap) * Cin + ci0 + c;
+      float f[VEC];
+#pragma unroll
+      for (int j = 0; j < VEC; ++j) f[j] = src[j];
+      if (vec) {
+        st16(dst, pack16<T>(f));
+      } else {
+#pragma unroll
+        for (int j = 0; j < VEC; ++j)
+          if (c + j < nci) Elem<T>::st(dst + j, f[j]);
+      }
+    }
+  }
+  if (dgr) {
+    const bool vec = Cout % VEC == 0 && ((size_t)dgr & 15) == 0;
+    for (int i = threadIdx.x; i < RS * PACK_T * NV; i += 256) {
+      const int c = (i % NV) * VEC, ct = i / NV, ci = ct % PACK_T, tap = ct / PACK_T;
+      if (ci >= nci || c >= nco) continue;
+      const float* src = tile + tap * PACK_TP + c * PACK_CP + ci;
+      T* dst = dgr + ((size_t)(ci0 + ci) * RS + tap) * Cout + co0 + c;
+      float f[VEC];
+#pragma unroll
+      for (int j = 0; j < VEC; ++j) f[j] = c + j < nco ? src[j * PACK_CP] : 0.f;
+      if (vec) {
+        st16(dst, pack16<T>(f));
+      } else {
+#pragma unroll
+        for (int j = 0; j < VEC; ++j)
+          if (c + j < nco) Elem<T>::st(dst + j, f[j]);
+      }
+    }
+  }
+}
+template <typename T>
+__global__ __launch_bounds__(256) void pack_weight_batch16_kernel(PackBatch b) {
+  __shared__ float tile[PACK_RS_MAX * PACK_TP];
+  int t = 0;
+  while (t + 1 < b.n && (int)blockIdx.x >= b.blk0[t + 1]) ++t;
+  switch (b.rs[t]) {
+    case 1: pack_tile_16b<T, 1>(b, t, tile); break;
+    case 3: pack_tile_16b<T, 3>(b, t, tile); break;
+    case 9: pack_tile_16b<T, 9>(b, t, tile); break;
+    default: pack_tile_16b<T, 0>(b, t, tile); break;
+  }
+}
+
 template <typename T, bool TO_NHWC>
 __global__ __launch_bounds__(256) void nchw_nhwc_kernel(const void* __restrict__ src_, void* __restrict__ dst_, int C,
                                                         long HW) {
@@ -1911,8 +1994,13 @@
       blocks += ceil_div(it.Cout, 32) * ceil_div(it.Cin, 32);
     }
     b.blk0[b.n] = blocks;
-    DISPATCH_T(dtype, hipLaunchKernelGGL(pack_weight_batch_kernel<bf16_t>, dim3(blocks), dim3(256), 0, stream, b),
-               hipLaunchKernelGGL(pack_weight_batch_kernel<float>, dim3(blocks), dim3(256), 0, stream, b), "pack_weight_batch");
+    if (sw::PACK_16B.get()) {
+      DISPATCH_T(dtype, hipLaunchKernelGGL(pack_weight_batch16_kernel<bf16_t>, dim3(blocks), dim3(256), 0, stream, b),
+                 hipLaunchKernelGGL(pack_weight_batch16_kernel<float>, dim3(blocks), dim3(256), 0, stream, b), "pack_weight_batch");
+    } else {
+      DISPATCH_T(dtype, hipLaunchKernelGGL(pack_weight_batch_kernel<bf16_t>, dim3(blocks), dim3(256), 0, stream, b),
+                 hipLaunchKernelGGL(pack_weight_batch_kernel<float>, dim3(blocks), dim3(256), 0, stream, b), "pack_weight_batch");
+    }
     ECG_CHECK_LAUNCH("pack_weight_batch");
   }
   return 0;
diff --git a/ecg-multimodal-model_amd/csrc/ops.h b/ecg-multimodal-model_amd/csrc/ops.h
--- a/ecg-multimodal-model_amd/csrc/ops.h
+++ b/ecg-multimodal-model_amd/csrc/ops.h
@@ -29,6 +29,16 @@
 void ecg_conv_wgrad_narrow(bool narrow, int slots = 256);
 int ecg_conv_wgrad(int dtype, const ConvGeom& g, const void* x, const void* dy, float* grad_oihw, int accumulate,
                    void* workspace, size_t workspace_bytes, hipStream_t stream);
+constexpr int ECG_WGRAD_BATCH_MAX = 4;
+struct EcgWgradPending {
+  const float* slab;
+  float* grad;
+  int ns, RS, Cout, Cin, accumulate;
+};
+size_t ecg_conv_wgrad_slab_bytes(int dtype, const ConvGeom& g);
+int ecg_conv_wgrad_launch(int dtype, const ConvGeom& g, const void* x, const void* dy, float* grad_oihw, int accumulate,
+                          void* workspace, size_t workspace_bytes, hipStream_t stream, EcgWgradPending* pending);
+int ecg_conv_wgrad_reduce_batch(const EcgWgradPending* pending, int n, hipStream_t stream);
 size_t ecg_stem_packed_elems(int Cin, int R);
 int ecg_stem_stats_rows(int N, int Cin, int H, int W, int R);
 int ecg_stem_pack(int dtype, const float* w, void* out, int Cin, int R, hipStream_t stream);
diff --git a/ecg-multimodal-model_amd/csrc/plan_common.h b/ecg-multimodal-model_amd/csrc/plan_common.h
--- a/ecg-multimodal-model_amd/csrc/plan_common.h
+++ b/ecg-multimodal-model_amd/csrc/plan_common.h
@@ -79,6 +79,31 @@
   }
 }
 
+struct WgradBlock {
+  int dtype;
+  unsigned char* base;
+  size_t bytes, off = 0;
+  hipStream_t stream;
+  EcgWgradPending pend[ECG_WGRAD_BATCH_MAX];
+  int n = 0;
+  WgradBlock(int dt, void* ws, size_t ws_bytes, hipStream_t s) : dtype(dt), base((unsigned char*)ws), bytes(ws_bytes), stream(s) {}
+  int launch(const ConvGeom& g, const void* x, const void* dy, float* grad) {
+    const size_t need = ecg_conv_wgrad_slab_bytes(dtype, g);
+    if (n && (n == ECG_WGRAD_BATCH_MAX || off + need > bytes)) ECG_TRY(reduce());
+    ECG_TRY(ecg_conv_wgrad_launch(dtype, g, x, dy, grad, 0, base + off, bytes - off, stream, &pend[n]));
+    ++n;
+    off = align_up(off + need, 256);
+    if (off > bytes) off = bytes;
+    return 0;
+  }
+  int reduce() {
+    const int m = n;
+    n = 0;
+    off = 0;
+    return ecg_conv_wgrad_reduce_batch(pend, m, stream);
+  }
+};
+
 inline int ws_view_find(const char* who, const WsTable& t, const char* name, int index, size_t ws_bytes, size_t* offset,
                         size_t* bytes) {
   if (t.overflow) ECG_FAIL(ECGMM_ERR_SHAPE, "%s: more named tensors than the view table holds", who);
diff --git a/ecg-multimodal-model_amd/csrc/plan_resnet18.hip b/ecg-multimodal-model_amd/csrc/plan_resnet18.hip
--- a/ecg-multimodal-model_amd/csrc/plan_resnet18.hip
+++ b/ecg-multimodal-model_amd/csrc/plan_resnet18.hip
@@ -335,6 +335,7 @@
       ConvGeom g2 = k.conv2_geom(N);
       const int pp = st & 1;
       void *dyb = q.dy[pp], *dy1b = q.dy1[pp], *dydb = q.dyd[pp];
+      WgradBlock wgb(dt, q.wg_ws, q.wg_bytes, ws);
       bool fused2 = false;
       int fused2_rows = 0;
       const bool fuse_here = train && sw::BN_FUSE.get() && M >= sw::BN_FUSE_MIN_M.get();
@@ -365,7 +366,7 @@
       }
       if (G(grads, k.p_conv2)) {
         if (side) side_fork(s);
-        ECG_TRY(ecg_conv_wgrad(dt, g2, b.a1, dyb, G(grads, k.p_conv2), 0, q.wg_ws, q.wg_bytes, ws));
+        ECG_TRY(wgb.launch(g2, b.a1, dyb, G(grads, k.p_conv2)));
         if (side) g_side.done2[0][pp] = side_mark();
       }
       ConvEpi ea = {};
@@ -381,9 +382,10 @@
       }
       if (G(grads, k.p_conv1)) {
         if (side) side_fork(s);
-        ECG_TRY(ecg_conv_wgrad(dt, g1, in, dy1b, G(grads, k.p_conv1), 0, q.wg_ws, q.wg_bytes, ws));
+        ECG_TRY(wgb.launch(g1, in, dy1b, G(grads, k.p_conv1)));
         if (side) g_side.done2[1][pp] = side_mark();
       }
+      if (!k.down) ECG_TRY(wgb.reduce());
       if (k.down) {
         ConvGeom gd = k.down_geom(N);
         if (!dual) {
@@ -393,9 +395,10 @@
         }
         if (G(grads, k.p_dconv)) {
           if (side) side_fork(s);
-          ECG_TRY(ecg_conv_wgrad(dt, gd, in, dydb, G(grads, k.p_dconv), 0, q.wg_ws, q.wg_bytes, ws));
+          ECG_TRY(wgb.launch(gd, in, dydb, G(grads, k.p_dconv)));
           if (side) g_side.done2[2][pp] = side_mark();
         }
+        ECG_TRY(wgb.reduce());
         ConvEpi ed = {};
         ed.src2 = dydb; ed.wpk2 = b.wdd;
         if (!sw::DOWN_FOLD.get()) ed.src2 = nullptr;
diff --git a/ecg-multimodal-model_amd/csrc/plan_resnet1d.hip b/ecg-multimodal-model_amd/csrc/plan_resnet1d.hip
--- a/ecg-multimodal-model_amd/csrc/plan_resnet1d.hip
+++ b/ecg-multimodal-model_amd/csrc/plan_resnet1d.hip
@@ -274,6 +274,7 @@
       const long M = (long)N * k.lout;
       ConvGeom g1 = k.conv1_geom(N);
       ConvGeom g2 = k.conv2_geom(N);
+      WgradBlock wgb(dt, q.wg_ws, q.wg_bytes, wst);
       const bool se_merge = sw::SE_MERGE.get() && train;
       if (se_merge) {
         ECG_TRY(ecg_se_gate_bn(dt, dcur, b.out, b.y2, b.coef2, q.dz, q.dg, q.sa1, q.sa2, q.sa3, N, k.lout, k.cout, s));
@@ -305,7 +306,7 @@
       }
       if (G(grads, p + T1_CONV2_W)) {
         if (side) g_side1.fork(s);
-        ECG_TRY(ecg_conv_wgrad(dt, g2, b.a1, q.dy, G(grads, p + T1_CONV2_W), 0, q.wg_ws, q.wg_bytes, wst));
+        ECG_TRY(wgb.launch(g2, b.a1, q.dy, G(grads, p + T1_CONV2_W)));
         if (side) g_side1.doneA = g_side1.mark();
       }
       ECG_TRY(ecg_conv_igemm(dt, 1, g2, q.dy, b.w2d, q.da, nullptr, nullptr, nullptr, 0, s));
@@ -315,9 +316,10 @@
                           G(grads, p + T1_CONV1_B), M, k.cout, q.bn_scratch, s));
       if (G(grads, p + T1_CONV1_W)) {
         if (side) g_side1.fork(s);
-        ECG_TRY(ecg_conv_wgrad(dt, g1, in, q.dy1, G(grads, p + T1_CONV1_W), 0, q.wg_ws, q.wg_bytes, wst));
+        ECG_TRY(wgb.launch(g1, in, q.dy1, G(grads, p + T1_CONV1_W)));
         if (side) g_side1.doneB = g_side1.mark();
       }
+      if (!k.down) ECG_TRY(wgb.reduce());
       if (k.down) {
         ConvGeom gd = k.down_geom(N);
         main_wait(s, g_side1.doneC);
@@ -326,9 +328,10 @@
                             q.bn_scratch, s));
         if (G(grads, p + T1_DOWN_W)) {
           if (side) g_side1.fork(s);
-          ECG_TRY(ecg_conv_wgrad(dt, gd, in, q.dyd, G(grads, p + T1_DOWN_W), 0, q.wg_ws, q.wg_bytes, wst));
+          ECG_TRY(wgb.launch(gd, in, q.dyd, G(grads, p + T1_DOWN_W)));
           if (side) g_side1.doneC = g_side1.mark();
         }
+        ECG_TRY(wgb.reduce());
         ConvEpi ed = {};
         if (sw::DOWN_FOLD.get()) { ed.src2 = q.dyd; ed.wpk2 = b.wdd; }
         if (ed.src2) ECG_TRY(ecg_conv_igemm(dt, 1, g1, q.dy1, b.w1d, din, nullptr, nullptr, nullptr, 0, s, &ed));
diff --git a/ecg-multimodal-model_amd/csrc/switches.h b/ecg-multimodal-model_amd/csrc/switches.h
--- a/ecg-multimodal-model_amd/csrc/switches.h
+++ b/ecg-multimodal-model_amd/csrc/switches.h
@@ -67,7 +67,7 @@
 
 inline Switch* const ALL[] = {
     &CONV_HALO,  &HALO_CUS,      &HALO_W4,       &HALO_STAGGER, &HALO_STREAM,   &HALO_PP,   &HALO_NCS1,  &WGRAD_RING,      &WGRAD_PP,
-    &WGRAD_GROUPS, &WGRAD_WGS,   &BN_FOLD,       &BN_FOLD_SLICE, &BN_FUSE,      &BN_FUSE_MIN_M, &RELU_BITS, &STEM_FUSE,    &STEM_RECOMPUTE,
+    &WGRAD_GROUPS, &WGRAD_WGS,   &BN_FOLD,      &BN_FOLD_SLICE, &BN_FUSE,      &BN_FUSE_MIN_M, &RELU_BITS, &STEM_FUSE,    &STEM_RECOMPUTE,
     &DOWN_FOLD,  &DOWN_SIDE,     &SIDE_WGRAD,    &INFER_DOWN_SIDE, &SE_MERGE,   &SE_MLP_FUSED, &HEAD_FUSED, &DENSE16};
 constexpr int COUNT = (int)(sizeof(ALL) / sizeof(ALL[0]));
 
@@ -76,4 +76,13 @@
     if (env && strcmp(s->env, env) == 0) return s;
   return nullptr;
 }
+
+struct RuntimeSwitch {
+  long v;
+  const char* doc;
+  long get() const { return v; }
+  void set(long x) { v = x != 0; }
+};
+inline RuntimeSwitch WGRAD_REDUCE_BATCH{1, "slab reductions as one batched launch with coalesced stores (0: wgrad_reduce_kernel per tensor)"};
+inline RuntimeSwitch PACK_16B{1, "batched weight pack with 16-byte loads and stores (0: one element per store)"};
 }
diff --git a/ecg-multimodal-model_amd/hip/lib.py b/ecg-multimodal-model_amd/hip/lib.py
--- a/ecg-multimodal-model_amd/hip/lib.py
+++ b/ecg-multimodal-model_amd/hip/lib.py
@@ -102,6 +102,10 @@
     "ecgmm_conv_bwd_data": (i32, [i32, P(ConvDesc), vp, vp, vp, vp, vp]),
     "ecgmm_conv_bwd_weight_workspace": (sz, [i32, P(ConvDesc)]),
     "ecgmm_conv_bwd_weight": (i32, [i32, P(ConvDesc), vp, vp, vp, i32, vp, sz, vp]),
+    "ecgmm_conv_bwd_weight_reduce_batch": (i32, [i32, P(vp), P(vp), P(i32), P(i32), P(i32), P(i32), P(i32), vp]),
+    "ecgmm_conv_wgrad_reduce_batched": (i32, [i32]),
+    "ecgmm_pack_conv_weight_batch": (i32, [i32, i32, P(vp), P(vp), P(vp), P(i32), P(i32), P(i32), vp]),
+    "ecgmm_pack_conv_weight_16b": (i32, [i32]),
     "ecgmm_stem_packed_elems": (sz, [i32, i32]),
     "ecgmm_stem_stats_rows": (i32, [i32, i32, i32, i32, i32]),
     "ecgmm_stem_pack": (i32, [i32, vp, vp, i32, i32, vp]),
@@ -310,7 +314,9 @@
                  "ecgmm_crnn_front_infer_workspace", "ecgmm_crnn_front_infer",
                  "ecgmm_linear_res_ln", "ecgmm_ffn_res_ln", "ecgmm_transformer_infer_prepared_bytes",
                  "ecgmm_transformer_infer_prepare", "ecgmm_transformer_infer_workspace", "ecgmm_transformer_infer",
-                 "ecgmm_tabnet_infer_prepared_bytes", "ecgmm_tabnet_infer_prepare", "ecgmm_tabnet_infer")
+                 "ecgmm_tabnet_infer_prepared_bytes", "ecgmm_tabnet_infer_prepare", "ecgmm_tabnet_infer",
+                 "ecgmm_conv_bwd_weight_reduce_batch", "ecgmm_conv_wgrad_reduce_batched", "ecgmm_pack_conv_weight_batch",
+                 "ecgmm_pack_conv_weight_16b")
 
 _lib = None
 
diff --git a/include/ecgmm.h b/include/ecgmm.h
--- a/include/ecgmm.h
+++ b/include/ecgmm.h
@@ -128,6 +128,9 @@
 int ecgmm_uncast(int dtype, const void* src, float* dst, int64_t n, void* stream);
 int ecgmm_pack_conv_weight(int dtype, const float* w_oihw, void* fwd, void* dgrad, int Cout, int Cin, int RS,
                            void* stream);
+int ecgmm_pack_conv_weight_batch(int dtype, int n, const float* const* w_oihw, void* const* fwd, void* const* dgrad,
+                                 const int* Cout, const int* Cin, const int* RS, void* stream);
+int ecgmm_pack_conv_weight_16b(int on);
 
 int ecgmm_conv_stats_rows(int64_t out_pixels);
 int ecgmm_conv_halo_enable(int on);
@@ -147,6 +150,9 @@
 size_t ecgmm_conv_bwd_weight_workspace(int dtype, const ecgmm_conv_desc* c);
 int ecgmm_conv_bwd_weight(int dtype, const ecgmm_conv_desc* c, const void* x, const void* dy, float* dw_oihw,
                           int accumulate, void* ws, size_t ws_bytes, void* stream);
+int ecgmm_conv_bwd_weight_reduce_batch(int n, const float* const* slabs, float* const* grads, const int* nsplit, const int* RS,
+                                       const int* Cout, const int* Cin, const int* accumulate, void* stream);
+int ecgmm_conv_wgrad_reduce_batched(int on);
 
 size_t ecgmm_stem_packed_elems(int Cin, int R);
 int ecgmm_stem_stats_rows(int N, int Cin, int H, int W, int R);
```

Result: no change. 40030 samples/s, median of 6 (+0.4%).
